# EvolEcolGroup/tidypopgen

Hardware: AMD Instinct MI355X
Metric: SNP-genotypes/s (N x M) for IBS+KING+GRM+Fst+PCA; max |delta| vs CPU ref (cpu_baseline.parity) (higher is better)
Workload: dtype fp4-e2m1 operands (exact integers, f32 accumulate) for the cross-products, the PCA Gram and the grouped counts, int8 (int32 accumulate) for the loadings, f64 for statistics

## Files before the change

### tidypopgen_amd/csrc/admix.hip

```cpp
#include "common.h"
#include "synth_common.h"

#include <math.h>

namespace {

constexpr int ADM_CHUNK = TPG_ADMIX_CHUNK_LOCI;
static_assert(ADM_CHUNK % 128 == 0, "a chunk is whole blocks of T");
constexpr uint64_t ADM_F_SALT = 0xF0F0F0F0F0F0F0F0ull;

__host__ __device__ inline double admix_u(uint64_t h) { return ((double)(h >> 11) + 0.5) * 0x1p-53; }

__device__ __forceinline__ double admix_clamp(double f) {
  return f < TPG_ADMIX_EPS ? TPG_ADMIX_EPS : f > 1.0 - TPG_ADMIX_EPS ? 1.0 - TPG_ADMIX_EPS : f;
}
__device__ __forceinline__ bool admix_finite(double x) { return fabs(x) <= 1.79769313486231570815e308; }

__device__ __forceinline__ int admix_code(uint32_t w, int e) { return (int)((w >> (8 * (e & 3) + 2 * (e >> 2))) & 3u); }

__global__ void admix_seed_q_kernel(double* __restrict__ Qd, int64_t n, int K, int KT, uint64_t seed) {
  const int64_t i = (int64_t)blockIdx.x * blockDim.x + threadIdx.x;
  if (i >= n) return;
  const uint64_t key = tpg_mix64(seed ^ tpg_mix64((uint64_t)i));
  double s = 0;
// ... 183 lines not shown
        pb = fma(qv[k], 1.0 - fs[k], pb);
      }
      cnt++;
      const double w1 = (double)g / p, w0 = (double)(2 - g) / pb;
#pragma unroll
      for (int k = 0; k < KT; k++) S[k] = fma(1.0 - fs[k], w0, fma(fs[k], w1, S[k]));
    }
  }
#pragma unroll
  for (int k = 0; k < KT; k++) S[k] += __shfl_xor(S[k], 32);
  cnt += __shfl_xor(cnt, 32);
  admix_wave_order_sum<KT>(S, cnt, stage, cnts, w, r, h);
  if (w != 0 || h != 0 || i >= n) return;
  const int64_t o = c * n + i;
#pragma unroll
  for (int k = 0; k < KT; k++) part[o * KT + k] = S[k];
  cpart[o] = cnt;
}

__global__ void admix_q_combine_kernel(const double* __restrict__ part, const int32_t* __restrict__ cpart, int64_t nchunks, int64_t n,
                                       int K, int KT, const double* __restrict__ Qd, double* __restrict__ Qn) {
  const int64_t idx = (int64_t)blockIdx.x * blockDim.x + threadIdx.x;
  if (idx >= n * KT) return;
  const int64_t i = idx / KT;
  const int k = (int)(idx % KT);
  double q = 0.0;
  if (k < K) {
    double s = 0.0;
    int64_t t = 0;
    for (int64_t c = 0; c < nchunks; c++) {
      s += part[(c * n + i) * KT + k];
      t += cpart[c * n + i];
    }
    q = Qd[idx];
    if (t > 0) q = (q / (2.0 * (double)t)) * s;
  }
  Qn[idx] = q;
}

__global__ __launch_bounds__(256) void admix_ll_sum_kernel(const double* __restrict__ ll_part, int64_t ntiles, double* __restrict__ out) {
  __shared__ double wll[4];
  double s = 0.0;
  for (int64_t t = threadIdx.x; t < ntiles; t += 256) s += ll_part[t];
  for (int o = 32; o > 0; o >>= 1) s += __shfl_xor(s, o);
  if ((threadIdx.x & 63) == 0) wll[threadIdx.x >> 6] = s;
  __syncthreads();
  if (threadIdx.x == 0) *out = ((wll[0] + wll[1]) + wll[2]) + wll[3];
}

int admix_kt(int K) { return K <= 4 ? K : K <= 8 ? 8 : K <= 16 ? 16 : 32; }

#define ADM_DISPATCH(kt, CALL) \
  switch (kt) {                \
    case 1: CALL(1); break;    \
    case 2: CALL(2); break;    \
    case 3: CALL(3); break;    \
    case 4: CALL(4); break;    \
    case 8: CALL(8); break;    \
    case 16: CALL(16); break;  \
    default: CALL(32); break;  \
  }

struct AdmixRun {
  tpg_ctx* ctx;
  const tpg_view* v;
  int K, KT;
  int64_t n, m, n_lt, n_rt, nchunks;
  DevArena sc;
  double *Q[2] = {}, *F[2] = {}, *part = nullptr, *ll_part = nullptr, *trace = nullptr;
  int32_t *cpart = nullptr, *flag = nullptr;

  int init(tpg_ctx* c, const tpg_view* view, int k, bool need_q_sweep, bool need_f_next, int64_t trace_len) {
    ctx = c; v = view; K = k; KT = admix_kt(k);
    n = v->n; m = v->m;
    n_lt = ceil_div(m, 32); n_rt = ceil_div(n, 32); nchunks = ceil_div(m, ADM_CHUNK);
    TPG_REQUIRE(n_lt <= 0x7FFFFFFF && n_rt <= 0x7FFFFFFF && nchunks <= 65535, TPG_EUNSUPPORTED, "admixture on a view of %lld x %lld",
                (long long)n, (long long)m);
    TPG_TRY(sc.get(&Q[0], (size_t)n * KT));
    TPG_TRY(sc.get(&F[0], (size_t)m * KT));
    TPG_TRY(sc.get(&ll_part, (size_t)n_lt));
    TPG_TRY(sc.get(&trace, (size_t)trace_len));
    TPG_TRY(sc.get(&flag, (size_t)1));
    if (need_f_next) TPG_TRY(sc.get(&F[1], (size_t)m * KT));
    if (need_q_sweep) {
      TPG_TRY(tpg_view_need_T(ctx, v));
      TPG_TRY(sc.get(&Q[1], (size_t)n * KT));
      TPG_TRY(sc.get(&part, (size_t)nchunks * n * KT));
      TPG_TRY(sc.get(&cpart, (size_t)nchunks * n));
    }
    return TPG_OK;
  }

  int f_sweep(int cur_q, int cur_f, bool update, int64_t slot) {
#define ADM_F(KT_)                                                                                                                  \
  do {                                                                                                                              \
    auto k_upd = admix_f_sweep_kernel<KT_, true>;                                                                                   \
    auto k_ll = admix_f_sweep_kernel<KT_, false>;                                                                                   \
    if (update)                                                                                                                     \
      TPG_LAUNCH(ctx, "admix_f_sweep", k_upd, dim3((unsigned)n_lt), dim3(256), 0, (const uint32_t*)v->L, \
                 v->Q, n, m, K, (const double*)Q[cur_q], (const double*)F[cur_f], F[1 - cur_f], ll_part);                           \
    else                                                                                                                            \
      TPG_LAUNCH(ctx, "admix_loglik", k_ll, dim3((unsigned)n_lt), dim3(256), 0, (const uint32_t*)v->L, \
                 v->Q, n, m, K, (const double*)Q[cur_q], (const double*)F[cur_f], (double*)nullptr, ll_part);                       \
  } while (0)
    ADM_DISPATCH(KT, ADM_F);
#undef ADM_F
    TPG_LAUNCH(ctx, "admix_ll_sum", admix_ll_sum_kernel, dim3(1), dim3(256), 0, (const double*)ll_part, n_lt, trace + slot);
    TPG_CHECK_LAUNCH();
    return TPG_OK;
  }

  int q_sweep(int cur_q, int cur_f) {
#define ADM_Q(KT_)                                                                                                               \
  TPG_LAUNCH(ctx, "admix_q_sweep", admix_q_sweep_kernel<KT_>, dim3((unsigned)n_rt, (unsigned)nchunks), dim3(256), 0,              \
             (const uint32_t*)v->T, v->KG, n, m, (const double*)Q[cur_q], (const double*)F[cur_f], part, cpart)
    ADM_DISPATCH(KT, ADM_Q);
#undef ADM_Q
    TPG_LAUNCH(ctx, "admix_q_combine", admix_q_combine_kernel, dim3((unsigned)ceil_div(n * KT, 256)), dim3(256), 0, (const double*)part,
               (const int32_t*)cpart, nchunks, n, K, KT, (const double*)Q[cur_q], Q[1 - cur_q]);
    TPG_CHECK_LAUNCH();
    return TPG_OK;
  }
};

int admix_check_view(const tpg_view* v, int K) {
  TPG_REQUIRE(K >= 1 && K <= TPG_ADMIX_MAX_K, TPG_EINVAL, "K = %d out of [1, %d]", K, TPG_ADMIX_MAX_K);
  TPG_REQUIRE(v->n > 0 && v->m > 0, TPG_EINVAL, "admixture needs at least one individual and one locus (view of %lld x %lld)",
              (long long)v->n, (long long)v->m);
  return TPG_OK;
}

}

extern "C" int64_t tpg_admix_chunk_loci(void) { return ADM_CHUNK; }

extern "C" int tpg_admix_params_default(tpg_admix_params* p) {
  TPG_REQUIRE(p, TPG_EINVAL, "null argument");
  p->max_iter = 1000;
  p->tol = 1e-4;
  p->update_q = 1;
  p->update_f = 1;
  p->seed = 0;
  return TPG_OK;
}

extern "C" int tpg_admix_em(tpg_ctx* ctx, const tpg_view* v, const double* ploidy, int K, const tpg_admix_params* params,
                            const double* q0, const double* f0, double* Q, double* P, double* loglik, double* loglik_trace,
                            int32_t* n_iter, int32_t* converged) {
  TpgEnter _enter(ctx);
  TPG_REQUIRE(ctx && v && Q && P, TPG_EINVAL, "null argument");
  tpg_admix_params pr;
  tpg_admix_params_default(&pr);
  if (params) pr = *params;
  TPG_TRY(admix_check_view(v, K));
  TPG_REQUIRE(pr.max_iter >= 0, TPG_EINVAL, "max_iter = %d is negative", (int)pr.max_iter);
  TPG_REQUIRE(pr.tol >= 0.0, TPG_EINVAL, "tol must be a non-negative number");
  TPG_TRY(tpg_require_diploid(v->n, ploidy, "admixture"));
  const bool upd_q = pr.update_q != 0, upd_f = pr.update_f != 0;
  const int64_t n = v->n, m = v->m;
  AdmixRun run;
  TPG_TRY(run.init(ctx, v, K, upd_q && pr.max_iter > 0, upd_f && pr.max_iter > 0, (int64_t)pr.max_iter + 1));
  const int KT = run.KT;
  const unsigned gn = (unsigned)ceil_div(n, 256), gm = (unsigned)ceil_div(m, 256);
  InBuf iq, ifr;
  TPG_HIP(hipMemsetAsync(run.flag, 0, sizeof(int32_t), ctx->stream));
  if (q0) {
// ... 72 lines not shown
```

### tidypopgen_amd/csrc/common.h

```cpp
#pragma once
#include <hip/hip_runtime.h>
#include <stdint.h>
#include <stdlib.h>

#include <map>
#include <memory>
#include <set>
#include <string>
#include <vector>

#include "../../include/tpg.h"

void tpg_set_error(const char* fmt, ...);

#define TPG_HIP(call)                                                                        \
  do {                                                                                       \
    hipError_t _e = (call);                                                                  \
    if (_e != hipSuccess) {                                                                  \
      tpg_set_error("%s:%d: %s -> %s", __FILE__, __LINE__, #call, hipGetErrorString(_e));     \
      return TPG_EHIP;                                                                       \
    }                                                                                        \
  } while (0)

#define TPG_REQUIRE(cond, code, ...)  \
// ... 47 lines not shown

struct ProfScope {
  tpg_ctx* ctx;
  ProfRec rec;
  bool on;
  ProfScope(tpg_ctx* c, const char* name);
  ~ProfScope();
};
int tpg_prof_resolve(tpg_ctx* ctx);
int tpg_gram_classes(tpg_ctx* ctx, const struct tpg_view* v, const double* d_w, double* d_what, double* d_K, bool* done,
                     bool centred_ok);
int tpg_gram_classes_exchanged(tpg_ctx* ctx, struct tpg_comm* comm, const struct tpg_view* v, const int32_t* d_counts,
                               const double* d_scale, double* d_K, bool* done);

#define TPG_LAUNCH(ctx, name, kernel, grid, block, shmem, ...)                          \
  do {                                                                                  \
    ProfScope _ps((ctx), (name));                                                       \
    hipLaunchKernelGGL(kernel, grid, block, shmem, (ctx)->stream, __VA_ARGS__);        \
  } while (0)

#define TPG_CHECK_LAUNCH() TPG_HIP(hipGetLastError())

struct tpg_fbm {
  tpg_ctx* ctx;
  uint8_t* d_bytes;
  int64_t nrow, ncol;
  int64_t bed_bpl = 0;
  bool pooled = false;
};

struct GroupedCounts {
  int32_t* cnt = nullptr;
  int64_t Mpad = 0;
  int Cpad = 0;
  int nclass = 0;
};

static inline int64_t ceil_div(int64_t a, int64_t b) { return (a + b - 1) / b; }

hipError_t tpg_pmalloc(void** p, size_t bytes);
void tpg_pfree(void* p);
void tpg_pool_trim(int pool_id);
struct TpgEnter {
  tpg_ctx* prev;
  explicit TpgEnter(tpg_ctx* ctx);
  ~TpgEnter();
};
tpg_ctx* tpg_current_ctx();

struct DevBuf {
  void* p = nullptr;
  int alloc(size_t bytes) {
    free();
    TPG_HIP(tpg_pmalloc(&p, bytes ? bytes : 16));
    return TPG_OK;
  }
  template <typename T> int alloc_n(size_t count) { return alloc(sizeof(T) * count); }
  void free() { if (p) tpg_pfree(p); p = nullptr; }
  void* release() { void* q = p; p = nullptr; return q; }
  template <typename T> T* as() const { return (T*)p; }
  DevBuf() = default;
  DevBuf(DevBuf&& o) noexcept : p(o.release()) {}
  DevBuf& operator=(DevBuf&& o) noexcept { if (this != &o) { free(); p = o.release(); } return *this; }
  DevBuf(const DevBuf&) = delete;
  DevBuf& operator=(const DevBuf&) = delete;
  ~DevBuf() { free(); }
};
struct DevArena {
  std::vector<DevBuf> blocks;
  template <typename T> int get(T** p, size_t count) {
    DevBuf b;
    TPG_TRY(b.alloc_n<T>(count));
    *p = b.as<T>();
    blocks.push_back(std::move(b));
    return TPG_OK;
  }
};

struct tpg_view {
  tpg_ctx* ctx;
  int64_t n, m;
  int64_t Q, KG;
  mutable uint4* T = nullptr;
  uint4* L;
  bool L_borrowed = false;
  size_t bytes_each;
  mutable uint4* T4 = nullptr;
  mutable DevBuf gc_buf;
  mutable GroupedCounts gc_cache;
  mutable std::vector<int32_t> gc_cls;
  uint32_t* lc_part = nullptr;
  int lc_chunks = 0;
  int64_t lc_row = 0;

  tpg_view(tpg_ctx* c, int64_t n_, int64_t m_, uint4* borrowed_L = nullptr)
      : ctx(c), n(n_), m(m_), Q(ceil_div(n_, 128)), KG(ceil_div(m_, 128)), L(borrowed_L), L_borrowed(borrowed_L != nullptr),
        bytes_each((size_t)Q * (size_t)KG * 4096) {}
  tpg_view(const tpg_view&) = delete;
  tpg_view& operator=(const tpg_view&) = delete;
  ~tpg_view();
  void drop_derived();
};
typedef std::unique_ptr<tpg_view> ViewPtr;

#define TPG_PW_PRODUCTS 5
enum { TPG_PW_SLAB_MM = 0, TPG_PW_SLAB_D = 1 , TPG_PW_SLAB_H = 2, TPG_PW_SLAB_HM = 3, TPG_PW_SLAB_MH = 4 };
#define TPG_PW_TA 3
#define TPG_PW_PLANE_INTS (TPG_PW_TA * 16 * 64)
#define TPG_PW_TILE_INTS (TPG_PW_PRODUCTS * TPG_PW_PLANE_INTS)
struct tpg_pairwise {
  tpg_ctx* ctx;
  int64_t n;
  int64_t nst;
  int64_t ntp;
  int32_t* acc;
  bool owns;
  void* order;
  int64_t nun;
  int64_t loci;
  int64_t as_pad_quirk;
  int nranks = 1, rank = 0;
  int64_t chunk_units = 0, tail_units = 0;
  std::vector<int32_t> band;
  int64_t* rowpad = nullptr;
  bool reduced = false;
  bool reducing = false;
  hipEvent_t ev_acc = nullptr, ev_red = nullptr;
  int64_t pending_loci = 0;
  int pending_lack = 0;
  int have = 31;
  std::map<int, std::pair<void*, int64_t>> orders;
};
#define TPG_PW_MAX_LOCI 2147483647ll
#define TPG_PW_HAVE_ALL (TPG_PW_ALL | TPG_PW_DH)
static inline int tpg_pw_products_for(bool ibs, bool king, bool as_or_grm) {
  if (ibs && !king && !as_or_grm) return TPG_PW_FOR_IBS_ALONE;
  return (ibs ? TPG_PW_FOR_IBS : 0) | (king ? TPG_PW_FOR_KING : 0) | (as_or_grm ? TPG_PW_FOR_AS : 0);
}

static inline bool tpg_env_set(const char* name) { return getenv(name) != nullptr; }
static inline int tpg_env_int(const char* name, int dflt) {
  const char* e = getenv(name);
  return e ? atoi(e) : dflt;
}

hipError_t tpg_h2d_async(tpg_ctx* ctx, void* dst, const void* src, size_t bytes);
hipError_t tpg_fetch_small(tpg_ctx* ctx, void* host_dst, const void* d_src, size_t bytes);
hipError_t tpg_push_small(tpg_ctx* ctx, void* d_dst, const void* host_src, size_t bytes);
hipError_t tpg_copy_dev(tpg_ctx* ctx, void* d_dst, const void* d_src, size_t bytes);
hipError_t tpg_upload(tpg_ctx* ctx, void* dst, const void* src, size_t bytes);
hipError_t tpg_download(tpg_ctx* ctx, void* dst, const void* src, size_t bytes);
int tpg_fbm_from_host_for_table(tpg_ctx* ctx, const uint8_t* bytes, int64_t nrow, int64_t ncol, const double* code256, tpg_fbm** out,
                                const double** view_table);
hipError_t tpg_upload_bedpacked(tpg_ctx* ctx, uint8_t* dst, const uint8_t* src, int64_t nrow, int64_t ncols, const uint8_t* lut16, bool* ok);
hipError_t tpg_download_rows(tpg_ctx* ctx, void* dst, size_t dpitch, const void* src, size_t width, size_t height);
void tpg_stage_keep(int buffers);

template <typename T>
static inline int tpg_dmalloc(T** p, size_t count) {
  TPG_HIP(hipMalloc((void**)p, count * sizeof(T) > 0 ? count * sizeof(T) : 16));
  return TPG_OK;
}

bool tpg_is_device_ptr(const void* p);
struct OutBuf {
  void* user = nullptr;
  void* d = nullptr;
  size_t bytes = 0;
  bool owned = false;
  int init(void* user_ptr, size_t nbytes);
  int commit(tpg_ctx* ctx);
  ~OutBuf();
  template <typename T> T* dev() { return (T*)d; }
};
struct InBuf {
  const void* d = nullptr;
  void* owned_ptr = nullptr;
  int init(tpg_ctx* ctx, const void* user_ptr, size_t nbytes);
  ~InBuf();
  template <typename T> const T* dev() { return (const T*)d; }
};
template <typename T>
struct HostIn {
  const T* p = nullptr;
  std::vector<T> keep;
  int init(tpg_ctx* ctx, const T* user, int64_t count) {
    p = user;
    if (!tpg_is_device_ptr(user)) return TPG_OK;
    keep.resize((size_t)count);
    TPG_HIP(tpg_download(ctx, keep.data(), user, sizeof(T) * (size_t)count));
    p = keep.data();
    return TPG_OK;
  }
  const T& operator[](int64_t i) const { return p[i]; }
};
int tpg_check_ranges(tpg_ctx* ctx, const int64_t* lo, const int64_t* hi, int64_t count, int64_t m, const char* what);

void tpg_resident_release(tpg_ctx* ctx);

struct tpg_comm {
  tpg_ctx* ctx = nullptr;
  int nranks = 1, rank = 0;
  void* nccl = nullptr;
  int (*host_fn)(void* user, void* buf, int64_t count, int dtype) = nullptr;
  void* host_user = nullptr;
  int32_t* d_status = nullptr;
  int a2a_state = 0;
};
#define TPG_COMM_STATUS_INTS 8
int tpg_sym_eig_topk_tol(tpg_ctx* ctx, const double* d_K, int64_t n, int k, double tol, double* lambda_host, double* d_U);
int tpg_pca_gram_allreduce(tpg_ctx* ctx, tpg_comm* comm, double* d_K, int64_t n);
int tpg_multi_stream_host(tpg_multi* mg, const uint8_t* fbm_bytes, int64_t nrow, int64_t ncol, size_t budget, const tpg_stream_job* job);
int tpg_comm_agree(tpg_comm* comm, int rc);
int tpg_comm_reduce_scatter_i32(tpg_comm* comm, int32_t* d_buf, int64_t chunk_count);
int tpg_comm_allreduce(tpg_comm* comm, void* d_buf, int64_t count, int dtype);
bool tpg_comm_alltoall_usable(tpg_comm* comm);
int tpg_comm_alltoallv64(tpg_comm* comm, const void* d_send, const size_t* scnt, const size_t* soff, void* d_recv,
                         const size_t* rcnt, const size_t* roff);

int tpg_launch_pack(tpg_ctx* ctx, const tpg_fbm* fbm, const int32_t* d_rows, const int32_t* d_cols,
                    const uint8_t* d_lut, tpg_view* v, tpg_view* v2);
int tpg_launch_unpack(tpg_ctx* ctx, const tpg_view* v, uint8_t* d_codes, int from_L);
int tpg_view_need_T(tpg_ctx* ctx, const tpg_view* v);
int tpg_view_impute_at(tpg_ctx* ctx, const tpg_view* raw, int method, uint64_t seed, int64_t col0, tpg_view** out,
                       tpg_impute_report* rep);
int tpg_launch_synth(tpg_ctx* ctx, uint8_t* d_bytes, uint64_t seed, int64_t nrow, int64_t ncol, int64_t j0,
                     int npop, uint32_t miss_thresh, int imputed_bytes);

int tpg_launch_loci_counts(tpg_ctx* ctx, const tpg_view* v, int32_t* d_counts );
int tpg_grouped_counts(tpg_ctx* ctx, const tpg_view* v, const int32_t* h_cls, int nclass, GroupedCounts* out);
struct ClassPlan {
  std::vector<int32_t> cls;
  std::vector<int32_t> group_size;
  int nclass = 0;
  int has_hap = 0;
};
int make_class_plan(int64_t n, const int32_t* groupIds0, int ngroups, const double* ploidy, ClassPlan* cp);
int tpg_check_group_ids(int64_t n, const int32_t* groupIds0, int ngroups);
int tpg_require_diploid(int64_t n, const double* ploidy, const char* what);
int tpg_launch_indiv_accumulate(tpg_ctx* ctx, const tpg_view* v, int32_t* d_acc);
int tpg_launch_indiv_finish(tpg_ctx* ctx, const int32_t* d_acc, int64_t n, int64_t m, int32_t* d_out);
```

### tidypopgen_amd/csrc/gramcls.hip

```cpp
#include <math.h>
#include <string.h>

#include <algorithm>
#include <vector>

#include <hipcub/hipcub.hpp>

#include "common.h"
#include "devfrag.h"
#include "host/host_bits2.h"

typedef int v8i __attribute__((ext_vector_type(8)));
typedef float v16f __attribute__((ext_vector_type(16)));
typedef uint32_t v4u __attribute__((ext_vector_type(4)));

constexpr int GA = 2, GB = 2, GP = GA * GB;
#define GCLS_SLAB (GP * 16 * 64)
#define GCLS_MAX_RUN 65536

__global__ void tpg_gcls_keys_kernel(const double* __restrict__ w, int64_t m, unsigned long long* __restrict__ key,
                                     uint32_t* __restrict__ idx) {
  for (int64_t j = blockIdx.x * (int64_t)blockDim.x + threadIdx.x; j < m; j += (int64_t)gridDim.x * blockDim.x) {
    const unsigned long long b = (unsigned long long)__double_as_longlong(w[j]);
    key[j] = (b + 16ull) & ~31ull;
// ... 640 lines not shown
  const double cost_dig = (double)ceil_div(nun_dig, (int64_t)(4 * ncu8)) * ((double)ceil_div(m, 128) * 0.25 * t_dig) + 65.0;
  while ((nblocks / 2 + S) / S + 2 >= (1 << 21)) S += 2;
  if (tpg_env_set("TPG_DEBUG"))
    fprintf(stderr, "[tpg] gram classes: %lld classes, %lld blocks for %lld loci, S = %d, model %.0f us (digits %.0f us)\n",
            (long long)nruns, (long long)nblocks, (long long)m, S, cost_cls, cost_dig);
  if (cost_cls > cost_dig && !force && !tpg_env_set("TPG_GRAM_CLASSES")) return TPG_OK;

  int32_t* d_src = nullptr;
  double* d_slabs = nullptr;
  unsigned long long* d_wblk = nullptr;
  ulonglong2* d_wblk2 = nullptr;
  uint4* d_T2g = nullptr;
  int2* d_order = nullptr;
  TPG_TRY(B.get(&d_src, (size_t)nblocks * 64));
  if (f64) TPG_TRY(B.get(&d_wblk, (size_t)nblocks));
  else TPG_TRY(B.get(&d_wblk2, (size_t)nblocks + 4));
  const int64_t rs2 = (nblocks + 1) / 2;
  TPG_TRY(B.get(&d_T2g, (size_t)(4 * Q) * (size_t)rs2 * 64));
  TPG_TRY(B.get(&d_order, (size_t)nun));
  TPG_TRY(B.get(&d_slabs, (size_t)S * (size_t)nun * GCLS_SLAB));
  TPG_HIP(tpg_h2d_async(ctx, d_order, order.data(), sizeof(int2) * (size_t)nun));
  TPG_HIP(hipMemsetAsync(d_src, 0xFF, sizeof(int32_t) * (size_t)nblocks * 64, ctx->stream));
  {
    ProfScope ps(ctx, "gcls_layout");
    hipLaunchKernelGGL(tpg_gcls_place_kernel, dim3(1024), dim3(256), 0, ctx->stream, (const uint32_t*)d_idx2,
                       (const unsigned long long*)d_ukeys, (const uint32_t*)d_estart, (const uint32_t*)d_bstart, (int)nruns, m,
                       d_src, d_what);
    if (f64)
      hipLaunchKernelGGL(tpg_gcls_block_table_kernel, dim3(256), dim3(256), 0, ctx->stream, (const unsigned long long*)d_ukeys,
                         (const uint32_t*)d_bstart, (const uint32_t*)d_nblk, (int)nruns, nblocks, d_wblk);
    else
      hipLaunchKernelGGL(tpg_gcls_block_table2_kernel, dim3(256), dim3(256), 0, ctx->stream, (const unsigned long long*)d_ukeys,
                         (const uint32_t*)d_bstart, (const uint32_t*)d_nblk, (int)nruns, nblocks, GCLS_GMAX, GCLS_GQ, d_wblk2);
  }
  {
    const int64_t tasks = Q * rs2;
    if (tasks >= ((int64_t)1 << 31)) return TPG_OK;
    const unsigned grid = (unsigned)std::min<int64_t>(ceil_div(tasks, 4), (int64_t)ctx->num_cu * 16);
    const int qw = tpg_env_int("TPG_GATHER_QW", Q >= 4 ? 4 : Q >= 2 ? 2 : 1);
#define GATHER_GO(C, W) TPG_LAUNCH(ctx, "gcls_gather", (tpg_gcls_gather_kernel<C, W>), dim3(grid), dim3(256), 0, src, Q, (const int32_t*)d_src, nblocks, rs2, d_T2g)
    if (cen) { if (qw == 4) GATHER_GO(true, 4); else if (qw == 2) GATHER_GO(true, 2); else GATHER_GO(true, 1); }
    else { if (qw == 4) GATHER_GO(false, 4); else if (qw == 2) GATHER_GO(false, 2); else GATHER_GO(false, 1); }
#undef GATHER_GO
  }
  if (f64)
    TPG_LAUNCH(ctx, "pca_gram_classes", tpg_gcls_gram_kernel, dim3((unsigned)nblk_grid), dim3(256), 0, (const uint4*)d_T2g, nblocks,
               rs2, nrtv, (const unsigned long long*)d_wblk, (const int2*)d_order, nun, S, d_slabs);
  else if (cen) {
    (void)hipFuncSetAttribute((const void*)tpg_gcls_gram2_kernel<true>, hipFuncAttributeMaxDynamicSharedMemorySize, GCLS2_LDS_BYTES);
    TPG_LAUNCH(ctx, "pca_gram_classes", tpg_gcls_gram2_kernel<true>, dim3((unsigned)nblk_grid), dim3(256), GCLS2_LDS_BYTES,
               (const uint4*)d_T2g, nblocks, rs2, nrtv, (const ulonglong2*)d_wblk2, (const int2*)d_order, nun, S, d_slabs);
  } else {
    (void)hipFuncSetAttribute((const void*)tpg_gcls_gram2_kernel<false>, hipFuncAttributeMaxDynamicSharedMemorySize, GCLS2_LDS_BYTES);
    TPG_LAUNCH(ctx, "pca_gram_classes", tpg_gcls_gram2_kernel<false>, dim3((unsigned)nblk_grid), dim3(256), GCLS2_LDS_BYTES,
               (const uint4*)d_T2g, nblocks, rs2, nrtv, (const ulonglong2*)d_wblk2, (const int2*)d_order, nun, S, d_slabs);
  }
  TPG_LAUNCH(ctx, "gcls_assemble", tpg_gcls_assemble_kernel, dim3((unsigned)std::min<int64_t>(nun, 4096)), dim3(256), 0,
             (const double*)d_slabs, (const int2*)d_order, nun, S, (int)n, d_K);
  TPG_CHECK_LAUNCH();
  *done = true;
  return TPG_OK;
}

__global__ __launch_bounds__(256) void tpg_gcls_l2lm_kernel(const uint4* __restrict__ L, int64_t Q, int64_t n_lt,
                                                            uint4* __restrict__ LM) {
  __shared__ uint4 sh[32][8];
  const int64_t QG = (Q + 3) / 4;
  const int lane = threadIdx.x & 63, wv = threadIdx.x >> 6;
  for (int64_t task = blockIdx.x; task < n_lt * QG; task += gridDim.x) {
    const int64_t lt = task / QG, q0 = (task % QG) * 4;
    if (q0 + wv < Q) sh[lane & 31][2 * wv + (lane >> 5)] = L[(lt * Q + q0 + wv) * 64 + lane];
    __syncthreads();
    const int r = threadIdx.x >> 3, p = threadIdx.x & 7;
    if (q0 + (p >> 1) < Q) LM[((lt * 32 + r) * Q + q0) * 2 + p] = sh[r][p];
    __syncthreads();
  }
}

int tpg_gram_classes(tpg_ctx* ctx, const tpg_view* v, const double* d_w, double* d_what, double* d_K, bool* done,
                     bool centred_ok) {
  *done = false;
  if (tpg_env_set("TPG_GRAM_DIGITS")) return TPG_OK;
  const int64_t n_lt = 4 * v->KG;
  DevBuf d_LM;
  TPG_TRY(d_LM.alloc_n<uint4>((size_t)n_lt * 32 * (size_t)v->Q * 2));
  TPG_LAUNCH(ctx, "gcls_l2lm", tpg_gcls_l2lm_kernel, dim3((unsigned)std::min<int64_t>(n_lt * ((v->Q + 3) / 4), (int64_t)ctx->num_cu * 32)),
             dim3(256), 0, (const uint4*)v->L, v->Q, n_lt, d_LM.as<uint4>());
  const GclsSrc src{d_LM.as<uint4>(), 0, 2 * v->Q, 0, 0, 2, 1};
  const int rc = gram_classes_core(ctx, v->n, v->Q, v->m, src, d_w, d_what, d_K, false, done, centred_ok);
  d_LM.free();
  return rc;
}

#define GCLX_REC_WORDS(Q) (4 * (Q) + 2)

__global__ void tpg_gclx_keys_kernel(const int32_t* __restrict__ counts, int64_t m, int n, int32_t* __restrict__ key,
                                     int32_t* __restrict__ hist) {
  for (int64_t j = blockIdx.x * (int64_t)blockDim.x + threadIdx.x; j < m; j += (int64_t)gridDim.x * blockDim.x) {
    const int c = counts[4 * j + 1] + 2 * counts[4 * j + 2];
    const int k = min(c, 2 * n - c);
    key[j] = k;
    atomicAdd(&hist[k], 1);
  }
}

__global__ void tpg_gclx_dest_kernel(const int32_t* __restrict__ key, int64_t m, const uint8_t* __restrict__ owner,
                                     uint32_t* __restrict__ dest, uint32_t* __restrict__ idx, int32_t* __restrict__ per_dest) {
  for (int64_t j = blockIdx.x * (int64_t)blockDim.x + threadIdx.x; j < m; j += (int64_t)gridDim.x * blockDim.x) {
    const uint32_t d = owner[key[j]];
    dest[j] = d;
    idx[j] = (uint32_t)j;
    atomicAdd(&per_dest[d], 1);
  }
}

__global__ __launch_bounds__(256) void tpg_gclx_pack_kernel(const uint4* __restrict__ L, int64_t Q, const uint32_t* __restrict__ order,
                                                            const double* __restrict__ scale, int64_t m,
                                                            uint4* __restrict__ rec) {
  const int lane = threadIdx.x & 63;
  const int64_t recq = 2 * Q + 1;
  for (int64_t i = (int64_t)blockIdx.x * 4 + (threadIdx.x >> 6); i < m; i += (int64_t)gridDim.x * 4) {
    const uint32_t j = order[i];
    const uint4* p = L + ((int64_t)(j >> 5) * Q) * 64 + (j & 31);
    for (int64_t t = lane; t < 2 * Q; t += 64) rec[i * recq + t] = p[(t >> 1) * 64 + (t & 1) * 32];
    if (lane == 0) {
      const double sc = scale[j], w = 1.0 / (sc * sc);
      rec[i * recq + 2 * Q] = make_uint4((uint32_t)__double_as_longlong(w), (uint32_t)(__double_as_longlong(w) >> 32), 0u, 0u);
    }
  }
}

__global__ void tpg_gclx_weights_kernel(const uint4* __restrict__ rec, int64_t Q, int64_t m, double* __restrict__ w) {
  const int64_t recq = 2 * Q + 1;
  for (int64_t i = blockIdx.x * (int64_t)blockDim.x + threadIdx.x; i < m; i += (int64_t)gridDim.x * blockDim.x) {
    const uint4 t = rec[i * recq + 2 * Q];
    w[i] = __longlong_as_double((long long)(((unsigned long long)t.y << 32) | t.x));
  }
}

int tpg_gram_classes_exchanged(tpg_ctx* ctx, tpg_comm* comm, const tpg_view* v, const int32_t* d_counts, const double* d_scale,
                               double* d_K, bool* done) {
  *done = false;
  const int R = comm->nranks, me = comm->rank;
  const int64_t n = v->n, m = v->m, Q = v->Q;
  if (R < 2 || R > 255 || n >= (1 << 30) || tpg_env_set("TPG_GRAM_NO_EXCHANGE")) return TPG_OK;
  DevArena B;
  int32_t *d_key = nullptr, *d_hist = nullptr, *d_perdest = nullptr;
  uint8_t* d_owner = nullptr;
  uint32_t *d_dest = nullptr, *d_dest2 = nullptr, *d_idx = nullptr, *d_idx2 = nullptr;
  void* d_tmp = nullptr;
  size_t t_sort = 0;
  std::vector<int32_t> hist((size_t)n + 1, 0);
  auto local = [&]() -> int {
    TPG_TRY(B.get(&d_key, (size_t)std::max<int64_t>(m, 1)));
    TPG_TRY(B.get(&d_hist, (size_t)n + 1));
    TPG_TRY(B.get(&d_perdest, (size_t)R));
    TPG_TRY(B.get(&d_owner, (size_t)n + 1));
    TPG_TRY(B.get(&d_dest, (size_t)std::max<int64_t>(m, 1)));
    TPG_TRY(B.get(&d_dest2, (size_t)std::max<int64_t>(m, 1)));
    TPG_TRY(B.get(&d_idx, (size_t)std::max<int64_t>(m, 1)));
    TPG_TRY(B.get(&d_idx2, (size_t)std::max<int64_t>(m, 1)));
    TPG_HIP(hipcub::DeviceRadixSort::SortPairs(nullptr, t_sort, d_dest, d_dest2, d_idx, d_idx2, (int)m, 0, 8, ctx->stream));
    TPG_TRY(B.get((uint8_t**)&d_tmp, t_sort));
    TPG_HIP(hipMemsetAsync(d_hist, 0, sizeof(int32_t) * ((size_t)n + 1), ctx->stream));
    TPG_HIP(hipMemsetAsync(d_perdest, 0, sizeof(int32_t) * (size_t)R, ctx->stream));
    if (m > 0)
      TPG_LAUNCH(ctx, "gclx_keys", tpg_gclx_keys_kernel, dim3(512), dim3(256), 0, d_counts, m, (int)n, d_key, d_hist);
    TPG_CHECK_LAUNCH();
    return TPG_OK;
  };
  TPG_TRY(tpg_comm_agree(comm, local()));
  if (!tpg_comm_alltoall_usable(comm)) return TPG_OK;
  {
    ProfScope ps(ctx, "gclx_histogram");
    TPG_TRY(tpg_comm_allreduce(comm, d_hist, n + 1, 0));
    TPG_HIP(hipMemcpyAsync(hist.data(), d_hist, sizeof(int32_t) * ((size_t)n + 1), hipMemcpyDeviceToHost, ctx->stream));
    TPG_HIP(hipStreamSynchronize(ctx->stream));
  }
  int64_t m_all = 0, runs_all = 0, blocks_all = 0;
  for (int64_t k = 0; k <= n; k++)
    if (hist[(size_t)k] > 0) { m_all += hist[(size_t)k]; runs_all++; blocks_all += ((int64_t)hist[(size_t)k] + 63) / 64; }
  if (m_all == 0) return TPG_OK;
  const double cost_all = (double)runs_all * 0.136 + (double)blocks_all * 0.079;
  const int nrtv = (int)ceil_div(n, 32);
  const double units = (double)nrtv * (double)nrtv / 8.0, waves = 8.0 * (double)(ctx->num_cu > 8 ? ctx->num_cu : 8);
  const double t_exch = units / waves * 4.0 * cost_all / R + 700.0 + (double)m_all / R * (double)(32 * Q + 16) / 300e3;
  const double shard_blocks = (double)blocks_all / R + (double)runs_all;
  const double t_cls_local = units / waves * 4.0 * ((double)runs_all * 0.136 + shard_blocks * 0.079) + 650.0;
  const double t_dig_local = ((double)nrtv * nrtv / 8.0 + nrtv) / (waves / 2.0) * ((double)m_all / R / 128.0) + 65.0;
  if (tpg_env_set("TPG_DEBUG") && me == 0)
    fprintf(stderr, "[tpg] gram exchange: %lld loci, %lld classes, %lld blocks over %d ranks: model %.0f us (local classes %.0f, digits %.0f)\n",
            (long long)m_all, (long long)runs_all, (long long)blocks_all, R, t_exch, t_cls_local, t_dig_local);
  if (t_exch > std::min(t_cls_local, t_dig_local) && !tpg_env_set("TPG_GRAM_EXCHANGE")) return TPG_OK;

  std::vector<uint8_t> owner((size_t)n + 1, (uint8_t)(R - 1));
  {
    double acc = 0;
    int r = 0;
    for (int64_t k = 0; k <= n; k++) {
      owner[(size_t)k] = (uint8_t)r;
      if (hist[(size_t)k] > 0) acc += 0.136 + 0.079 * (double)(((int64_t)hist[(size_t)k] + 63) / 64);
      while (r < R - 1 && acc >= cost_all * (double)(r + 1) / R) r++;
    }
  }
  std::vector<int32_t> per_dest((size_t)R, 0);
  uint4 *d_send = nullptr, *d_recv = nullptr;
  double* d_w = nullptr;
  const int64_t recq = 2 * Q + 1;
  std::vector<size_t> scnt((size_t)R), soff((size_t)R), rcnt((size_t)R), roff((size_t)R);
  std::vector<int32_t> cm((size_t)R * R, 0);
  int64_t m_in = 0;
  auto pack = [&]() -> int {
    TPG_HIP(tpg_h2d_async(ctx, d_owner, owner.data(), (size_t)n + 1));
    if (m > 0) {
      ProfScope ps(ctx, "gclx_sort");
      hipLaunchKernelGGL(tpg_gclx_dest_kernel, dim3(512), dim3(256), 0, ctx->stream, (const int32_t*)d_key, m, (const uint8_t*)d_owner,
                         d_dest, d_idx, d_perdest);
      size_t t = t_sort;
      TPG_HIP(hipcub::DeviceRadixSort::SortPairs(d_tmp, t, d_dest, d_dest2, d_idx, d_idx2, (int)m, 0, 8, ctx->stream));
    }
    TPG_HIP(hipMemcpyAsync(per_dest.data(), d_perdest, sizeof(int32_t) * (size_t)R, hipMemcpyDeviceToHost, ctx->stream));
    TPG_HIP(hipStreamSynchronize(ctx->stream));
    TPG_TRY(B.get(&d_send, (size_t)std::max<int64_t>(m, 1) * (size_t)recq));
    if (m > 0)
      TPG_LAUNCH(ctx, "gclx_pack", tpg_gclx_pack_kernel, dim3((unsigned)std::min<int64_t>(ceil_div(m, 4), (int64_t)ctx->num_cu * 16)),
                 dim3(256), 0, (const uint4*)v->L, Q, (const uint32_t*)d_idx2, d_scale, m, d_send);
    TPG_HIP(hipGetLastError());
    return TPG_OK;
  };
  TPG_TRY(tpg_comm_agree(comm, pack()));
  {
    int32_t* d_cm = nullptr;
    auto cm_up = [&]() -> int {
      TPG_TRY(B.get(&d_cm, (size_t)R * R));
      for (int d = 0; d < R; d++) cm[(size_t)me * R + d] = per_dest[(size_t)d];
      TPG_HIP(tpg_h2d_async(ctx, d_cm, cm.data(), sizeof(int32_t) * (size_t)R * R));
      return TPG_OK;
    };
    TPG_TRY(tpg_comm_agree(comm, cm_up()));
    TPG_TRY(tpg_comm_allreduce(comm, d_cm, (int64_t)R * R, 0));
    TPG_HIP(hipMemcpyAsync(cm.data(), d_cm, sizeof(int32_t) * (size_t)R * R, hipMemcpyDeviceToHost, ctx->stream));
    TPG_HIP(hipStreamSynchronize(ctx->stream));
  }
  {
    size_t so = 0, ro = 0;
    for (int r = 0; r < R; r++) {
      scnt[(size_t)r] = (size_t)cm[(size_t)me * R + r] * (size_t)recq * 2;
      soff[(size_t)r] = so;
      so += scnt[(size_t)r];
      rcnt[(size_t)r] = (size_t)cm[(size_t)r * R + me] * (size_t)recq * 2;
      roff[(size_t)r] = ro;
      ro += rcnt[(size_t)r];
      m_in += cm[(size_t)r * R + me];
    }
  }
  auto recv_alloc = [&]() -> int {
    TPG_TRY(B.get(&d_recv, (size_t)std::max<int64_t>(m_in, 1) * (size_t)recq));
    TPG_TRY(B.get(&d_w, (size_t)std::max<int64_t>(m_in, 1)));
    return TPG_OK;
  };
  TPG_TRY(tpg_comm_agree(comm, recv_alloc()));
  {
    ProfScope ps(ctx, "gclx_alltoall");
    TPG_TRY(tpg_comm_alltoallv64(comm, d_send, scnt.data(), soff.data(), d_recv, rcnt.data(), roff.data()));
  }
  if (m_in == 0) {
    TPG_HIP(hipMemsetAsync(d_K, 0, sizeof(double) * (size_t)n * (size_t)n, ctx->stream));
    *done = true;
    return TPG_OK;
  }
  TPG_LAUNCH(ctx, "gclx_weights", tpg_gclx_weights_kernel, dim3(512), dim3(256), 0, (const uint4*)d_recv, Q, m_in, d_w);
  const GclsSrc src{d_recv, 0, recq, 0, 0, 2, 1};
  bool ok = false;
  TPG_TRY(gram_classes_core(ctx, n, Q, m_in, src, d_w, nullptr, d_K, true, &ok, true));
  TPG_REQUIRE(ok, TPG_EHIP, "class Gram of the exchanged loci was not computed");
  *done = true;
  return TPG_OK;
}
```

### tidypopgen_amd/csrc/impute.hip

```cpp
#include <stdlib.h>
#include <string.h>

#include <algorithm>

#include "common.h"
#include "devfrag.h"
#include "synth_common.h"

TPG_HD int tpg_impute_fill(int method, int64_t c0, int64_t c1, int64_t c2) {
  if (method == TPG_IMPUTE_MODE) {
    int v = 0;
    int64_t best = c0;
    if (c1 > best) { v = 1; best = c1; }
    if (c2 > best) v = 2;
    return v;
  }
  const int64_t t = c0 + c1 + c2, s2 = 2 * (c1 + 2 * c2);
  if (s2 <= t) return 0;
  if (s2 < 3 * t) return 1;
  return 2;
}
TPG_HD uint64_t tpg_impute_locus_key(uint64_t seed, uint64_t j) { return tpg_mix64(seed ^ tpg_mix64(j)); }
TPG_HD int tpg_impute_draw(uint64_t locus_key, uint64_t i, uint64_t thr) {
  const uint64_t h = tpg_mix64(locus_key ^ tpg_mix64(i));
// ... 225 lines not shown
    TPG_HIP(hipStreamSynchronize(ctx->stream));
  }
  stat.free();
  TPG_REQUIRE(h[2] == 0, TPG_EUNSUPPORTED, "object x is already imputed (%llu loci hold a store byte above 3; the store is unchanged)",
              h[2]);
  if (rep) {
    rep->imputed = (int64_t)h[0];
    rep->loci_all_missing = (int64_t)h[1];
  }
  return TPG_OK;
}

__global__ __launch_bounds__(256) void tpg_impute_view_kernel(const uint4* __restrict__ L, uint4* __restrict__ out, int64_t n_lt, int64_t Q,
                                                              int64_t n, int64_t m, int method, uint64_t seed, int64_t col0,
                                                              unsigned long long* __restrict__ d_rep) {
  const int lane = threadIdx.x & 63, r = lane & 31, h = lane >> 5;
  const int64_t lt = (int64_t)blockIdx.x * 4 + (threadIdx.x >> 6);
  if (lt >= n_lt) return;
  const uint4* p = L + (lt * Q) * 64 + lane;
  uint4* o = out + (lt * Q) * 64 + lane;
  int c1 = 0, c2 = 0, c3 = 0;
  for (int64_t q = 0; q < Q; q++) {
    const uint4 a = p[q * 64];
    const uint32_t w[4] = {a.x, a.y, a.z, a.w};
#pragma unroll
    for (int d = 0; d < 4; d++) {
      const uint32_t lo = w[d] & 0x55555555u, hi = (w[d] >> 1) & 0x55555555u;
      c1 += __popc(lo & ~hi);
      c2 += __popc(hi & ~lo);
      c3 += __popc(lo & hi);
    }
  }
  c1 += __shfl_xor(c1, 32);
  c2 += __shfl_xor(c2, 32);
  c3 += __shfl_xor(c3, 32);
  const int64_t j = lt * 32 + r;
  c3 -= (int)(Q * 128 - n);
  const int64_t c0 = n - c1 - c2 - c3, t = n - c3, s = (int64_t)c1 + 2 * (int64_t)c2;
  const bool fill = j < m && t > 0 && c3 > 0;
  const int v = fill && method != TPG_IMPUTE_RANDOM ? tpg_impute_fill(method, c0, c1, c2) : 0;
  const uint64_t key = tpg_impute_locus_key(seed, (uint64_t)(col0 + j)), thr = fill ? ((uint64_t)s << 31) / (uint64_t)t : 0;
  for (int64_t q = 0; q < Q; q++) {
    const uint4 a = p[q * 64];
    uint32_t w[4] = {a.x, a.y, a.z, a.w};
    if (fill) {
#pragma unroll
      for (int d = 0; d < 4; d++) {
        const int64_t base = 128 * q + 32 * d + 16 * h;
        uint32_t miss = w[d] & (w[d] >> 1) & 0x55555555u;
        if (base + 16 > n) {
          uint32_t real = 0;
          for (int e = 0; e < 16; e++)
            if (base + e < n) real |= 1u << tpg_elem_shift(e);
          miss &= real;
        }
        if (method != TPG_IMPUTE_RANDOM) {
          w[d] = (w[d] & ~(miss * 3u)) | (miss * (uint32_t)v);
        } else {
          while (miss) {
            const int pos = __ffs(miss) - 1;
            miss &= miss - 1;
            const int e = 4 * ((pos & 7) >> 1) + (pos >> 3);
            const int vv = tpg_impute_draw(key, (uint64_t)(base + e), thr);
            w[d] = (w[d] & ~(3u << pos)) | ((uint32_t)vv << pos);
          }
        }
      }
    }
    o[q * 64] = make_uint4(w[0], w[1], w[2], w[3]);
  }
  int imp = lane < 32 && fill ? c3 : 0, allmiss = lane < 32 && j < m && t == 0 ? 1 : 0;
  imp = wave_sum(imp);
  allmiss = wave_sum(allmiss);
  if (lane == 0) {
    if (imp) atomicAdd(d_rep, (unsigned long long)imp);
    if (allmiss) atomicAdd(d_rep + 1, (unsigned long long)allmiss);
  }
}

int tpg_view_impute_at(tpg_ctx* ctx, const tpg_view* raw, int method, uint64_t seed, int64_t col0, tpg_view** out,
                       tpg_impute_report* rep) {
  TPG_REQUIRE(ctx && raw && out, TPG_EINVAL, "null argument");
  TPG_TRY(check_method(method));
  TPG_REQUIRE(raw->L, TPG_EINVAL, "the view has no locus-tiled layout");
  ViewPtr v(new tpg_view(ctx, raw->n, raw->m));
  DevBuf d_rep;
  TPG_HIP(tpg_pmalloc((void**)&v->L, v->bytes_each));
  TPG_TRY(d_rep.alloc(16));
  TPG_HIP(hipMemsetAsync(d_rep.p, 0, 16, ctx->stream));
  const int64_t n_lt = 4 * raw->KG;
  TPG_LAUNCH(ctx, "impute_view", tpg_impute_view_kernel, dim3((unsigned)ceil_div(n_lt, 4)), dim3(256), 0, (const uint4*)raw->L, v->L, n_lt,
             raw->Q, raw->n, raw->m, method, seed, col0, d_rep.as<unsigned long long>());
  TPG_CHECK_LAUNCH();
  unsigned long long h[2] = {0, 0};
  if (rep) TPG_HIP(tpg_fetch_small(ctx, h, d_rep.p, sizeof(h)));
  if (rep) {
    rep->imputed = (int64_t)h[0];
    rep->loci_all_missing = (int64_t)h[1];
  }
  *out = v.release();
  return TPG_OK;
}

extern "C" int tpg_view_impute(tpg_ctx* ctx, const tpg_view* raw, int method, uint64_t seed, tpg_view** out, tpg_impute_report* rep) {
  TpgEnter _enter(ctx);
  return tpg_view_impute_at(ctx, raw, method, seed, 0, out, rep);
}
```

### tidypopgen_amd/csrc/ld.hip

```cpp
#include "common.h"
#include "devfrag.h"
#include <hipcub/hipcub.hpp>

#include <cmath>

#define TPG_LD_MAX_N (1ll << 22)
#define TPG_LD_MAX_ROUNDS 32
#define LD_TK 4
#define LD_SC (4 * LD_TK)
#define LD_UNDECIDED 0
#define LD_KEPT 1
#define LD_FALLEN 2

typedef int ld_v8i __attribute__((ext_vector_type(8)));
typedef float ld_v16f __attribute__((ext_vector_type(16)));
#define LD_MFMA(a, b, c)                                                                                         \
  __builtin_amdgcn_mfma_scale_f32_32x32x64_f8f6f4((ld_v8i){(int)(a)[0], (int)(a)[1], (int)(a)[2], (int)(a)[3], 0, 0, 0, 0}, \
                                                  (ld_v8i){(int)(b)[0], (int)(b)[1], (int)(b)[2], (int)(b)[3], 0, 0, 0, 0}, (c), 4, 4, 0, \
                                                  (int)0x80808080, 0, (int)0x80808080)

__device__ __forceinline__ void ld_operand(const uint4& f, int S, uint32_t (&o)[4]) {
  const uint32_t p0 = S == 0 ? f.x : f.z, p1 = S == 0 ? f.y : f.w;
  o[0] = p0 & 0x33333333u;
  o[1] = (p0 >> 2) & 0x33333333u;
// ... 257 lines not shown
          base = ju + 1 + 32 * w;
        } else {
          word = back[ju * bstride + (w - stride)];
          base = ((ju >> 5) - (w - stride)) * 32;
        }
        while (word) {
          const int bb = __ffs((int)word) - 1;
          word &= word - 1;
          any |= __hip_atomic_load(&state[base + bb], __ATOMIC_RELAXED, __HIP_MEMORY_SCOPE_AGENT) == LD_KEPT;
        }
      }
      const bool falls = __ballot(any) != 0;
      if (lane == 0)
        __hip_atomic_store(&state[ju], (uint8_t)(falls ? LD_FALLEN : LD_KEPT), __ATOMIC_RELEASE, __HIP_MEMORY_SCOPE_AGENT);
      __builtin_amdgcn_fence(__ATOMIC_SEQ_CST, "agent");
    }
  }
}

__global__ __launch_bounds__(256) void tpg_ld_keep_kernel(const uint8_t* __restrict__ state, int64_t m, uint8_t* __restrict__ keep,
                                                          unsigned long long* __restrict__ kept) {
  const int64_t j = (int64_t)blockIdx.x * 256 + threadIdx.x;
  const int k = j < m && state[j] == LD_KEPT;
  if (j < m) keep[j] = (uint8_t)k;
  const unsigned long long bal = __ballot(k);
  if ((threadIdx.x & 63) == 0 && bal) atomicAdd(kept, (unsigned long long)__popcll(bal));
}

namespace {

struct LdBand {
  int64_t words = 0;
  int32_t* d_sx = nullptr;
  double* d_dd = nullptr;
  int64_t* d_hi = nullptr;
  int32_t* d_flags = nullptr;
  unsigned long long* d_counters = nullptr;
};

int ld_window(tpg_ctx* ctx, const int64_t* hi, int64_t m, HostIn<int64_t>& h, int64_t* words) {
  TPG_TRY(h.init(ctx, hi, m));
  int64_t W = 0;
  for (int64_t j = 0; j < m; j++) {
    TPG_REQUIRE(h[(size_t)j] >= j && h[(size_t)j] < m, TPG_EINVAL, "hi[%lld] = %lld outside [%lld, %lld)", (long long)j,
                (long long)h[(size_t)j], (long long)j, (long long)m);
    TPG_REQUIRE(j == 0 || h[(size_t)j] >= h[(size_t)j - 1], TPG_EINVAL, "hi decreases at locus %lld", (long long)j);
    if (h[(size_t)j] - j > W) W = h[(size_t)j] - j;
  }
  *words = ceil_div(W, 32);
  return TPG_OK;
}

int ld_check_args(tpg_ctx* ctx, const tpg_view* v, const int64_t* hi, double thr_r2) {
  TPG_REQUIRE(ctx && v && hi, TPG_EINVAL, "null argument");
  TPG_REQUIRE(thr_r2 >= 0.0 && thr_r2 <= 1.0, TPG_EINVAL, "thr_r2 must lie in [0, 1]");
  TPG_REQUIRE(v->m >= 1 && v->n >= 1, TPG_EINVAL, "empty view");
  TPG_REQUIRE(v->n < TPG_LD_MAX_N, TPG_EUNSUPPORTED, "LD of 2^22 individuals or more");
  TPG_REQUIRE(v->m < (1ll << 31) - 64, TPG_EUNSUPPORTED, "LD of 2^31 loci or more");
  return TPG_OK;
}

int ld_prepare(tpg_ctx* ctx, const tpg_view* v, const HostIn<int64_t>& h, DevArena& sc, LdBand* B) {
  const int64_t m = v->m;
  int32_t* d_counts = nullptr;
  TPG_TRY(sc.get(&d_counts, 4 * (size_t)m));
  TPG_TRY(sc.get(&B->d_sx, (size_t)m));
  TPG_TRY(sc.get(&B->d_dd, (size_t)m));
  TPG_TRY(sc.get(&B->d_hi, (size_t)m));
  TPG_TRY(sc.get(&B->d_flags, 1));
  TPG_TRY(sc.get(&B->d_counters, 2 + TPG_LD_MAX_ROUNDS));
  TPG_HIP(hipMemsetAsync(B->d_flags, 0, sizeof(int32_t), ctx->stream));
  TPG_HIP(hipMemsetAsync(B->d_counters, 0, sizeof(unsigned long long) * (2 + TPG_LD_MAX_ROUNDS), ctx->stream));
  TPG_TRY(tpg_launch_loci_counts(ctx, v, d_counts));
  TPG_LAUNCH(ctx, "ld_prep", tpg_ld_prep_kernel, dim3((unsigned)ceil_div(m, 256)), dim3(256), 0, (const int4*)d_counts, v->n, m,
             B->d_sx, B->d_dd, B->d_flags);
  TPG_CHECK_LAUNCH();
  TPG_HIP(tpg_upload(ctx, B->d_hi, h.p, sizeof(int64_t) * (size_t)m));
  return TPG_OK;
}

int ld_launch_band(tpg_ctx* ctx, const tpg_view* v, double thr_r2, const LdBand& B, uint32_t* d_bits, int64_t stride,
                   uint32_t* d_back, int64_t bstride) {
  const int64_t m = v->m;
  if (stride > 0) TPG_HIP(hipMemsetAsync(d_bits, 0, sizeof(uint32_t) * (size_t)m * (size_t)stride, ctx->stream));
  if (d_back) TPG_HIP(hipMemsetAsync(d_back, 0, sizeof(uint32_t) * (size_t)m * (size_t)bstride, ctx->stream));
  TPG_LAUNCH(ctx, "ld_band", tpg_ld_band_kernel, dim3((unsigned)ceil_div(m, 32)), dim3(256), 0, (const uint4*)v->L, v->Q, v->n,
             m, (const int64_t*)B.d_hi, (const int32_t*)B.d_sx, (const double*)B.d_dd, thr_r2, d_bits, stride, d_back,
             bstride, B.d_counters);
  TPG_CHECK_LAUNCH();
  return TPG_OK;
}

}

extern "C" int tpg_ld_band_links(tpg_ctx* ctx, const tpg_view* v, const int64_t* hi, double thr_r2, uint32_t* bits,
                                 int64_t stride_words, int64_t* n_links) {
  TpgEnter _enter(ctx);
  TPG_TRY(ld_check_args(ctx, v, hi, thr_r2));
  TPG_REQUIRE(stride_words >= 0 && (bits || stride_words == 0), TPG_EINVAL, "null argument");
  HostIn<int64_t> h;
  LdBand B;
  TPG_TRY(ld_window(ctx, hi, v->m, h, &B.words));
  TPG_REQUIRE(stride_words >= B.words, TPG_EINVAL, "stride_words = %lld, the window needs %lld", (long long)stride_words,
              (long long)B.words);
  DevArena sc;
  TPG_TRY(ld_prepare(ctx, v, h, sc, &B));
  int32_t flags = 0;
  TPG_HIP(tpg_fetch_small(ctx, &flags, B.d_flags, sizeof(flags)));
  TPG_REQUIRE(!(flags & 1), TPG_ENUMERIC, "LD of a view with missing genotypes (impute it first)");
  unsigned long long links = 0;
  if (stride_words > 0) {
    OutBuf o;
    TPG_TRY(o.init(bits, sizeof(uint32_t) * (size_t)v->m * (size_t)stride_words));
    TPG_TRY(ld_launch_band(ctx, v, thr_r2, B, o.dev<uint32_t>(), stride_words, nullptr, 0));
    TPG_HIP(tpg_fetch_small(ctx, &links, B.d_counters, sizeof(links)));
    TPG_TRY(o.commit(ctx));
  }
  if (n_links) *n_links = (int64_t)links;
  return TPG_OK;
}

extern "C" int tpg_ld_clump(tpg_ctx* ctx, const tpg_view* v, const int64_t* hi, double thr_r2, const double* S,
                            const uint8_t* exclude, uint8_t* keep, tpg_ld_report* report) {
  TpgEnter _enter(ctx);
  TPG_TRY(ld_check_args(ctx, v, hi, thr_r2));
  TPG_REQUIRE(keep, TPG_EINVAL, "null argument");
  const int64_t m = v->m;
  HostIn<int64_t> h;
  LdBand B;
  TPG_TRY(ld_window(ctx, hi, m, h, &B.words));
  const int64_t stride = B.words > 0 ? B.words : 1, bstride = B.words + 1;
  DevArena sc;
  TPG_TRY(ld_prepare(ctx, v, h, sc, &B));
  InBuf inS, inX;
  if (S) TPG_TRY(inS.init(ctx, S, sizeof(double) * (size_t)m));
  if (exclude) TPG_TRY(inX.init(ctx, exclude, (size_t)m));
  unsigned long long *d_key = nullptr, *d_key2 = nullptr;
  uint32_t *d_idx = nullptr, *d_order = nullptr, *d_rank = nullptr;
  uint8_t *d_s0 = nullptr, *d_s1 = nullptr;
  TPG_TRY(sc.get(&d_key, (size_t)m));
  TPG_TRY(sc.get(&d_key2, (size_t)m));
  TPG_TRY(sc.get(&d_idx, (size_t)m));
  TPG_TRY(sc.get(&d_order, (size_t)m));
  TPG_TRY(sc.get(&d_rank, (size_t)m));
  TPG_TRY(sc.get(&d_s0, (size_t)m));
  TPG_TRY(sc.get(&d_s1, (size_t)m));
  const unsigned g256 = (unsigned)ceil_div(m, 256);
  TPG_LAUNCH(ctx, "ld_key", tpg_ld_key_kernel, dim3(g256), dim3(256), 0, (const int32_t*)B.d_sx, S ? inS.dev<double>() : nullptr,
             v->n, m, d_key, d_idx, B.d_flags);
  TPG_CHECK_LAUNCH();
  int32_t flags = 0;
  TPG_HIP(tpg_fetch_small(ctx, &flags, B.d_flags, sizeof(flags)));
  TPG_REQUIRE(!(flags & 1), TPG_ENUMERIC, "LD clumping of a view with missing genotypes (impute it first)");
  TPG_REQUIRE(!(flags & 2), TPG_EINVAL, "NaN in S");
  {
    const int end_bit = S ? 64 : 24;
    size_t t_sort = 0;
    TPG_HIP(hipcub::DeviceRadixSort::SortPairs(nullptr, t_sort, d_key, d_key2, d_idx, d_order, (int)m, 0, end_bit, ctx->stream));
    uint8_t* d_tmp = nullptr;
    TPG_TRY(sc.get(&d_tmp, t_sort));
    ProfScope ps(ctx, "ld_sort");
    TPG_HIP(hipcub::DeviceRadixSort::SortPairs(d_tmp, t_sort, d_key, d_key2, d_idx, d_order, (int)m, 0, end_bit, ctx->stream));
  }
  TPG_LAUNCH(ctx, "ld_rank", tpg_ld_rank_kernel, dim3(g256), dim3(256), 0, (const uint32_t*)d_order, m, d_rank,
             exclude ? inX.dev<uint8_t>() : nullptr, d_s0);
  TPG_CHECK_LAUNCH();
// ... 40 lines not shown
```

### tidypopgen_amd/csrc/loci.hip

```cpp
#include <string.h>

#include "common.h"
#include <type_traits>
#include "devfrag.h"

__global__ __launch_bounds__(256) void tpg_loci_counts_kernel(const uint4* __restrict__ L, int64_t n_lt,
                                                              int64_t Q, int64_t n, int64_t m,
                                                              int4* __restrict__ out) {
  const int lane = threadIdx.x & 63;
  const int64_t lt = (int64_t)blockIdx.x * 4 + (threadIdx.x >> 6);
  if (lt >= n_lt) return;
  const uint4* p = L + (lt * Q) * 64 + lane;
  int c_lo = 0, c_hi = 0, c_both = 0;
  auto acc = [&](uint32_t w) {
    const uint32_t lo = w & 0x55555555u, hi = (w >> 1) & 0x55555555u;
    c_lo += __popc(lo);
    c_hi += __popc(hi);
    c_both += __popc(lo & hi);
  };
  int64_t q = 0;
  for (; q + 4 <= Q; q += 4) {
    uint4 a0 = p[(q + 0) * 64], a1 = p[(q + 1) * 64], a2 = p[(q + 2) * 64], a3 = p[(q + 3) * 64];
    acc(a0.x); acc(a0.y); acc(a0.z); acc(a0.w);
    acc(a1.x); acc(a1.y); acc(a1.z); acc(a1.w);
    acc(a2.x); acc(a2.y); acc(a2.z); acc(a2.w);
    acc(a3.x); acc(a3.y); acc(a3.z); acc(a3.w);
  }
  for (; q < Q; q++) {
    uint4 a0 = p[q * 64];
    acc(a0.x); acc(a0.y); acc(a0.z); acc(a0.w);
  }
  c_lo += __shfl_xor(c_lo, 32);
  c_hi += __shfl_xor(c_hi, 32);
  c_both += __shfl_xor(c_both, 32);
  const int64_t j = lt * 32 + (lane & 31);
  if (lane < 32 && j < m) {
    const int n3 = c_both, n1 = c_lo - c_both, n2 = c_hi - c_both;
    const int npad = (int)(Q * 128 - n);
    out[j] = make_int4((int)(Q * 128) - n1 - n2 - n3, n1, n2, n3 - npad);
  }
}

__global__ __launch_bounds__(256) void tpg_loci_counts_sum_kernel(const uint32_t* __restrict__ part, int chunks, int64_t row,
                                                                  int64_t n, int64_t m, int4* __restrict__ out) {
  const int64_t j = (int64_t)blockIdx.x * 256 + threadIdx.x;
  if (j >= m) return;
  int lo = 0, hi = 0, both = 0;
  for (int c = 0; c < chunks; c++) {
    const uint32_t w = part[(int64_t)c * row + j];
    lo += (int)(w & 1023u);
    hi += (int)((w >> 10) & 1023u);
    both += (int)(w >> 20);
  }
  const int n1 = lo - both, n2 = hi - both;
  out[j] = make_int4((int)n - n1 - n2 - both, n1, n2, both);
}

int tpg_launch_loci_counts(tpg_ctx* ctx, const tpg_view* v, int32_t* d_counts) {
  if (v->lc_part) {
    TPG_LAUNCH(ctx, "loci_counts", tpg_loci_counts_sum_kernel, dim3((unsigned)ceil_div(v->m, 256)), dim3(256), 0,
               (const uint32_t*)v->lc_part, v->lc_chunks, v->lc_row, v->n, v->m, (int4*)d_counts);
    TPG_CHECK_LAUNCH();
    return TPG_OK;
  }
  const int64_t n_lt = v->KG * 4;
  TPG_LAUNCH(ctx, "loci_counts", tpg_loci_counts_kernel, dim3((unsigned)ceil_div(n_lt, 4)), dim3(256), 0,
             (const uint4*)v->L, n_lt, v->Q, v->n, v->m, (int4*)d_counts);
  TPG_CHECK_LAUNCH();
  return TPG_OK;
}

extern "C" int tpg_loci_counts(tpg_ctx* ctx, const tpg_view* v, int32_t* out) {
  TpgEnter _enter(ctx);
  TPG_REQUIRE(ctx && v && out, TPG_EINVAL, "null argument");
  OutBuf o;
  TPG_TRY(o.init(out, sizeof(int32_t) * 4 * (size_t)v->m));
  TPG_TRY(tpg_launch_loci_counts(ctx, v, o.dev<int32_t>()));
  return o.commit(ctx);
}

extern "C" int tpg_indiv_counts(tpg_ctx* ctx, const tpg_view* v, int32_t* out) {
  TpgEnter _enter(ctx);
  TPG_REQUIRE(ctx && v && out, TPG_EINVAL, "null argument");
  OutBuf o;
  TPG_TRY(o.init(out, sizeof(int32_t) * 4 * (size_t)v->n));
  TPG_TRY(tpg_view_need_T(ctx, v));
  const int64_t n_rt = v->Q * 4;
  TPG_LAUNCH(ctx, "indiv_counts", tpg_loci_counts_kernel, dim3((unsigned)ceil_div(n_rt, 4)), dim3(256), 0,
             (const uint4*)v->T, n_rt, v->KG, v->m, v->n, o.dev<int4>());
  TPG_CHECK_LAUNCH();
  return o.commit(ctx);
}

#define TPG_IA_STRIDE 49
__global__ __launch_bounds__(256) void tpg_indiv_accumulate_kernel(const uint4* __restrict__ L, int64_t n_lt, int64_t Q,
                                                                   int64_t n, int64_t m, int tiles,
                                                                   int32_t* __restrict__ acc) {
  __shared__ uint32_t red[4][64 * TPG_IA_STRIDE];
  const int lane = threadIdx.x & 63, wave = threadIdx.x >> 6;
  const int64_t q = (int64_t)blockIdx.x * 4 + wave;
  const int64_t lt0 = (int64_t)blockIdx.y * tiles, lt1 = lt0 + tiles < n_lt ? lt0 + tiles : n_lt;
  uint32_t a8[4][3][4] = {};
  if (q < Q) {
    const uint4* p = L + q * 64 + lane;
    const int64_t r = lane & 31;
    for (int64_t base = lt0; base < lt1; base += 15) {
      uint32_t a4[4][3][2] = {};
#pragma unroll
      for (int g = 0; g < 5; g++) {
        uint32_t a2[4][3] = {};
#pragma unroll
        for (int u = 0; u < 3; u++) {
          const int64_t lt = base + 3 * g + u;
          uint4 w = make_uint4(0, 0, 0, 0);
          if (lt < lt1 && lt * 32 + r < m) w = p[lt * Q * 64];
          const uint32_t ws[4] = {w.x, w.y, w.z, w.w};
#pragma unroll
          for (int s = 0; s < 4; s++) {
            const uint32_t lo = ws[s] & 0x55555555u, hi = (ws[s] >> 1) & 0x55555555u;
            a2[s][0] += lo;
            a2[s][1] += hi;
            a2[s][2] += lo & hi;
          }
        }
#pragma unroll
        for (int s = 0; s < 4; s++)
#pragma unroll
          for (int pl = 0; pl < 3; pl++) {
            a4[s][pl][0] += a2[s][pl] & 0x33333333u;
            a4[s][pl][1] += (a2[s][pl] >> 2) & 0x33333333u;
          }
      }
#pragma unroll
      for (int s = 0; s < 4; s++)
#pragma unroll
        for (int pl = 0; pl < 3; pl++)
#pragma unroll
          for (int e = 0; e < 2; e++) {
            a8[s][pl][e] += a4[s][pl][e] & 0x0F0F0F0Fu;
            a8[s][pl][2 + e] += (a4[s][pl][e] >> 4) & 0x0F0F0F0Fu;
          }
    }
  }
  uint32_t* my = red[wave];
#pragma unroll
  for (int s = 0; s < 4; s++)
#pragma unroll
    for (int pl = 0; pl < 3; pl++)
#pragma unroll
      for (int k = 0; k < 4; k++) my[lane * TPG_IA_STRIDE + (s * 3 + pl) * 4 + k] = a8[s][pl][k];
  __syncthreads();
  if (q >= Q) return;
  for (int item = lane; item < 96; item += 64) {
    const int h = item / 48, j = item % 48;
    uint32_t ev = 0, od = 0;
    for (int r = 0; r < 32; r++) {
      const uint32_t x = my[(32 * h + r) * TPG_IA_STRIDE + j];
      ev += x & 0x00FF00FFu;
      od += (x >> 8) & 0x00FF00FFu;
    }
    const int k = j & 3, pl = (j >> 2) % 3, s = j / 12;
    const int64_t i0 = q * 128 + 32 * s + 16 * h + 4 * k;
    const uint32_t c[4] = {ev & 0xFFFFu, od & 0xFFFFu, ev >> 16, od >> 16};
#pragma unroll
    for (int b = 0; b < 4; b++)
      if (c[b] && i0 + b < n) atomicAdd(acc + (i0 + b) * 4 + 1 + pl, (int32_t)c[b]);
  }
}

__global__ void tpg_indiv_finish_kernel(const int4* acc, int64_t n, int32_t m, int4* out) {
  for (int64_t i = blockIdx.x * (int64_t)blockDim.x + threadIdx.x; i < n; i += (int64_t)gridDim.x * blockDim.x) {
    const int4 a = acc[i];
    const int n1 = a.y - a.w, n2 = a.z - a.w;
    out[i] = make_int4(m - n1 - n2 - a.w, n1, n2, a.w);
  }
}

int tpg_launch_indiv_accumulate(tpg_ctx* ctx, const tpg_view* v, int32_t* d_acc) {
  const int64_t n_lt = ceil_div(v->m, 32), gx = ceil_div(v->Q, 4);
  int64_t tiles = ceil_div(ceil_div(n_lt, ceil_div(4 * (int64_t)ctx->num_cu, gx)), 15) * 15;
  tiles = tiles < 30 ? 30 : tiles > 255 ? 255 : tiles;
  const int64_t gy = ceil_div(n_lt, tiles);
  TPG_REQUIRE(gy <= 65535 && gx <= 0x7FFFFFFF, TPG_EUNSUPPORTED, "per-individual counts of a view of %lld x %lld", (long long)v->n,
              (long long)v->m);
  TPG_LAUNCH(ctx, "indiv_accumulate", tpg_indiv_accumulate_kernel, dim3((unsigned)gx, (unsigned)gy), dim3(256), 0,
             (const uint4*)v->L, n_lt, v->Q, v->n, v->m, (int)tiles, d_acc);
  TPG_CHECK_LAUNCH();
  return TPG_OK;
}

int tpg_launch_indiv_finish(tpg_ctx* ctx, const int32_t* d_acc, int64_t n, int64_t m, int32_t* d_out) {
  TPG_LAUNCH(ctx, "indiv_finish", tpg_indiv_finish_kernel, dim3((unsigned)(ceil_div(n, 256) < 1024 ? ceil_div(n, 256) : 1024)),
             dim3(256), 0, (const int4*)d_acc, n, (int32_t)m, (int4*)d_out);
  TPG_CHECK_LAUNCH();
  return TPG_OK;
}

__global__ void tpg_ind_hetero_kernel(const int4* __restrict__ counts, int64_t n, int32_t* __restrict__ out) {
  for (int64_t i = blockIdx.x * (int64_t)blockDim.x + threadIdx.x; i < n; i += (int64_t)gridDim.x * blockDim.x) {
    out[2 * i] = counts[i].y;
    out[2 * i + 1] = counts[i].w;
  }
}

extern "C" int tpg_gt_ind_hetero(tpg_ctx* ctx, const tpg_view* v, int32_t* out) {
  TpgEnter _enter(ctx);
  TPG_REQUIRE(ctx && v && out, TPG_EINVAL, "null argument");
  DevBuf d_counts;
  TPG_TRY(d_counts.alloc_n<int32_t>(4 * (size_t)v->n));
  TPG_TRY(tpg_indiv_counts(ctx, v, d_counts.as<int32_t>()));
  OutBuf o;
  TPG_TRY(o.init(out, sizeof(int32_t) * 2 * (size_t)v->n));
  TPG_LAUNCH(ctx, "ind_hetero", tpg_ind_hetero_kernel, dim3(256), dim3(256), 0, (const int4*)d_counts.p, v->n, o.dev<int32_t>());
  TPG_CHECK_LAUNCH();
  TPG_HIP(hipStreamSynchronize(ctx->stream));
  return o.commit(ctx);
}

__global__ void tpg_pi_kernel(const int4* __restrict__ counts, int64_t m, double* __restrict__ pi) {
  for (int64_t j = blockIdx.x * (int64_t)blockDim.x + threadIdx.x; j < m; j += (int64_t)gridDim.x * blockDim.x) {
    const int4 c = counts[j];
    const double cnt = (double)(c.y + 2 * c.z), valid = (double)(2 * (c.x + c.y + c.z));
    pi[j] = valid > 0 ? (cnt * (valid - cnt) / (valid * (valid - 1) / 2)) : __longlong_as_double(0x7FF8000000000000ll);
  }
}

extern "C" int tpg_gt_pi_diploid(tpg_ctx* ctx, const tpg_view* v, double* pi) {
  TpgEnter _enter(ctx);
  TPG_REQUIRE(ctx && v && pi, TPG_EINVAL, "null argument");
  DevBuf d_counts;
  TPG_TRY(d_counts.alloc_n<int32_t>(4 * (size_t)v->m));
  TPG_TRY(tpg_launch_loci_counts(ctx, v, d_counts.as<int32_t>()));
  OutBuf o;
  TPG_TRY(o.init(pi, sizeof(double) * (size_t)v->m));
  TPG_LAUNCH(ctx, "pi_diploid", tpg_pi_kernel, dim3(1024), dim3(256), 0, (const int4*)d_counts.p, v->m, o.dev<double>());
  TPG_CHECK_LAUNCH();
  TPG_HIP(hipStreamSynchronize(ctx->stream));
  return o.commit(ctx);
}

__global__ void tpg_onehot_kernel(const int32_t* __restrict__ cls, int64_t n, int64_t Q, int GT,
                                  uint4* __restrict__ OH) {
  const int64_t total = Q * 2 * GT * 64;
  for (int64_t idx = blockIdx.x * (int64_t)blockDim.x + threadIdx.x; idx < total;
       idx += (int64_t)gridDim.x * blockDim.x) {
    const int lane = (int)(idx & 63);
    const int64_t t = idx >> 6;
    const int gt = (int)(t % GT);
    const int64_t qS = t / GT;
    const int S = (int)(qS & 1);
    const int64_t q = qS >> 1;
    const int c = 32 * gt + (lane & 31), h = lane >> 5;
    uint32_t w[4] = {0, 0, 0, 0};
    for (int d = 0; d < 4; d++)
      for (int j = 0; j < 8; j++) {
        const int e = (j >> 1) + 8 * (j & 1) + 4 * (d & 1);
        const int64_t i = 128 * q + 32 * (2 * S + (d >> 1)) + 16 * h + e;
        if (i < n && cls[i] == c) w[d] |= 2u << (4 * j);
      }
    OH[idx] = make_uint4(w[0], w[1], w[2], w[3]);
  }
}

#define GC_NLT 1
#define GC_D 4
template <int C, class F>
__device__ __forceinline__ void gc_static_for(F&& f) {
// ... 65 lines not shown
    constexpr int C = decltype(Cc)::value, M = decltype(Mm)::value;
    static_assert(GC_D % 2 == 0, "the slot of a group's fragments is its parity, known at compile time in the unrolled loop");
    const int qn2 = q + GC_D - 1 < Qi ? q + GC_D - 1 : Qi - 1, qo2 = q + 2 < Qi ? q + 2 : Qi - 1;
    const int cur = q & 1;
#pragma unroll
    for (int t = 0; t < GC_NLT; t++) R[M][t] = LDG(pa[t], qn2);
#pragma unroll
    for (int j = 0; j < NIT; j++) {
      const int it = wv + 4 * j;
      if (it < 2 * GT) on[C & 1][j] = frag(qo2, it);
    }
#pragma unroll
    for (int S = 0; S < 2; S++) {
      uint32_t fy[GC_NLT][4], fz[GC_NLT][4], fw[GC_NLT][4];
#pragma unroll
      for (int t = 0; t < GC_NLT; t++) {
        const uint32_t P[2] = {S == 0 ? R[C][t].x : R[C][t].z, S == 0 ? R[C][t].y : R[C][t].w};
#pragma unroll
        for (int d = 0; d < 4; d++) {
          const uint32_t X = (d & 1) ? (P[d >> 1] >> 2) & 0x33333333u : P[d >> 1] & 0x33333333u;
          fy[t][d] = X & 0x11111111u;
          fz[t][d] = X & 0x22222222u;
          fw[t][d] = fy[t][d] & (fz[t][d] >> 1);
        }
      }
#pragma unroll
      for (int g = 0; g < GT; g++) {
        const uint4 b = ohb[cur][S * GT + g][lane];
#pragma unroll
        for (int t = 0; t < GC_NLT; t++) {
          acc[0][t][g] = GC_MFMA(fy[t], b, acc[0][t][g], (int)0x80808080);
          acc[1][t][g] = GC_MFMA(fz[t], b, acc[1][t][g], 0x7F7F7F7F);
          acc[2][t][g] = GC_MFMA(fw[t], b, acc[2][t][g], (int)0x80808080);
        }
      }
    }
#pragma unroll
    for (int j = 0; j < NIT; j++) {
      const int it = wv + 4 * j;
      if (it < 2 * GT) ohb[cur ^ 1][it][lane] = on[(C & 1) ^ 1][j];
    }
    tpg_lds_barrier();
  };
  for (int q = 0; q < Qi; q += GC_D)
    gc_static_for<GC_D>([&](auto kk) {
      constexpr int k = decltype(kk)::value;
      if (q + k < Qi) group(std::integral_constant<int, k>{}, std::integral_constant<int, (k + GC_D - 1) % GC_D>{}, q + k);
    });
#pragma unroll
  for (int t = 0; t < GC_NLT; t++) {
    if (lt0 + t >= n_lt) break;
#pragma unroll
    for (int g = 0; g < GT; g++) {
      const int cs = csize[32 * (gt0 + g) + (lane & 31)];
#pragma unroll
      for (int r = 0; r < 16; r++) {
        const int64_t row = (lt0 + t) * 32 + tpg_cd_row(r, lane);
        const int64_t o = row * Cpad + 32 * (gt0 + g) + (lane & 31);
        const int nmiss = (int)acc[2][t][g][r];
        cnt[o] = (int)acc[0][t][g][r] - nmiss;
        cnt[Mpad * Cpad + o] = (int)acc[1][t][g][r] - nmiss;
        cnt[2 * Mpad * Cpad + o] = cs - nmiss;
      }
    }
  }
}

int tpg_grouped_counts(tpg_ctx* ctx, const tpg_view* v, const int32_t* h_cls, int nclass, GroupedCounts* out) {
  TPG_REQUIRE(nclass > 0, TPG_EINVAL, "no classes");
  for (int64_t i = 0; i < v->n; i++)
    TPG_REQUIRE(h_cls[i] >= 0 && h_cls[i] < nclass, TPG_EINVAL, "class id %d of individual %lld out of [0,%d)",
                h_cls[i], (long long)i, nclass);
  TPG_REQUIRE(v->n < (1 << 24), TPG_EUNSUPPORTED, "grouped counts of more than 2^24 individuals");
  GroupedCounts& gc = v->gc_cache;
  if (gc.cnt && gc.nclass == nclass && v->gc_cls.size() == (size_t)v->n &&
      memcmp(v->gc_cls.data(), h_cls, sizeof(int32_t) * (size_t)v->n) == 0) {
    *out = gc;
    return TPG_OK;
  }
  const int GT = (int)ceil_div(nclass, 32);
  const int64_t n_lt = v->KG * 4, Mpad = n_lt * 32;
  const int Cpad = GT * 32;
  gc = GroupedCounts();
  TPG_TRY(v->gc_buf.alloc_n<int32_t>(3 * (size_t)Mpad * (size_t)Cpad));
  int32_t* cnt = v->gc_buf.as<int32_t>();
  std::vector<int32_t> h_up((size_t)v->n + (size_t)GT * 32, 0);
  memcpy(h_up.data(), h_cls, sizeof(int32_t) * (size_t)v->n);
  for (int64_t i = 0; i < v->n; i++) h_up[(size_t)v->n + (size_t)h_cls[i]]++;
  DevArena sc;
  int32_t* d_cls = nullptr;
  uint4* d_oh = nullptr;
  TPG_TRY(sc.get(&d_cls, h_up.size()));
  TPG_TRY(sc.get(&d_oh, (size_t)v->Q * 2 * GT * 64));
  TPG_HIP(tpg_h2d_async(ctx, d_cls, h_up.data(), sizeof(int32_t) * h_up.size()));
  TPG_LAUNCH(ctx, "onehot", tpg_onehot_kernel, dim3(1024), dim3(256), 0, d_cls, v->n, v->Q, GT, d_oh);
  const unsigned grid = (unsigned)ceil_div(n_lt, 4 * GC_NLT);
  int g0 = 0;
  while (g0 < GT) {
    if (GT - g0 >= 2) {
      TPG_LAUNCH(ctx, "grouped_counts", tpg_grouped_counts_kernel<2>, dim3(grid), dim3(256), 0, (const uint4*)v->L,
                 (const uint4*)d_oh, n_lt, v->Q, g0, GT, (const int32_t*)(d_cls + v->n), cnt, Mpad, Cpad);
      g0 += 2;
    } else {
      TPG_LAUNCH(ctx, "grouped_counts", tpg_grouped_counts_kernel<1>, dim3(grid), dim3(256), 0, (const uint4*)v->L,
                 (const uint4*)d_oh, n_lt, v->Q, g0, GT, (const int32_t*)(d_cls + v->n), cnt, Mpad, Cpad);
      g0 += 1;
    }
  }
  TPG_CHECK_LAUNCH();
  gc.cnt = cnt;
  gc.Mpad = Mpad;
  gc.Cpad = Cpad;
  gc.nclass = nclass;
  v->gc_cls.assign(h_cls, h_cls + v->n);
  *out = gc;
  return TPG_OK;
}

int tpg_check_group_ids(int64_t n, const int32_t* groupIds0, int ngroups) {
  TPG_REQUIRE(ngroups > 0, TPG_EINVAL, "ngroups must be positive");
  if (groupIds0)
    for (int64_t i = 0; i < n; i++)
      TPG_REQUIRE(groupIds0[i] >= 0 && groupIds0[i] < ngroups, TPG_EINVAL, "groupIds[%lld] = %d out of [0,%d)", (long long)i,
                  groupIds0[i], ngroups);
  return TPG_OK;
}

int tpg_require_diploid(int64_t n, const double* ploidy, const char* what) {
  if (ploidy)
    for (int64_t i = 0; i < n; i++) TPG_REQUIRE(ploidy[i] == 2.0, TPG_EINVAL, "%s only works on diploid data", what);
  return TPG_OK;
}

int make_class_plan(int64_t n, const int32_t* groupIds0, int ngroups, const double* ploidy, ClassPlan* cp) {
  TPG_REQUIRE(ngroups > 0, TPG_EINVAL, "ngroups must be positive");
  cp->has_hap = 0;
  if (ploidy)
    for (int64_t i = 0; i < n; i++) {
      TPG_REQUIRE(ploidy[i] == 1.0 || ploidy[i] == 2.0, TPG_EUNSUPPORTED,
                  "ploidy[%lld] = %g: only diploid (2) and pseudohaploid (1) individuals are supported",
                  (long long)i, ploidy[i]);
      if (ploidy[i] == 1.0) cp->has_hap = 1;
    }
  TPG_TRY(tpg_check_group_ids(n, groupIds0, ngroups));
  cp->nclass = ngroups * (cp->has_hap ? 2 : 1);
  cp->cls.resize((size_t)n);
  cp->group_size.assign((size_t)ngroups, 0);
  for (int64_t i = 0; i < n; i++) {
    const int g = groupIds0 ? groupIds0[i] : 0;
    cp->group_size[(size_t)g]++;
    cp->cls[(size_t)i] = cp->has_hap ? 2 * g + (ploidy[i] == 1.0 ? 1 : 0) : g;
  }
  return TPG_OK;
}

struct GroupVals {
  double alt, valid, het2, nvalid_ind;
};

__device__ __forceinline__ GroupVals tpg_group_vals(const int32_t* __restrict__ cnt, int64_t Mpad, int Cpad,
                                                    int64_t j, int g, int has_hap) {
  GroupVals r;
  const int64_t plane = Mpad * Cpad;
  if (!has_hap) {
    const int64_t o = j * Cpad + g;
    const int n1 = cnt[o], n2 = cnt[plane + o], nv = cnt[2 * plane + o];
// ... 439 lines not shown
```

### tidypopgen_amd/csrc/pack.hip

```cpp
#include <type_traits>

#include "common.h"
#include "devfrag.h"
#include "synth_common.h"

#define TILE 128
#define LDS_STRIDE 132

__device__ __forceinline__ uint8_t tpg_bed_byte(uint8_t packed, int slot) {
  return (uint8_t)((0x00010302u >> (8 * ((packed >> (2 * slot)) & 3))) & 0xFF);
}

__global__ __launch_bounds__(256) void tpg_pack_kernel(const uint8_t* __restrict__ fbm, int64_t nrow, int64_t bed_bpl,
                                                       const int32_t* __restrict__ rows,
                                                       const int32_t* __restrict__ cols, uint8_t* lut_and_flag,
                                                       int64_t n, int64_t m, int64_t Q, int64_t KG,
                                                       uint32_t* __restrict__ T, uint32_t* __restrict__ L) {
  __shared__ __attribute__((aligned(16))) uint8_t smem[256 + TILE * LDS_STRIDE];
  uint8_t* lut = smem;
  uint8_t* codes = smem + 256;
  const int tid = threadIdx.x;
  const int64_t bj = blockIdx.x;
  const int64_t bi = blockIdx.y;
  lut[tid] = lut_and_flag[tid];
  __syncthreads();

  bool bad = false;
  const bool bed_fast = (bed_bpl > 0) && (rows == nullptr) && (bi * TILE + TILE <= n);
  if (bed_fast) {
    const int b = tid & 31;
#pragma unroll 4
    for (int l = tid >> 5; l < TILE; l += 8) {
      const int64_t j = bj * TILE + l;
      uint8_t pk = 0x55;
      if (j < m) {
        const int64_t src_col = cols ? (int64_t)cols[j] - 1 : j;
        pk = fbm[bi * (TILE / 4) + b + src_col * bed_bpl];
      }
#pragma unroll
      for (int q = 0; q < 4; q++) {
        uint8_t c = j < m ? lut[tpg_bed_byte(pk, q)] : (uint8_t)3;
        if (c == 0xFF) { bad = true; c = 3; }
        codes[l * LDS_STRIDE + 4 * b + q] = c;
      }
    }
  } else {
    const int ii = tid & 127;
    const int64_t i = bi * TILE + ii;
    int64_t src_row = -1;
    if (i < n) src_row = rows ? (int64_t)rows[i] - 1 : i;
    for (int l = tid >> 7; l < TILE; l += 2) {
      const int64_t j = bj * TILE + l;
      uint8_t c = 3;
      if (src_row >= 0 && j < m) {
        const int64_t src_col = cols ? (int64_t)cols[j] - 1 : j;
        const uint8_t raw = bed_bpl ? tpg_bed_byte(fbm[(src_row >> 2) + src_col * bed_bpl], (int)(src_row & 3))
                                    : fbm[src_row + src_col * nrow];
        c = lut[raw];
        if (c == 0xFF) { bad = true; c = 3; }
      }
      codes[l * LDS_STRIDE + ii] = c;
    }
  }
  if (bad) atomicOr((unsigned int*)(lut_and_flag + 256), 1u);
  __syncthreads();

#pragma unroll
  for (int it = 0; it < 4; it++) {
    const int idx = tid + 256 * it;
    const int s = idx & 3, lane = (idx >> 2) & 63, tl = idx >> 8;
    const int r = lane & 31, h = lane >> 5;
    {
      const int ind = 32 * tl + r;
      uint32_t w = 0;
#pragma unroll
      for (int e = 0; e < 16; e++) w |= (uint32_t)codes[(32 * s + 16 * h + e) * LDS_STRIDE + ind] << tpg_elem_shift(e);
      const int64_t rt = bi * 4 + tl;
      T[((rt * KG + bj) * 64 + lane) * 4 + s] = w;
    }
    {
      const int loc = 32 * tl + r;
      uint32_t w = 0;
#pragma unroll
      for (int e = 0; e < 16; e++) w |= (uint32_t)codes[loc * LDS_STRIDE + 32 * s + 16 * h + e] << tpg_elem_shift(e);
      const int64_t lt = bj * 4 + tl;
      L[((lt * Q + bi) * 64 + lane) * 4 + s] = w;
    }
  }
}

#ifndef PACK_NSUB
#define PACK_NSUB 2
#endif
__device__ __forceinline__ int64_t tpg_pack_uniform64(int64_t x) {
  const uint32_t lo = __builtin_amdgcn_readfirstlane((uint32_t)x), hi = __builtin_amdgcn_readfirstlane((uint32_t)((uint64_t)x >> 32));
  return (int64_t)(((uint64_t)hi << 32) | lo);
}
typedef uint32_t pk_u4 __attribute__((ext_vector_type(4)));
typedef pk_u4 pk_u4a8 __attribute__((aligned(8)));
template <int NV, bool BED = false>
__global__ __launch_bounds__(256) void tpg_pack_fast_kernel(const uint8_t* __restrict__ fbm, int64_t nrow,
                                                            const int32_t* __restrict__ cols, uint8_t* lut_and_flag,
                                                            int64_t n, int64_t m, int64_t Q, int64_t KG,
                                                            uint32_t* __restrict__ T0, uint32_t* __restrict__ L0,
                                                            uint32_t* __restrict__ T1, uint32_t* __restrict__ L1,
                                                            uint32_t* __restrict__ T4, int xcd_map,
                                                            uint32_t* __restrict__ P0, uint32_t* __restrict__ P1) {
  extern __shared__ __attribute__((aligned(16))) uint8_t smem[];
  bool need_[NV];
  int slot_[NV];
#pragma unroll
  for (int vw = 0; vw < NV; vw++) {
    need_[vw] = vw ? T1 != nullptr : (T0 != nullptr || T4 != nullptr);
    slot_[vw] = vw ? (need_[0] ? 1 : 0) : 0;
  }
  uint8_t* codes_all = smem + NV * (256 + 16);
  const int tid = threadIdx.x;
  constexpr int NSUB = PACK_NSUB;
  const int64_t QB = (Q + NSUB - 1) / NSUB;
  int64_t bj = blockIdx.x / QB;
  int64_t bi0 = (blockIdx.x % QB) * NSUB;
  if (xcd_map) {
    const int64_t k = blockIdx.x >> 3;
    bj = (k / QB) * 8 + (blockIdx.x & 7);
    bi0 = (k % QB) * NSUB;
    if (bj >= KG) return;
  }
#pragma unroll
  for (int vw = 0; vw < NV; vw++) smem[vw * (256 + 16) + tid] = lut_and_flag[vw * (256 + 16) + tid];
  __syncthreads();
  uint32_t lo_[NV], hi_[NV];
  bool bad_[NV];
#pragma unroll
  for (int vw = 0; vw < NV; vw++) {
    lo_[vw] = *reinterpret_cast<const uint32_t*>(smem + vw * (256 + 16));
    hi_[vw] = *reinterpret_cast<const uint32_t*>(smem + vw * (256 + 16) + 4);
    bad_[vw] = false;
  }
  if constexpr (BED) {
#pragma unroll
    for (int vw = 0; vw < NV; vw++) {
      const uint8_t* lut = smem + vw * (256 + 16);
      lo_[vw] = (uint32_t)lut[2] | ((uint32_t)lut[3] << 8) | ((uint32_t)lut[1] << 16) | ((uint32_t)lut[0] << 24);
      hi_[vw] = lo_[vw];
    }
  }
  auto conv = [&](uint32_t w, int vw) -> uint32_t {
    const uint8_t* lut = smem + vw * (256 + 16);
    const uint32_t lo = lo_[vw], hi = hi_[vw];
    bool& bad = bad_[vw];
    uint32_t c;
    if ((w & 0xF8F8F8F8u) == 0) c = __builtin_amdgcn_perm(hi, lo, w);
    else
      c = (uint32_t)lut[w & 0xFF] | ((uint32_t)lut[(w >> 8) & 0xFF] << 8) | ((uint32_t)lut[(w >> 16) & 0xFF] << 16) |
          ((uint32_t)lut[w >> 24] << 24);
    if (c & 0x80808080u) {
      bad = true;
      const uint32_t msk = ((c & 0x80808080u) >> 7) * 0xFFu;
      c = (c & ~msk) | (0x03030303u & msk);
    }
    return c;
  };
  const int c16 = tid & 7;
  uint2 va[NSUB][4], vb[NSUB][4];
#pragma unroll
  for (int sub = 0; sub < NSUB; sub++) {
    const int64_t i0 = (bi0 + sub) * TILE + 16 * c16;
#pragma unroll
    for (int it = 0; it < 4; it++) {
      const int64_t j = bj * TILE + (tid >> 3) + 32 * it;
      va[sub][it] = make_uint2(0, 0);
      vb[sub][it] = make_uint2(0, 0);
      if constexpr (BED) {
        if (j < m && bi0 + sub < Q && i0 < n) {
          const int64_t src_col = cols ? (int64_t)cols[j] - 1 : j;
          const uint8_t* p = fbm + (i0 >> 2) + src_col * nrow;
          typedef uint32_t pk_u1a1 __attribute__((aligned(1)));
          if ((i0 >> 2) + 4 <= nrow) {
            va[sub][it].x = *reinterpret_cast<const pk_u1a1*>(p);
          } else {
            uint32_t w = 0;
            for (int b = 0; (i0 >> 2) + b < nrow; b++) w |= (uint32_t)p[b] << (8 * b);
            va[sub][it].x = w;
          }
        }
      } else if (j < m && bi0 + sub < Q) {
        const int64_t src_col = cols ? (int64_t)cols[j] - 1 : j;
        const uint8_t* p = fbm + i0 + src_col * nrow;
        if (i0 + 16 <= n) {
          const pk_u4 t = *reinterpret_cast<const pk_u4a8*>(p);
          va[sub][it] = make_uint2(t[0], t[1]);
          vb[sub][it] = make_uint2(t[2], t[3]);
        } else if (i0 + 8 <= n) {
          va[sub][it] = *reinterpret_cast<const uint2*>(p);
        }
      }
    }
  }
  uint32_t anyw = 0;
#pragma unroll
  for (int sub = 0; sub < NSUB; sub++)
#pragma unroll
    for (int it = 0; it < 4; it++) anyw |= va[sub][it].x | va[sub][it].y | vb[sub][it].x | vb[sub][it].y;
  const bool fastw = BED || __builtin_amdgcn_ballot_w64((anyw & 0xF8F8F8F8u) != 0) == 0;
  uint32_t cacc[NV];
#pragma unroll
  for (int vw = 0; vw < NV; vw++) cacc[vw] = 0;
  uint32_t cnt3[NV][4];
#pragma unroll
  for (int vw = 0; vw < NV; vw++)
#pragma unroll
    for (int it = 0; it < 4; it++) cnt3[vw][it] = 0;
  const bool cnt_on = P0 != nullptr;
#pragma unroll
  for (int sub = 0; sub < NSUB; sub++) {
  const int64_t bi = bi0 + sub;
  if (bi >= Q) break;
  if (sub) __syncthreads();
  auto phase1 = [&](auto fastc, auto fullc) {
    constexpr bool FAST = decltype(fastc)::value, FULL = decltype(fullc)::value;
    const int64_t i0 = bi * TILE + 16 * c16;
    const int l0 = tid >> 3;
    const uint32_t rot0 = (uint32_t)(16 * c16 + 32 * (l0 >> 4)) & 127u;
    const uint32_t cb[2] = {(uint32_t)l0 * TILE + rot0, (uint32_t)l0 * TILE + (rot0 ^ 64u)};
    const uint32_t loff = (uint32_t)(l0 + 32 * (c16 & 1)) * 16u + (uint32_t)(c16 >> 1) * 4u;
    typedef __attribute__((address_space(1))) char gchar;
    typedef __attribute__((address_space(1))) uint32_t gu32;
#pragma unroll
    for (int it = 0; it < 4; it++) {
      const int l = l0 + 32 * it;
      const bool inside = bj * TILE + l < m;
#pragma unroll
      for (int vw = 0; vw < NV; vw++) {
        uint8_t* codes = codes_all + slot_[vw] * TILE * TILE;
        uint32_t c[4] = {0x03030303u, 0x03030303u, 0x03030303u, 0x03030303u};
        if constexpr (FAST && BED) {
          const uint32_t wb = va[sub][it].x;
#pragma unroll
          for (int q = 0; q < 4; q++) {
            const uint32_t Bq = (wb >> (8 * q)) & 0xFFu, xq = (Bq | (Bq << 12)) & 0x000F000Fu;
            const uint32_t sel = (xq | (xq << 6)) & 0x03030303u;
            uint32_t cq = __builtin_amdgcn_perm(hi_[vw], lo_[vw], sel);
            if constexpr (!FULL) {
              uint32_t keep = 0;
#pragma unroll
              for (int e = 0; e < 4; e++) keep |= (inside && i0 + 4 * q + e < n) ? (0xFFu << (8 * e)) : 0u;
              cq = (cq & keep) | (0x03030303u & ~keep);
            }
            c[q] = cq;
          }
          cacc[vw] |= (c[0] | c[1]) | (c[2] | c[3]);
        } else if constexpr (FAST) {
          const uint32_t w[4] = {va[sub][it].x, va[sub][it].y, vb[sub][it].x, vb[sub][it].y};
          const bool h0 = inside && i0 + 8 <= n, h1 = inside && i0 + 16 <= n;
#pragma unroll
          for (int q = 0; q < 4; q++) {
            const uint32_t cq = __builtin_amdgcn_perm(hi_[vw], lo_[vw], w[q]);
            c[q] = FULL || (q < 2 ? h0 : h1) ? cq : 0x03030303u;
          }
          cacc[vw] |= (c[0] | c[1]) | (c[2] | c[3]);
        } else {
          if (inside && i0 + 8 <= n) { c[0] = conv(va[sub][it].x, vw); c[1] = conv(va[sub][it].y, vw); }
          if (inside && i0 + 16 <= n) { c[2] = conv(vb[sub][it].x, vw); c[3] = conv(vb[sub][it].y, vw); }
        }
        if (need_[vw]) *reinterpret_cast<uint4*>(codes + cb[it & 1] + it * 32 * TILE) = make_uint4(c[0], c[1], c[2], c[3]);
        gchar* Lb = (gchar*)tpg_pack_uniform64((int64_t)((vw ? L1 : L0) + ((bj * 4 + it) * Q + bi) * 256));
        const uint32_t lw = c[0] | (c[1] << 2) | (c[2] << 4) | (c[3] << 6);
        *(gu32*)(Lb + loff) = lw;
        if (cnt_on) {
          uint32_t wc = lw;
          if constexpr (!FULL && BED) {
            uint32_t vm = 0;
#pragma unroll
            for (int k = 0; k < 4; k++)
#pragma unroll
              for (int b = 0; b < 4; b++) vm |= (inside && i0 + 4 * k + b < n) ? (3u << (8 * b + 2 * k)) : 0u;
            wc = lw & vm;
          } else if constexpr (!FULL) wc = (inside && i0 + 16 <= n) ? lw : (inside && i0 + 8 <= n) ? (lw & 0x0F0F0F0Fu) : 0u;
          cnt3[vw][it] += (uint32_t)__popc(wc & 0x55555555u) | ((uint32_t)__popc(wc & 0xAAAAAAAAu) << 10) |
                          ((uint32_t)__popc(wc & (wc >> 1) & 0x55555555u) << 20);
        }
      }
    }
  };
  const bool fullw = __builtin_amdgcn_ballot_w64(!(bj * TILE + (tid >> 3) + 96 < m && bi * TILE + 16 * c16 + 16 <= n)) == 0;
  if (fastw && fullw) phase1(std::true_type{}, std::true_type{});
  else if (fastw) phase1(std::true_type{}, std::false_type{});
  else phase1(std::false_type{}, std::false_type{});
  __syncthreads();
  {
    const int wv = tid >> 6, t = tid & 63;
    const int g = t >> 3, iqq = t & 7;
#pragma unroll
    for (int vw = 0; vw < NV; vw++) {
    const uint8_t* codes = codes_all + slot_[vw] * TILE * TILE;
    uint32_t* T = vw ? T1 : T0;
    uint32_t* T4v = vw ? nullptr : T4;
    if (!T && !T4v) continue;
    uint32_t d[16];
#pragma unroll
    for (int e = 0; e < 16; e++)
      d[e] = *reinterpret_cast<const uint32_t*>(codes + (16 * g + e) * TILE + ((32 * wv + 4 * iqq + 32 * g) & 127));
    const int64_t rt = bi * 4 + wv;
    typedef __attribute__((address_space(1))) char gchar2;
    if (T) {
      uint32_t W[4] = {0, 0, 0, 0};
#pragma unroll
      for (int k = 0; k < 4; k++) {
        const uint32_t x0 = d[4 * k], x1 = d[4 * k + 1], x2 = d[4 * k + 2], x3 = d[4 * k + 3];
        const uint32_t t0 = __builtin_amdgcn_perm(x1, x0, 0x05010400u), t1 = __builtin_amdgcn_perm(x1, x0, 0x07030602u);
        const uint32_t t2 = __builtin_amdgcn_perm(x3, x2, 0x05010400u), t3 = __builtin_amdgcn_perm(x3, x2, 0x07030602u);
        W[0] |= __builtin_amdgcn_perm(t2, t0, 0x05040100u) << (2 * k);
        W[1] |= __builtin_amdgcn_perm(t2, t0, 0x07060302u) << (2 * k);
        W[2] |= __builtin_amdgcn_perm(t3, t1, 0x05040100u) << (2 * k);
        W[3] |= __builtin_amdgcn_perm(t3, t1, 0x07060302u) << (2 * k);
      }
      uint32_t* dst = T + ((rt * KG + bj) * 64 + 4 * iqq + 32 * (g & 1)) * 4 + (g >> 1);
#pragma unroll
      for (int b = 0; b < 4; b++) dst[b * 4] = W[b];
      if (T4v) {
        const int sT = g >> 1;
        uint32_t* dst4 = T4v + (((rt * KG + bj) * 2 + (sT >> 1)) * 64 + 4 * iqq + 32 * (g & 1)) * 4 + 2 * (sT & 1);
#pragma unroll
        for (int b = 0; b < 4; b++) {
          uint32_t lo, hi;
          tpg_t4_words(W[b], rt * 32 + 4 * iqq + b < n ? m - (bj * TILE + 16 * g) : 0, lo, hi);
          *reinterpret_cast<uint2*>(dst4 + b * 4) = make_uint2(lo, hi);
        }
      }
    } else {
      uint32_t N[4][4];
#pragma unroll
      for (int k = 0; k < 4; k++) {
        const uint32_t x0 = d[4 * k], x1 = d[4 * k + 1], x2 = d[4 * k + 2], x3 = d[4 * k + 3];
        const uint32_t t0 = __builtin_amdgcn_perm(x1, x0, 0x05010400u), t1 = __builtin_amdgcn_perm(x1, x0, 0x07030602u);
        const uint32_t t2 = __builtin_amdgcn_perm(x3, x2, 0x05010400u), t3 = __builtin_amdgcn_perm(x3, x2, 0x07030602u);
        N[k][0] = (uint32_t)tpg_lut(TPG_NIB_LUT, __builtin_amdgcn_perm(t2, t0, 0x05040100u));
        N[k][1] = (uint32_t)tpg_lut(TPG_NIB_LUT, __builtin_amdgcn_perm(t2, t0, 0x07060302u));
        N[k][2] = (uint32_t)tpg_lut(TPG_NIB_LUT, __builtin_amdgcn_perm(t3, t1, 0x05040100u));
        N[k][3] = (uint32_t)tpg_lut(TPG_NIB_LUT, __builtin_amdgcn_perm(t3, t1, 0x07060302u));
      }
      if (!(bj * TILE + TILE <= m && bi * TILE + TILE <= n)) {
#pragma unroll
        for (int b = 0; b < 4; b++) {
          const int64_t left = rt * 32 + 4 * iqq + b < n ? m - (bj * TILE + 16 * g) : 0;
#pragma unroll
          for (int k = 0; k < 4; k++) N[k][b] &= tpg_t4_keep(left, k);
        }
      }
      const int sT = g >> 1;
      gchar2* B4 = (gchar2*)tpg_pack_uniform64((int64_t)(T4v + ((rt * KG + bj) * 2) * 256));
      const uint32_t o4 = (uint32_t)(sT >> 1) * 1024u + (uint32_t)(4 * iqq + 32 * (g & 1)) * 16u + (uint32_t)(sT & 1) * 8u;
#pragma unroll
      for (int b = 0; b < 4; b++) {
        typedef uint32_t pk_u2 __attribute__((ext_vector_type(2)));
        typedef __attribute__((address_space(1))) pk_u2 gu2;
        *(gu2*)(B4 + o4 + b * 16) = pk_u2{N[0][b] | (N[1][b] << 4), N[2][b] | (N[3][b] << 4)};
      }
    }
    }
  }
  }
#pragma unroll
  for (int vw = 0; vw < NV; vw++)
    if (bad_[vw] || (cacc[vw] & 0x80808080u)) atomicOr((unsigned int*)(lut_and_flag + vw * (256 + 16) + 256), 1u);
  if (cnt_on) {
    const int64_t Mp = KG * TILE;
#pragma unroll
    for (int vw = 0; vw < NV; vw++) {
      uint32_t* P = vw ? P1 : P0;
#pragma unroll
      for (int it = 0; it < 4; it++) {
        uint32_t pk = cnt3[vw][it];
        pk += (uint32_t)__shfl_xor((int)pk, 1);
        pk += (uint32_t)__shfl_xor((int)pk, 2);
        pk += (uint32_t)__shfl_xor((int)pk, 4);
        if (c16 == 0) P[(bi0 / NSUB) * Mp + bj * TILE + (tid >> 3) + 32 * it] = pk;
      }
    }
  }
}

int tpg_launch_pack(tpg_ctx* ctx, const tpg_fbm* fbm, const int32_t* d_rows, const int32_t* d_cols,
                    const uint8_t* d_lut, tpg_view* v, tpg_view* v2) {
  TPG_REQUIRE(v->KG < 2147483647ll && v->Q <= 65535, TPG_EINVAL, "view too large for the pack grid");
  dim3 grid((unsigned)v->KG, (unsigned)v->Q);
  const bool fast_bytes = fbm->bed_bpl == 0 && (fbm->nrow & 7) == 0 && (((uintptr_t)fbm->d_bytes) & 7) == 0;
  const bool fast_bed = fbm->bed_bpl > 0 && tpg_env_int("TPG_PACK_BED_GENERIC", 0) == 0;
  if ((fast_bytes || fast_bed) && d_rows == nullptr && !tpg_env_set("TPG_PACK_GENERIC")) {
    TPG_REQUIRE((v->KG + 8) * v->Q < 2147483647ll, TPG_EINVAL, "view too large for the pack grid");
    const int xmap = tpg_env_int("TPG_PACK_XCD", 1);
    const dim3 g1((unsigned)((xmap ? (v->KG + 7) / 8 * 8 : v->KG) * ((v->Q + PACK_NSUB - 1) / PACK_NSUB)));
    static const bool counts_on = tpg_env_int("TPG_PACK_COUNTS", 1) != 0;
    const int64_t qb = (v->Q + PACK_NSUB - 1) / PACK_NSUB;
    static_assert(PACK_NSUB * 8 * 16 < 1024, "a 10-bit field holds the counts of a chunk: NSUB x 8 threads x 16 individuals");
    if (counts_on)
      for (tpg_view* w : {v, v2}) {
        if (!w || w->lc_part) continue;
        if (tpg_pmalloc((void**)&w->lc_part, sizeof(uint32_t) * (size_t)qb * (size_t)w->KG * TILE) != hipSuccess) { w->lc_part = nullptr; continue; }
        w->lc_chunks = (int)qb;
        w->lc_row = w->KG * TILE;
      }
    uint32_t* lp0 = v->lc_part && (!v2 || v2->lc_part) ? v->lc_part : nullptr;
    uint32_t* lp1 = lp0 && v2 ? v2->lc_part : nullptr;
    if (!lp0)
      for (tpg_view* w : {v, v2})
        if (w && w->lc_part) { tpg_pfree(w->lc_part); w->lc_part = nullptr; w->lc_chunks = 0; }
    auto lds_bytes = [&](int nv, bool t_a, bool t_b) { return (size_t)nv * (256 + 16) + (size_t)((t_a ? 1 : 0) + (t_b ? 1 : 0)) * TILE * TILE; };
    if (v2 && fast_bed)
      TPG_LAUNCH(ctx, "pack2", (tpg_pack_fast_kernel<2, true>), g1, dim3(256), lds_bytes(2, v->T || v->T4, v2->T != nullptr), fbm->d_bytes, fbm->bed_bpl, d_cols, (uint8_t*)d_lut,
                 v->n, v->m, v->Q, v->KG, (uint32_t*)v->T, (uint32_t*)v->L, (uint32_t*)v2->T, (uint32_t*)v2->L,
                 (uint32_t*)v->T4, xmap, lp0, lp1);
    else if (fast_bed)
      TPG_LAUNCH(ctx, "pack", (tpg_pack_fast_kernel<1, true>), g1, dim3(256), lds_bytes(1, v->T || v->T4, false), fbm->d_bytes, fbm->bed_bpl, d_cols, (uint8_t*)d_lut,
                 v->n, v->m, v->Q, v->KG, (uint32_t*)v->T, (uint32_t*)v->L, (uint32_t*)nullptr, (uint32_t*)nullptr,
                 (uint32_t*)v->T4, xmap, lp0, lp1);
    else if (v2)
      TPG_LAUNCH(ctx, "pack2", tpg_pack_fast_kernel<2>, g1, dim3(256), lds_bytes(2, v->T || v->T4, v2->T != nullptr), fbm->d_bytes, fbm->nrow, d_cols, (uint8_t*)d_lut,
                 v->n, v->m, v->Q, v->KG, (uint32_t*)v->T, (uint32_t*)v->L, (uint32_t*)v2->T, (uint32_t*)v2->L,
                 (uint32_t*)v->T4, xmap, lp0, lp1);
    else
      TPG_LAUNCH(ctx, "pack", tpg_pack_fast_kernel<1>, g1, dim3(256), lds_bytes(1, v->T || v->T4, false), fbm->d_bytes, fbm->nrow, d_cols, (uint8_t*)d_lut,
                 v->n, v->m, v->Q, v->KG, (uint32_t*)v->T, (uint32_t*)v->L, (uint32_t*)nullptr, (uint32_t*)nullptr,
                 (uint32_t*)v->T4, xmap, lp0, lp1);
    TPG_CHECK_LAUNCH();
    return TPG_OK;
  }
  for (tpg_view* w : {v, v2}) {
    if (!w) continue;
    if (!w->T) TPG_HIP(tpg_pmalloc((void**)&w->T, w->bytes_each));
    if (w->T4) { tpg_pfree(w->T4); w->T4 = nullptr; }
  }
  TPG_LAUNCH(ctx, "pack", tpg_pack_kernel, grid, dim3(256), 0, fbm->d_bytes, fbm->nrow, fbm->bed_bpl, d_rows, d_cols,
             (uint8_t*)d_lut, v->n, v->m, v->Q, v->KG, (uint32_t*)v->T, (uint32_t*)v->L);
  if (v2)
    TPG_LAUNCH(ctx, "pack", tpg_pack_kernel, grid, dim3(256), 0, fbm->d_bytes, fbm->nrow, fbm->bed_bpl, d_rows, d_cols,
               (uint8_t*)d_lut + 256 + 16, v2->n, v2->m, v2->Q, v2->KG, (uint32_t*)v2->T, (uint32_t*)v2->L);
  TPG_CHECK_LAUNCH();
  return TPG_OK;
}

__global__ void tpg_unpack_kernel(const uint32_t* __restrict__ T, const uint32_t* __restrict__ L, int from_L,
                                  int64_t n, int64_t m, int64_t Q, int64_t KG, uint8_t* __restrict__ out) {
  const int64_t total = n * m;
  for (int64_t idx = blockIdx.x * (int64_t)blockDim.x + threadIdx.x; idx < total;
       idx += (int64_t)gridDim.x * blockDim.x) {
    const int64_t i = idx % n, j = idx / n;
    uint32_t w;
    int e;
    if (!from_L) {
      const int64_t rt = i >> 5, kg = j >> 7;
      const int r = (int)(i & 31), jj = (int)(j & 127);
      const int s = jj >> 5, h = (jj >> 4) & 1;
      e = jj & 15;
      w = T[((rt * KG + kg) * 64 + (r + 32 * h)) * 4 + s];
    } else {
      const int64_t lt = j >> 5, q = i >> 7;
      const int r = (int)(j & 31), ii = (int)(i & 127);
      const int s = ii >> 5, h = (ii >> 4) & 1;
      e = ii & 15;
      w = L[((lt * Q + q) * 64 + (r + 32 * h)) * 4 + s];
    }
    out[idx] = (uint8_t)((w >> tpg_elem_shift(e)) & 3u);
  }
}

__global__ __launch_bounds__(256) void tpg_l2t_kernel(const uint32_t* __restrict__ L, int64_t Q, int64_t KG,
                                                      uint32_t* __restrict__ T) {
  __shared__ __attribute__((aligned(16))) uint8_t codes[TILE * LDS_STRIDE];
  const int tid = threadIdx.x;
  const int64_t bj = blockIdx.x, bi = blockIdx.y;
#pragma unroll
  for (int it = 0; it < 4; it++) {
    const int idx = tid + 256 * it;
    const int s = idx & 3, lane = (idx >> 2) & 63, tl = idx >> 8;
    const int r = lane & 31, h = lane >> 5;
    const uint32_t w = L[(((bj * 4 + tl) * Q + bi) * 64 + lane) * 4 + s];
#pragma unroll
    for (int e = 0; e < 16; e++) codes[(32 * tl + r) * LDS_STRIDE + 32 * s + 16 * h + e] = (uint8_t)((w >> tpg_elem_shift(e)) & 3u);
  }
  __syncthreads();
#pragma unroll
  for (int it = 0; it < 4; it++) {
    const int idx = tid + 256 * it;
    const int s = idx & 3, lane = (idx >> 2) & 63, tl = idx >> 8;
    const int r = lane & 31, h = lane >> 5;
    const int ind = 32 * tl + r;
    uint32_t w = 0;
#pragma unroll
    for (int e = 0; e < 16; e++) w |= (uint32_t)codes[(32 * s + 16 * h + e) * LDS_STRIDE + ind] << tpg_elem_shift(e);
    T[(((bi * 4 + tl) * KG + bj) * 64 + lane) * 4 + s] = w;
  }
}

int tpg_view_need_T(tpg_ctx* ctx, const tpg_view* v) {
  if (v->T) return TPG_OK;
  TPG_REQUIRE(v->KG < 2147483647ll && v->Q <= 65535, TPG_EINVAL, "view too large for the pack grid");
  uint4* t = nullptr;
  TPG_HIP(tpg_pmalloc((void**)&t, v->bytes_each));
  TPG_LAUNCH(ctx, "l2t", tpg_l2t_kernel, dim3((unsigned)v->KG, (unsigned)v->Q), dim3(256), 0, (const uint32_t*)v->L, v->Q,
             v->KG, (uint32_t*)t);
  v->T = t;
  TPG_CHECK_LAUNCH();
  return TPG_OK;
}

int tpg_launch_unpack(tpg_ctx* ctx, const tpg_view* v, uint8_t* d_codes, int from_L) {
  if (!from_L) TPG_TRY(tpg_view_need_T(ctx, v));
  TPG_LAUNCH(ctx, "unpack", tpg_unpack_kernel, dim3(2048), dim3(256), 0, (const uint32_t*)v->T,
             (const uint32_t*)v->L, from_L, v->n, v->m, v->Q, v->KG, d_codes);
  TPG_CHECK_LAUNCH();
  return TPG_OK;
}

__global__ __launch_bounds__(256) void tpg_synth_kernel(uint8_t* __restrict__ out, uint64_t seed, int64_t nrow,
                                                        int64_t ncol, int64_t j0, int npop, uint32_t miss_thresh,
                                                        int imputed_bytes) {
  __shared__ uint32_t pjg[1024];
  for (int64_t j = blockIdx.x; j < ncol; j += gridDim.x) {
    __syncthreads();
    for (int g = threadIdx.x; g < npop; g += blockDim.x) pjg[g] = tpg_synth_pjg(seed, (uint64_t)(j0 + j), (uint32_t)g, (uint32_t)npop);
    __syncthreads();
    for (int64_t i = threadIdx.x; i < nrow; i += blockDim.x)
      out[i + j * nrow] = tpg_synth_geno(seed, (uint64_t)i, (uint64_t)(j0 + j), pjg[i % npop], miss_thresh, imputed_bytes);
  }
}

int tpg_launch_synth(tpg_ctx* ctx, uint8_t* d_bytes, uint64_t seed, int64_t nrow, int64_t ncol, int64_t j0,
                     int npop, uint32_t miss_thresh, int imputed_bytes) {
  unsigned grid = (unsigned)(ncol < 65536 ? ncol : 65536);
  TPG_LAUNCH(ctx, "synth", tpg_synth_kernel, dim3(grid), dim3(256), 0, d_bytes, seed, nrow, ncol, j0, npop,
             miss_thresh, imputed_bytes);
  TPG_CHECK_LAUNCH();
  return TPG_OK;
}
```

### tidypopgen_amd/csrc/pca.hip

```cpp
#include <math.h>
#include <stdio.h>
#include <stdlib.h>
#include <string.h>
#include <time.h>

#include <algorithm>

#include "common.h"
#include <type_traits>
#include "devfrag.h"

#define MFMA_I8(a, b, c) __builtin_amdgcn_mfma_i32_32x32x32_i8((a), (b), (c), 0, 0, 0)
#define PCA_NAN __longlong_as_double(0x7FF8000000000000ll)

__global__ void tpg_pca_center_scale_kernel(const int4* __restrict__ counts, int64_t m, int64_t n,
                                            double* __restrict__ center, double* __restrict__ scale,
                                            int* __restrict__ flags) {
  for (int64_t j = blockIdx.x * (int64_t)blockDim.x + threadIdx.x; j < m; j += (int64_t)gridDim.x * blockDim.x) {
    const int4 c = counts[j];
    if (c.w != 0) flags[0] = 1;
    const double mean = (double)(c.y + 2 * c.z) / (double)n;
    const double p = mean / 2;
    const double sd = sqrt(2 * p * (1 - p));
    if (!(sd > 0)) flags[1] = 1;
// ... 1381 lines not shown
  TPG_TRY(eig_topk_any(ctx, d_K, (int)n, k, lam.data(), ou.dev<double>(), tol));
  st.mark("eig_topk");
  std::vector<double> dh((size_t)k);
  for (int j = 0; j < k; j++) dh[(size_t)j] = sqrt(lam[(size_t)j] > 0 ? lam[(size_t)j] : 0.0);
  TPG_HIP(tpg_push_small(ctx, d_dk, dh.data(), sizeof(double) * (size_t)k));
  TPG_TRY(pca_loadings_device(ctx, v, oc.dev<double>(), os.dev<double>(), ou.dev<double>(), d_dk, k, ov.dev<double>()));
  if (tpg_is_device_ptr(d)) TPG_HIP(tpg_push_small(ctx, d, dh.data(), sizeof(double) * (size_t)k));
  else memcpy(d, dh.data(), sizeof(double) * (size_t)k);
  TPG_HIP(hipStreamSynchronize(ctx->stream));
  st.mark("loadings");
  TPG_TRY(oc.commit(ctx));
  TPG_TRY(os.commit(ctx));
  TPG_TRY(ou.commit(ctx));
  return ov.commit(ctx);
}

#define LD_TU 6

__global__ void tpg_u_digits_kernel(const double* __restrict__ U, int64_t n, int k, int FU, int64_t Q, int CT,
                                    uint4* __restrict__ UD) {
  const int64_t total = Q * 4 * CT * 64;
  for (int64_t idx = blockIdx.x * (int64_t)blockDim.x + threadIdx.x; idx < total;
       idx += (int64_t)gridDim.x * blockDim.x) {
    const int lane = (int)(idx & 63);
    const int64_t tq = idx >> 6;
    const int ct = (int)(tq % CT);
    const int64_t qs = tq / CT;
    const int s = (int)(qs & 3);
    const int64_t q = qs >> 2;
    const int col = 32 * ct + (lane & 31), h = lane >> 5;
    const int kk = col / LD_TU, t = col % LD_TU;
    uint32_t w[4] = {0, 0, 0, 0};
    if (kk < k)
      for (int e = 0; e < 16; e++) {
        const int64_t i = 128 * q + 32 * s + 16 * h + e;
        if (i >= n) continue;
        long long W = llrint(ldexp(U[i + (int64_t)kk * n], FU));
        long long dig = 0;
        for (int tt = 0; tt <= t; tt++) {
          dig = W & 127;
          if (dig >= 64) dig -= 128;
          W = (W - dig) >> 7;
        }
        w[e >> 2] |= (uint32_t)((int)dig & 0xFF) << (8 * (e & 3));
      }
    UD[idx] = make_uint4(w[0], w[1], w[2], w[3]);
  }
}

__global__ __launch_bounds__(256) void tpg_uq_colsum_kernel(const double* __restrict__ U, int64_t n, int FU,
                                                            double* __restrict__ usum) {
  __shared__ double sh[256];
  const int kk = blockIdx.x;
  double acc = 0;
  for (int64_t i = threadIdx.x; i < n; i += 256) acc += ldexp((double)llrint(ldexp(U[i + (int64_t)kk * n], FU)), -FU);
  sh[threadIdx.x] = acc;
  __syncthreads();
  for (int w = 128; w > 0; w >>= 1) {
    if ((int)threadIdx.x < w) sh[threadIdx.x] += sh[threadIdx.x + w];
    __syncthreads();
  }
  if (threadIdx.x == 0) usum[kk] = sh[0];
}

#ifndef LD_NLT
#define LD_NLT 2
#endif
#ifndef LD_WGS
#define LD_WGS 2
#endif
__device__ __forceinline__ int64_t tpg_uniform64_pca(int64_t x) {
  const uint32_t lo = __builtin_amdgcn_readfirstlane((uint32_t)x), hi = __builtin_amdgcn_readfirstlane((uint32_t)((uint64_t)x >> 32));
  return (int64_t)(((uint64_t)hi << 32) | lo);
}

template <int C, class F>
__device__ __forceinline__ void tpg_pca_static_for(F&& f) {
  if constexpr (C > 0) {
    tpg_pca_static_for<C - 1>(f);
    f(std::integral_constant<int, C - 1>{});
  }
}

template <int CTP>
__global__ __launch_bounds__(256, LD_WGS) void tpg_loadings_mfma_kernel(const uint4* __restrict__ L,
                                                                   const uint4* __restrict__ UD, int64_t n_lt,
                                                                   int64_t Q, int ct0, int CT,
                                                                   int32_t* __restrict__ out, int Cpad) {
  __shared__ __attribute__((aligned(16))) uint4 ubuf[2][4 * CTP][64];
  const int lane = threadIdx.x & 63, wv = threadIdx.x >> 6;
  const int64_t lt0 = ((int64_t)blockIdx.x * 4 + wv) * LD_NLT;
  v16i acc[LD_NLT][CTP];
#pragma unroll
  for (int t = 0; t < LD_NLT; t++)
#pragma unroll
    for (int c = 0; c < CTP; c++)
#pragma unroll
      for (int r = 0; r < 16; r++) acc[t][c][r] = 0;
  const int Qi = (int)Q;
  const int64_t lt0u = tpg_uniform64_pca(lt0);
  const char* pa[LD_NLT];
#pragma unroll
  for (int t = 0; t < LD_NLT; t++) pa[t] = (const char*)(L + ((lt0u + t < n_lt ? lt0u + t : 0) * Q) * 64);
  auto LDG = [&](const char* p, int blk) {
    uint32_t off = (uint32_t)lane * 16u + (uint32_t)blk * 1024u;
    asm("" : "+v"(off));
    return *(const uint4*)(p + off);
  };
  constexpr int LD_D = 4;
  static_assert(LD_D % 2 == 0, "the slot of a group's digit fragments is its parity");
  uint4 AR[LD_D][LD_NLT];
#pragma unroll
  for (int d = 0; d < LD_D - 1; d++)
#pragma unroll
    for (int t = 0; t < LD_NLT; t++) AR[d][t] = LDG(pa[t], d < Qi ? d : Qi - 1);
  const char* pu = (const char*)(UD + ct0 * 64);
  uint4 un[2][CTP];
  auto ufrag = [&](int q, int j) {
    const int it = wv + 4 * j;
    return LDG(pu, (q * 4 + it / CTP) * CT + it % CTP);
  };
#pragma unroll
  for (int j = 0; j < CTP; j++) {
    ubuf[0][wv + 4 * j][lane] = ufrag(0, j);
    un[1][j] = ufrag(Qi > 1 ? 1 : 0, j);
  }
  tpg_lds_barrier();
  auto group = [&](auto Cc, auto Mm, int q) {
    constexpr int C = decltype(Cc)::value, M = decltype(Mm)::value;
    const int qa = q + LD_D - 1 < Qi ? q + LD_D - 1 : Qi - 1, qu = q + 2 < Qi ? q + 2 : Qi - 1;
    const int cur = q & 1;
#pragma unroll
    for (int t = 0; t < LD_NLT; t++) AR[M][t] = LDG(pa[t], qa);
#pragma unroll
    for (int j = 0; j < CTP; j++) un[C & 1][j] = ufrag(qu, j);
#pragma unroll
    for (int s = 0; s < 4; s++) {
      v4i fg[LD_NLT];
#pragma unroll
      for (int t = 0; t < LD_NLT; t++) {
        const uint32_t w = s == 0 ? AR[C][t].x : s == 1 ? AR[C][t].y : s == 2 ? AR[C][t].z : AR[C][t].w;
#pragma unroll
        for (int k = 0; k < 4; k++) fg[t][k] = (int)tpg_codes(w, k);
      }
#pragma unroll
      for (int c = 0; c < CTP; c++) {
        const uint4 bq = ubuf[cur][s * CTP + c][lane];
        v4i fb = {(int)bq.x, (int)bq.y, (int)bq.z, (int)bq.w};
#pragma unroll
        for (int t = 0; t < LD_NLT; t++) acc[t][c] = MFMA_I8(fg[t], fb, acc[t][c]);
      }
    }
#pragma unroll
    for (int j = 0; j < CTP; j++) ubuf[cur ^ 1][wv + 4 * j][lane] = un[(C & 1) ^ 1][j];
    tpg_lds_barrier();
  };
  for (int q = 0; q < Qi; q += LD_D)
    tpg_pca_static_for<LD_D>([&](auto kk) {
      constexpr int k = decltype(kk)::value;
      if (q + k < Qi) group(std::integral_constant<int, k>{}, std::integral_constant<int, (k + LD_D - 1) % LD_D>{}, q + k);
    });
#pragma unroll
  for (int t = 0; t < LD_NLT; t++) {
    if (lt0 + t >= n_lt) break;
#pragma unroll
    for (int c = 0; c < CTP; c++)
#pragma unroll
      for (int r = 0; r < 16; r++) {
        const int64_t row = (lt0 + t) * 32 + tpg_cd_row(r, lane);
        out[row * Cpad + 32 * (ct0 + c) + (lane & 31)] = acc[t][c][r];
      }
  }
}

__global__ void tpg_loadings_finalize_kernel(const int32_t* __restrict__ acc, int Cpad, int64_t m, int k, int FU,
                                             const double* __restrict__ center, const double* __restrict__ scale,
                                             const double* __restrict__ usum, const double* __restrict__ d,
                                             double* __restrict__ vload) {
  const int64_t total = m * k;
  for (int64_t idx = blockIdx.x * (int64_t)blockDim.x + threadIdx.x; idx < total;
       idx += (int64_t)gridDim.x * blockDim.x) {
    const int kk = (int)(idx % k);
    const int64_t j = idx / k;
    long long S = 0;
#pragma unroll
    for (int t = LD_TU - 1; t >= 0; t--) S = S * 128 + (long long)acc[j * Cpad + kk * LD_TU + t];
    const double gu = ldexp((double)S, -FU);
    vload[j + (int64_t)kk * m] = (gu - center[j] * usum[kk]) / (scale[j] * d[kk]);
  }
}

__global__ __launch_bounds__(1024) void tpg_absmax_kernel(const double* __restrict__ x, int64_t total, double* __restrict__ out) {
  __shared__ double sh[1024];
  double mx = 0;
  bool bad = false;
  for (int64_t i = threadIdx.x; i < total; i += 1024) {
    const double a = fabs(x[i]);
    if (a != a) bad = true;
    mx = a > mx ? a : mx;
  }
  sh[threadIdx.x] = bad ? __longlong_as_double(0x7FF8000000000000ll) : mx;
  __syncthreads();
  for (int w = 512; w > 0; w >>= 1) {
    if ((int)threadIdx.x < w) {
      const double a = sh[threadIdx.x], b = sh[threadIdx.x + w];
      sh[threadIdx.x] = (a != a || b != b) ? __longlong_as_double(0x7FF8000000000000ll) : (a > b ? a : b);
    }
    __syncthreads();
  }
  if (threadIdx.x == 0) out[0] = sh[0];
}

static int pca_loadings_device(tpg_ctx* ctx, const tpg_view* v, const double* d_center, const double* d_scale,
                               const double* d_U, const double* d_dk, int k, double* d_V) {
  const int64_t n = v->n, m = v->m;
  double amax = 0;
  {
    DevBuf d_amax;
    TPG_TRY(d_amax.alloc_n<double>(1));
    TPG_LAUNCH(ctx, "loadings_u_digits", tpg_absmax_kernel, dim3(1), dim3(1024), 0, d_U, n * (int64_t)k, d_amax.as<double>());
    TPG_HIP(tpg_fetch_small(ctx, &amax, d_amax.p, sizeof(double)));
  }
  TPG_REQUIRE(amax > 0 && amax == amax && amax < 1e300, TPG_ENUMERIC, "degenerate eigenvectors");
  int ex = 0;
  frexp(amax, &ex);
  const int FU = 7 * LD_TU - 2 - ex;
  const int CT = (int)ceil_div((int64_t)k * LD_TU, 32);
  const int Cpad = CT * 32;
  const int64_t n_lt = v->KG * 4;
  DevBuf b_UD, b_acc, b_usum;
  TPG_TRY(b_UD.alloc((size_t)v->Q * 4 * CT * 1024));
  TPG_TRY(b_acc.alloc_n<int32_t>((size_t)n_lt * 32 * (size_t)Cpad));
  TPG_TRY(b_usum.alloc_n<double>((size_t)k));
  uint4* const d_UD = b_UD.as<uint4>();
  int32_t* const d_acc = b_acc.as<int32_t>();
  double* const d_usum = b_usum.as<double>();
  TPG_LAUNCH(ctx, "loadings_u_digits", tpg_u_digits_kernel, dim3(1024), dim3(256), 0, d_U, n, k, FU, v->Q, CT, d_UD);
  TPG_LAUNCH(ctx, "loadings_u_digits", tpg_uq_colsum_kernel, dim3((unsigned)k), dim3(256), 0, d_U, n, FU, d_usum);
  const unsigned grid = (unsigned)ceil_div(n_lt, 4 * LD_NLT);
  for (int ct0 = 0; ct0 < CT;) {
    const int left = CT - ct0;
#define LD_LAUNCH(C)                                                                                             \
  TPG_LAUNCH(ctx, "loadings_mfma", tpg_loadings_mfma_kernel<C>, dim3(grid), dim3(256), 0, (const uint4*)v->L,     \
             (const uint4*)d_UD, n_lt, v->Q, ct0, CT, d_acc, Cpad)
    if (left >= 4) { LD_LAUNCH(4); ct0 += 4; }
    else if (left == 3) { LD_LAUNCH(3); ct0 += 3; }
    else if (left == 2) { LD_LAUNCH(2); ct0 += 2; }
    else { LD_LAUNCH(1); ct0 += 1; }
#undef LD_LAUNCH
  }
  TPG_LAUNCH(ctx, "loadings_finalize", tpg_loadings_finalize_kernel, dim3(2048), dim3(256), 0, (const int32_t*)d_acc,
             Cpad, m, k, FU, d_center, d_scale, (const double*)d_usum, d_dk, d_V);
  TPG_CHECK_LAUNCH();
  TPG_HIP(hipStreamSynchronize(ctx->stream));
  return TPG_OK;
}

int tpg_sym_eig_topk_tol(tpg_ctx* ctx, const double* d_K, int64_t n, int k, double tol, double* lambda_host, double* d_U) {
  TPG_REQUIRE(ctx && d_K && lambda_host && d_U, TPG_EINVAL, "null argument");
  TPG_REQUIRE(n > 0 && k >= 1 && k <= n, TPG_EINVAL, "bad n = %lld / k = %d", (long long)n, k);
  return eig_topk_any(ctx, d_K, (int)n, k, lambda_host, d_U, tol);
}

extern "C" int tpg_sym_eig_topk(tpg_ctx* ctx, const double* K, int64_t n, int k, double* lambda, double* U) {
  TpgEnter _enter(ctx);
  TPG_REQUIRE(ctx && K && lambda && U, TPG_EINVAL, "null argument");
  TPG_REQUIRE(n > 0 && k >= 1 && k <= n, TPG_EINVAL, "bad n = %lld / k = %d", (long long)n, k);
  InBuf ik;
  TPG_TRY(ik.init(ctx, K, sizeof(double) * (size_t)n * (size_t)n));
  OutBuf ou;
  TPG_TRY(ou.init(U, sizeof(double) * (size_t)n * (size_t)k));
  std::vector<double> lam((size_t)k);
  TPG_TRY(eig_topk_any(ctx, ik.dev<double>(), (int)n, k, lam.data(), ou.dev<double>(), 1e-12));
  if (tpg_is_device_ptr(lambda)) TPG_HIP(hipMemcpyAsync(lambda, lam.data(), sizeof(double) * (size_t)k, hipMemcpyHostToDevice, ctx->stream));
  else memcpy(lambda, lam.data(), sizeof(double) * (size_t)k);
  TPG_HIP(hipStreamSynchronize(ctx->stream));
  return ou.commit(ctx);
}

extern "C" int tpg_pca_loadings(tpg_ctx* ctx, const tpg_view* v, const double* center, const double* scale,
                                const double* U, const double* d, int k, double* vload) {
  TpgEnter _enter(ctx);
  TPG_REQUIRE(ctx && v && center && scale && U && d && vload, TPG_EINVAL, "null argument");
  TPG_REQUIRE(k >= 1, TPG_EINVAL, "k must be positive");
  const int64_t n = v->n, m = v->m;
  InBuf ic, is, iu, id;
  TPG_TRY(ic.init(ctx, center, sizeof(double) * (size_t)m));
  TPG_TRY(is.init(ctx, scale, sizeof(double) * (size_t)m));
  TPG_TRY(iu.init(ctx, U, sizeof(double) * (size_t)n * (size_t)k));
  TPG_TRY(id.init(ctx, d, sizeof(double) * (size_t)k));
  OutBuf ov;
  TPG_TRY(ov.init(vload, sizeof(double) * (size_t)m * (size_t)k));
  DevBuf d_counts, d_flag;
  TPG_TRY(d_counts.alloc_n<int32_t>(4 * (size_t)m));
  TPG_TRY(d_flag.alloc_n<int>(2));
  int flag[2] = {0, 1};
  TPG_TRY(tpg_launch_loci_counts(ctx, v, d_counts.as<int32_t>()));
  TPG_HIP(hipMemsetAsync(d_flag.p, 0, 2 * sizeof(int), ctx->stream));
  TPG_LAUNCH(ctx, "pca_center_check", tpg_center_is_mean_kernel, dim3(1024), dim3(256), 0, (const int4*)d_counts.p,
             ic.dev<double>(), m, n, d_flag.as<int>());
  TPG_HIP(tpg_fetch_small(ctx, flag, d_flag.p, 2 * sizeof(int)));
  d_counts.free();
  d_flag.free();
  if (!flag[1]) {
    TPG_TRY(pca_loadings_device(ctx, v, ic.dev<double>(), is.dev<double>(), iu.dev<double>(), id.dev<double>(), k,
                                ov.dev<double>()));
  } else {
    DevBuf d_inv;
    TPG_TRY(d_inv.alloc_n<double>((size_t)m));
    TPG_LAUNCH(ctx, "inv_scale", tpg_inv_kernel, dim3(1024), dim3(256), 0, is.dev<double>(), m, d_inv.as<double>());
    TPG_TRY(run_sweep(ctx, SW_ROWSCALE, v->L, v->KG * 4, v->Q, m, n, ic.dev<double>(), d_inv.as<double>(), iu.dev<double>(), n, k,
                      ov.dev<double>(), id.dev<double>(), nullptr));
  }
  return ov.commit(ctx);
}
```

### tidypopgen_amd/csrc/runtime.hip

```cpp
#include <ctype.h>
#include <fcntl.h>
#include <math.h>
#include <sched.h>
#include <stdarg.h>
#include <stdio.h>
#include <string.h>
#include <sys/mman.h>
#include <sys/stat.h>
#include <unistd.h>

#include "common.h"
#include "host/host_bedpack.h"
#include "host/host_nibpack.h"

#include <mutex>
#include <thread>
#include <unordered_map>

static thread_local char g_err[1024] = "";

struct Pool {
  std::multimap<size_t, void*> free_blocks;
  size_t cached_bytes = 0;
  int device = 0;
// ... 1023 lines not shown
extern "C" int tpg_fbm_alloc_bed(tpg_ctx* ctx, int64_t n, int64_t m, tpg_fbm** out) {
  TpgEnter _enter(ctx);
  TPG_REQUIRE(ctx && out, TPG_EINVAL, "null argument");
  TPG_REQUIRE(n > 0 && m > 0, TPG_EINVAL, "empty .bed (%lld x %lld)", (long long)n, (long long)m);
  tpg_fbm* f = new tpg_fbm{ctx, nullptr, n, m};
  f->bed_bpl = (n + 3) / 4;
  hipError_t e = hipMalloc((void**)&f->d_bytes, (size_t)f->bed_bpl * (size_t)m);
  if (e != hipSuccess) { delete f; tpg_set_error("hipMalloc failed: %s", hipGetErrorString(e)); return TPG_EHIP; }
  *out = f;
  return TPG_OK;
}

extern "C" int tpg_fbm_upload_bed_snps(tpg_ctx* ctx, tpg_fbm* fbm, const uint8_t* host_snps, int64_t snp0, int64_t nsnps) {
  TpgEnter _enter(ctx);
  TPG_REQUIRE(ctx && fbm && host_snps, TPG_EINVAL, "null argument");
  TPG_REQUIRE(fbm->bed_bpl > 0, TPG_EUNSUPPORTED, "not a .bed store (tpg_fbm_upload_cols fills a byte FBM)");
  TPG_REQUIRE(snp0 >= 0 && nsnps >= 0 && snp0 + nsnps <= fbm->ncol, TPG_EINVAL, "SNPs [%lld, %lld) outside the store",
              (long long)snp0, (long long)(snp0 + nsnps));
  const size_t sz = (size_t)nsnps * (size_t)fbm->bed_bpl;
  uint8_t* dst = fbm->d_bytes + (size_t)snp0 * (size_t)fbm->bed_bpl;
  TPG_HIP(sz >= XFER_BIG ? tpg_upload_pinned(ctx, dst, host_snps, sz) : tpg_upload(ctx, dst, host_snps, sz));
  return TPG_OK;
}

extern "C" int tpg_fbm_open_bed(tpg_ctx* ctx, const char* path, int64_t n, int64_t m, tpg_fbm** out) {
  TpgEnter _enter(ctx);
  TPG_REQUIRE(ctx && path && out, TPG_EINVAL, "null argument");
  TPG_REQUIRE(n > 0 && m > 0, TPG_EINVAL, "empty .bed (%lld x %lld)", (long long)n, (long long)m);
  int fd = open(path, O_RDONLY);
  TPG_REQUIRE(fd >= 0, TPG_EINVAL, "cannot open %s", path);
  const size_t sz = 3 + (size_t)((n + 3) / 4) * (size_t)m;
  struct stat st;
  if (fstat(fd, &st) != 0 || (size_t)st.st_size < sz) {
    close(fd);
    tpg_set_error("%s is smaller than a %lld x %lld .bed", path, (long long)n, (long long)m);
    return TPG_EINVAL;
  }
  void* p = mmap(nullptr, sz, PROT_READ, MAP_PRIVATE, fd, 0);
  close(fd);
  TPG_REQUIRE(p != MAP_FAILED, TPG_EINVAL, "mmap of %s failed", path);
  const uint8_t* b = (const uint8_t*)p;
  int rc;
  if (b[0] != 0x6C || b[1] != 0x1B || b[2] != 0x01) {
    tpg_set_error("%s is not a SNP-major PLINK .bed (magic %02x %02x %02x)", path, b[0], b[1], b[2]);
    rc = TPG_EINVAL;
  } else {
    rc = tpg_fbm_from_bed_host(ctx, b + 3, n, m, out);
  }
  munmap(p, sz);
  return rc;
}

extern "C" int tpg_fbm_to_host(tpg_ctx* ctx, const tpg_fbm* fbm, uint8_t* bytes) {
  TpgEnter _enter(ctx);
  TPG_REQUIRE(ctx && fbm && bytes, TPG_EINVAL, "null argument");
  TPG_REQUIRE(fbm->bed_bpl == 0, TPG_EUNSUPPORTED, "a .bed store has no FBM bytes; unpack a view instead");
  TPG_HIP(hipMemcpyAsync(bytes, fbm->d_bytes, (size_t)fbm->nrow * (size_t)fbm->ncol, hipMemcpyDeviceToHost, ctx->stream));
  TPG_HIP(hipStreamSynchronize(ctx->stream));
  return TPG_OK;
}

extern "C" void tpg_fbm_free(tpg_fbm* fbm) {
  if (!fbm) return;
  if (fbm->d_bytes) {
    if (fbm->pooled) tpg_pfree(fbm->d_bytes);
    else (void)hipFree(fbm->d_bytes);
  }
  delete fbm;
}

static void make_lut(const double* code256, uint8_t* lut) {
  for (int b = 0; b < 256; b++) {
    if (!code256) { lut[b] = b < 3 ? (uint8_t)b : 3; continue; }
    double x = code256[b];
    if (!(x > -1)) lut[b] = 3;
    else if (x == 0.0) lut[b] = 0;
    else if (x == 1.0) lut[b] = 1;
    else if (x == 2.0) lut[b] = 2;
    else lut[b] = 0xFF;
  }
}

static int view_create_impl(tpg_ctx* ctx, const tpg_fbm* fbm, const int32_t* rowInd1, int64_t n, const int32_t* colInd1,
                            int64_t m, const double* code256_a, const double* code256_b, bool two, tpg_view** out_a,
                            tpg_view** out_b) {
  TPG_REQUIRE(ctx && fbm && out_a && (!two || out_b), TPG_EINVAL, "null argument");
  if (!rowInd1) n = fbm->nrow;
  if (!colInd1) m = fbm->ncol;
  TPG_REQUIRE(n > 0 && m > 0, TPG_EINVAL, "empty view (%lld x %lld)", (long long)n, (long long)m);
  TPG_REQUIRE(n < (1ll << 24), TPG_EINVAL, "n = %lld too large", (long long)n);
  if (rowInd1)
    for (int64_t i = 0; i < n; i++)
      TPG_REQUIRE(rowInd1[i] >= 1 && rowInd1[i] <= fbm->nrow, TPG_EINVAL, "rowInd[%lld] = %d out of [1,%lld]",
                  (long long)i, rowInd1[i], (long long)fbm->nrow);
  if (colInd1)
    for (int64_t j = 0; j < m; j++)
      TPG_REQUIRE(colInd1[j] >= 1 && colInd1[j] <= fbm->ncol, TPG_EINVAL, "colInd[%lld] = %d out of [1,%lld]",
                  (long long)j, colInd1[j], (long long)fbm->ncol);
  const int nv = two ? 2 : 1;
  uint8_t lut[2 * (256 + 16)];
  memset(lut, 0, sizeof(lut));
  make_lut(code256_a, lut);
  if (two) make_lut(code256_b, lut + 256 + 16);
  ViewPtr v[2];
  DevBuf d_rows, d_cols, d_lut;
  for (int k = 0; k < nv; k++) {
    v[k].reset(new tpg_view(ctx, n, m));
    if (!two && code256_a) TPG_HIP(tpg_pmalloc((void**)&v[k]->T, v[k]->bytes_each));
    else if (k == 0) TPG_HIP(tpg_pmalloc((void**)&v[k]->T4, 2 * v[k]->bytes_each));
    TPG_HIP(tpg_pmalloc((void**)&v[k]->L, v[k]->bytes_each));
  }
  TPG_TRY(d_lut.alloc(sizeof(lut)));
  TPG_HIP(tpg_h2d_async(ctx, d_lut.p, lut, (size_t)nv * (256 + 16)));
  if (rowInd1) {
    TPG_TRY(d_rows.alloc_n<int32_t>((size_t)n));
    TPG_HIP(tpg_h2d_async(ctx, d_rows.p, rowInd1, sizeof(int32_t) * (size_t)n));
  }
  if (colInd1) {
    TPG_TRY(d_cols.alloc_n<int32_t>((size_t)m));
    TPG_HIP(tpg_h2d_async(ctx, d_cols.p, colInd1, sizeof(int32_t) * (size_t)m));
  }
  TPG_TRY(tpg_launch_pack(ctx, fbm, d_rows.as<int32_t>(), d_cols.as<int32_t>(), d_lut.as<uint8_t>(), v[0].get(), v[1].get()));
  uint8_t back[2 * (256 + 16)];
  TPG_HIP(tpg_fetch_small(ctx, back, d_lut.p, (size_t)nv * (256 + 16)));
  for (int k = 0; k < nv; k++) {
    int32_t bad;
    memcpy(&bad, back + k * (256 + 16) + 256, sizeof(bad));
    TPG_REQUIRE(!bad, TPG_EUNSUPPORTED,
                "code256 maps an occurring FBM byte to a value outside {0,1,2,NA}; the 2-bit device path cannot represent it");
  }
  *out_a = v[0].release();
  if (two) *out_b = v[1].release();
  return TPG_OK;
}

extern "C" int tpg_view_create(tpg_ctx* ctx, const tpg_fbm* fbm, const int32_t* rowInd1, int64_t n,
                               const int32_t* colInd1, int64_t m, const double* code256, tpg_view** out) {
  TpgEnter _enter(ctx);
  return view_create_impl(ctx, fbm, rowInd1, n, colInd1, m, code256, nullptr, false, out, nullptr);
}

extern "C" int tpg_view_create_pair(tpg_ctx* ctx, const tpg_fbm* fbm, const int32_t* rowInd1, int64_t n,
                                    const int32_t* colInd1, int64_t m, const double* code256_a, const double* code256_b,
                                    tpg_view** out_a, tpg_view** out_b) {
  TpgEnter _enter(ctx);
  return view_create_impl(ctx, fbm, rowInd1, n, colInd1, m, code256_a, code256_b, true, out_a, out_b);
}

tpg_view::~tpg_view() {
  drop_derived();
  if (L && !L_borrowed) tpg_pfree(L);
}
void tpg_view::drop_derived() {
  if (T) tpg_pfree(T);
  if (T4) tpg_pfree(T4);
  if (lc_part) tpg_pfree(lc_part);
  T = T4 = nullptr;
  lc_part = nullptr;
  lc_chunks = 0;
  gc_buf.free();
  gc_cache = GroupedCounts();
  gc_cls.clear();
}
extern "C" void tpg_view_free(tpg_view* v) { delete v; }
extern "C" int64_t tpg_view_n(const tpg_view* v) { return v ? v->n : 0; }
extern "C" int64_t tpg_view_m(const tpg_view* v) { return v ? v->m : 0; }

extern "C" int tpg_view_unpack(tpg_ctx* ctx, const tpg_view* v, uint8_t* codes) {
  TpgEnter _enter(ctx);
  TPG_REQUIRE(ctx && v && codes, TPG_EINVAL, "null argument");
  OutBuf o;
  TPG_TRY(o.init(codes, (size_t)v->n * (size_t)v->m));
  TPG_TRY(tpg_launch_unpack(ctx, v, o.dev<uint8_t>(), 0));
  DevBuf d2;
  TPG_TRY(d2.alloc((size_t)v->n * (size_t)v->m));
  TPG_TRY(tpg_launch_unpack(ctx, v, d2.as<uint8_t>(), 1));
  std::vector<uint8_t> a((size_t)v->n * (size_t)v->m), b((size_t)v->n * (size_t)v->m);
  TPG_HIP(hipMemcpyAsync(a.data(), o.dev<uint8_t>(), a.size(), hipMemcpyDeviceToHost, ctx->stream));
  TPG_HIP(hipMemcpyAsync(b.data(), d2.p, b.size(), hipMemcpyDeviceToHost, ctx->stream));
  TPG_HIP(hipStreamSynchronize(ctx->stream));
  TPG_REQUIRE(a == b, TPG_EHIP, "internal error: T and L layouts of the view disagree");
  return o.commit(ctx);
}
```

### tidypopgen_amd/csrc/stream.hip

```cpp
#include <fcntl.h>
#include <math.h>
#include <stdio.h>
#include <string.h>
#include <sys/mman.h>
#include <sys/stat.h>
#include <unistd.h>

#include <atomic>
#include <chrono>
#include <condition_variable>
#include <deque>
#include <memory>
#include <mutex>
#include <thread>

#include "common.h"

namespace {

enum SrcKind { SRC_BYTES = 0, SRC_BED = 1, SRC_SYNTH = 2 };

struct StreamSource {
  SrcKind kind = SRC_BYTES;
  const uint8_t* bytes = nullptr;
// ... 377 lines not shown
      }
      hipError_t e = hipSuccess;
      if (t.ready) e = hipStreamWaitEvent(down_ctx->stream, t.ready, 0);
      stamp("    download starts, MB:", (long long)(t.width * t.height >> 20));
      if (e == hipSuccess) e = tpg_download_rows(down_ctx, t.dst, t.dpitch, t.src, t.width, t.height);
      stamp("    download done");
      if (e != hipSuccess) {
        char buf[160];
        snprintf(buf, sizeof(buf), "download of a block's results failed: %s", hipGetErrorString(e));
        sh.fail(TPG_EHIP, buf);
        return;
      }
      {
        std::lock_guard<std::mutex> lk(sh.mu);
        bytes_down += t.width * t.height;
        if (t.slot >= 0) out[t.slot].pending--;
      }
      sh.cv.notify_all();
    }
  }
  void start_downloader() {
    if (down_running) return;
    down_stop = false;
    down_th = std::thread([this] { downloader(); });
    down_running = true;
  }
  int join_downloader() {
    if (!down_running) return TPG_OK;
    {
      std::lock_guard<std::mutex> lk(sh.mu);
      down_stop = true;
    }
    sh.cv.notify_all();
    down_th.join();
    down_running = false;
    if (sh.failed) { tpg_set_error("%s", sh.msg.c_str()); return sh.code; }
    return TPG_OK;
  }
  int wait_slot(int slot) {
    std::unique_lock<std::mutex> lk(sh.mu);
    sh.cv.wait(lk, [&] { return sh.failed || out[slot].pending == 0; });
    if (sh.failed) { tpg_set_error("%s", sh.msg.c_str()); return sh.code; }
    return TPG_OK;
  }

  int rows_out(void* dst, size_t elem, int64_t rows_total, int64_t q, const void* d_src, int64_t mb, int64_t ncols, hipEvent_t ev,
               int slot) {
    if (!dst || mb <= 0 || ncols <= 0) return TPG_OK;
    uint8_t* to = (uint8_t*)dst + elem * (size_t)q;
    if (tpg_is_device_ptr(dst)) {
      TPG_HIP(hipMemcpy2DAsync(to, elem * (size_t)rows_total, d_src, elem * (size_t)mb, elem * (size_t)mb, (size_t)ncols,
                               hipMemcpyDeviceToDevice, ctx->stream));
      return TPG_OK;
    }
    start_downloader();
    DownTask t;
    t.ready = ev;
    t.src = d_src;
    t.dst = to;
    t.width = elem * (size_t)mb;
    t.height = (size_t)ncols;
    t.dpitch = elem * (size_t)rows_total;
    t.slot = slot;
    {
      std::lock_guard<std::mutex> lk(sh.mu);
      if (slot >= 0) out[slot].pending++;
      down_q.push_back(t);
    }
    sh.cv.notify_all();
    return TPG_OK;
  }

  void sample() {
    const size_t u = device_used();
    if (u > peak_used) peak_used = u;
  }

  int make_views(const tpg_fbm* f, int slot, ViewPtr* v ) {
    const tpg_stream_job* j = job;
    tpg_view* p[3] = {nullptr, nullptr, nullptr};
    int rc;
    const int a = 0, b = ntab == 2 ? 1 : (view_of_pca >= 0 ? view_of_pca : 2);
    if (ntab == 1) rc = tpg_view_create(ctx, f, j->rowInd1, n, nullptr, 0, block_table(slot, tab[0]), &p[0]);
    else rc = tpg_view_create_pair(ctx, f, j->rowInd1, n, nullptr, 0, tab[a], tab[b], &p[a], &p[b]);
    if (rc == TPG_OK && ntab == 3) rc = tpg_view_create(ctx, f, j->rowInd1, n, nullptr, 0, tab[3 - a - b], &p[3 - a - b]);
    for (int t = 0; t < 3; t++) v[t].reset(p[t]);
    return rc;
  }

  int alloc_common() {
    const size_t unit = src->unit();
    const int64_t bmax = std::min<int64_t>(B, P1 - P0);
    for (int k = 0; k < 2 && k < nblocks; k++) TPG_TRY(d_blk[k].alloc((size_t)bmax * unit));
    for (int k = 0; k < 2; k++) {
      if (!out[k].ev) TPG_HIP(hipEventCreateWithFlags(&out[k].ev, hipEventDisableTiming));
      if (!out[k].ev2) TPG_HIP(hipEventCreateWithFlags(&out[k].ev2, hipEventDisableTiming));
    }
    for (int k = 0; k < 4; k++)
      if (!ev_fin[k]) TPG_HIP(hipEventCreateWithFlags(&ev_fin[k], hipEventDisableTiming));
    return TPG_OK;
  }

  int sweep1() {
    const tpg_stream_job* j = job;
    TpgEnter _enter(ctx);
    t_start = now();
    base_used = device_used();
    peak_used = base_used;
    TPG_TRY(alloc_common());
    const int G = j->ngroups, P = j->P;
    const int64_t bmax = std::min<int64_t>(B, P1 - P0);
    if (want_pw) {
      if (comm) TPG_TRY(tpg_pairwise_create_sharded(ctx, comm, n, &pw));
      else TPG_TRY(tpg_pairwise_create(ctx, n, nullptr, &pw));
    }
    if (want_fst) {
      TPG_TRY(d_fsum.alloc(sizeof(double) * 2 * (size_t)P * (size_t)j->nfst));
      TPG_TRY(d_fpart.alloc(sizeof(double) * 2 * (size_t)P));
      TPG_HIP(hipMemsetAsync(d_fsum.p, 0, sizeof(double) * 2 * (size_t)P * (size_t)j->nfst, ctx->stream));
    }
    if (want_pca) {
      TPG_TRY(d_K.alloc(sizeof(double) * (size_t)n * (size_t)n));
      have_K = false;
      fro = 0.0;
      saved_fbits = ctx->pca_digit_fbits;
      if (budget) ctx->pca_digit_fbits = 30;
      big_views = budget == 0 && keep_views && nblocks > 1;
      batch_gram = big_views && nblocks > 2 && src->kind != SRC_BYTES && tpg_env_int("TPG_STREAM_GRAM_BATCH", 1) != 0;
      gram_from = 0;
      if (big_views) {
        const size_t per128 = (size_t)ceil_div(n, 128) * 4096;
        TPG_TRY(bigL.alloc((size_t)ceil_div(P1 - P0, 128) * per128));
        TPG_TRY(big_c.alloc(8 * (size_t)(P1 - P0)));
        TPG_TRY(big_s.alloc(8 * (size_t)(P1 - P0)));
      }
    }
    for (int s = 0; s < 2 && s < nblocks; s++) {
      OutSlot& o = out[s];
      if (j->alt_freq) TPG_TRY(o.af.alloc(16 * (size_t)bmax));
      if (j->grouped_alt_freq) TPG_TRY(o.gaf.alloc(16 * (size_t)G * (size_t)bmax));
      if (j->grouped_missingness) TPG_TRY(o.gm.alloc(8 * (size_t)G * (size_t)bmax));
      if (j->loci_counts) TPG_TRY(o.lc.alloc(16 * (size_t)bmax));
      for (int i = 0; i < j->nfst; i++)
        if (j->fst_by_locus[i]) {
          TPG_TRY(o.fl[i].alloc(8 * (size_t)P * (size_t)bmax));
          if (j->fst_return_num_dem) TPG_TRY(o.fd[i].alloc(8 * (size_t)P * (size_t)bmax));
        }
      if (want_pca) {
        TPG_TRY(o.dc.alloc(8 * (size_t)bmax));
        TPG_TRY(o.ds.alloc(8 * (size_t)bmax));
      }
    }
    if (nblocks == 0) return TPG_OK;
    if (ntab == 1) set_bedpack(tab[0]);
    TPG_TRY(start_uploader());
    std::vector<double> tot_scratch((size_t)(P > 0 ? P : 1));
    for (int64_t b = 0; b < nblocks; b++) {
      int64_t q0, q1;
      block_range(b, &q0, &q1);
      const int64_t mb = q1 - q0;
      const int slot = (int)(b & 1);
      stamp("wait for block", b);
      TPG_TRY(wait_block(b));
      stamp("got block", b);
      const tpg_fbm f = block_fbm(slot, mb);
      ViewPtr v[3];
      TPG_TRY(make_views(&f, slot, v));
      release_block(b);
      stamp("packed", b);
      OutSlot& o = out[slot];
      TPG_TRY(wait_slot(slot));
      stamp("output slot free", b);
      if (want_loc || want_fst) {
        const tpg_view* vl = v[view_of_loc].get();
        if (j->alt_freq) TPG_TRY(tpg_alt_freq_dip_pseudo(ctx, vl, j->ploidy, j->as_counts, o.af.as<double>()));
        if (j->grouped_alt_freq)
          TPG_TRY(tpg_grouped_alt_freq_dip_pseudo(ctx, vl, j->groupIds0, G, j->ploidy, j->as_counts, o.gaf.as<double>()));
        if (j->grouped_missingness) TPG_TRY(tpg_grouped_missingness(ctx, vl, j->groupIds0, G, o.gm.as<double>()));
        if (j->loci_counts) TPG_TRY(tpg_loci_counts(ctx, vl, o.lc.as<int32_t>()));
        for (int i = 0; i < j->nfst; i++) {
          if (j->fst_tot[i]) {
            TPG_TRY(tpg_pairwise_pop_fst_sums(ctx, vl, j->groupIds0, G, j->ploidy, j->fst_method[i], j->pairs1, P, d_fpart.as<double>(),
                                              d_fpart.as<double>() + P));
            hipLaunchKernelGGL(tpg_stream_add_kernel, dim3(8), dim3(256), 0, ctx->stream, d_fsum.as<double>() + 2 * (size_t)P * (size_t)i,
                               (const double*)d_fpart.as<double>(), (int64_t)2 * P);
            TPG_CHECK_LAUNCH();
          }
          if (j->fst_by_locus[i])
            TPG_TRY(tpg_pairwise_pop_fst(ctx, vl, j->groupIds0, G, j->ploidy, j->fst_method[i], j->pairs1, P, 1, j->fst_return_num_dem ? 1 : 0,
                                         tot_scratch.data(), o.fl[i].as<double>(), j->fst_return_num_dem ? o.fd[i].as<double>() : nullptr));
        }
        TPG_HIP(hipEventRecord(o.ev, ctx->stream));
        TPG_TRY(rows_out(j->alt_freq, 8, m, q0, o.af.p, mb, 2, o.ev, slot));
        TPG_TRY(rows_out(j->grouped_alt_freq, 8, m, q0, o.gaf.p, mb, 2 * (int64_t)G, o.ev, slot));
        TPG_TRY(rows_out(j->grouped_missingness, 8, m, q0, o.gm.p, mb, G, o.ev, slot));
        if (j->loci_counts) TPG_TRY(rows_out(j->loci_counts, 16, 1, q0, o.lc.p, mb, 1, o.ev, slot));
        for (int i = 0; i < j->nfst; i++) {
          TPG_TRY(rows_out(j->fst_by_locus[i], 8, m, q0, o.fl[i].p, mb, P, o.ev, slot));
          if (j->fst_return_num_dem && j->fst_by_locus[i]) TPG_TRY(rows_out(j->fst_by_locus_den[i], 8, m, q0, o.fd[i].p, mb, P, o.ev, slot));
        }
      }
      stamp("per-locus enqueued", b);
      if (want_pw) TPG_TRY(tpg_pairwise_accumulate_products(ctx, pw, v[view_of_pw].get(), 0, -1, products));
      if (want_pca) {
        tpg_view* vp = v[view_of_pca].get();
        ViewPtr imp;
        if (impute) {
          TPG_TRY(tpg_view_impute_at(ctx, vp, impute, j->impute_seed, q0, &vp, nullptr));
          imp.reset(vp);
        }
        double *dc = o.dc.as<double>(), *ds = o.ds.as<double>();
        Kept* kp = nullptr;
        if (keep_views) {
          kept.emplace_back();
          kp = &kept.back();
          kp->q0 = q0;
          kp->mb = mb;
          TPG_TRY(kp->dc.alloc(8 * (size_t)mb));
          TPG_TRY(kp->ds.alloc(8 * (size_t)mb));
          dc = kp->dc.as<double>();
          ds = kp->ds.as<double>();
        }
        TPG_TRY(tpg_pca_center_scale(ctx, vp, dc, ds));
        if (!batch_gram) {
          if (!have_K) TPG_TRY(tpg_pca_gram(ctx, vp, dc, ds, d_K.as<double>()));
          else TPG_TRY(tpg_pca_gram_add(ctx, vp, dc, ds, d_K.as<double>()));
          have_K = true;
        }
        if (j->square_frobenius) {
          double fb = 0;
          TPG_TRY(tpg_square_frobenius(ctx, vp, dc, ds, &fb));
          fro += fb;
        }
        hipEvent_t ev = o.ev2;
        TPG_HIP(hipEventRecord(ev, ctx->stream));
        TPG_TRY(rows_out(j->center, 8, m, q0, dc, mb, 1, ev, keep_views ? -1 : slot));
        TPG_TRY(rows_out(j->scale, 8, m, q0, ds, mb, 1, ev, keep_views ? -1 : slot));
        if (kp) {
          kp->v = std::move(imp ? imp : v[view_of_pca]);
          kp->v->drop_derived();
        }
        if (big_views) {
          const size_t per128 = (size_t)ceil_div(n, 128) * 4096;
          uint8_t* at = bigL.as<uint8_t>() + (size_t)((q0 - P0) / 128) * per128;
          TPG_HIP(tpg_copy_dev(ctx, at, kp->v->L, (size_t)kp->v->KG * per128));
          TPG_HIP(tpg_copy_dev(ctx, big_c.as<double>() + (q0 - P0), dc, 8 * (size_t)mb));
          TPG_HIP(tpg_copy_dev(ctx, big_s.as<double>() + (q0 - P0), ds, 8 * (size_t)mb));
          tpg_pfree(kp->v->L);
          kp->v->L = (uint4*)at;
          kp->v->L_borrowed = true;
          if (batch_gram && b == nblocks - 1) {
            const tpg_view bv(ctx, n, (q1 - P0) - gram_from, (uint4*)(bigL.as<uint8_t>() + (size_t)(gram_from / 128) * per128));
            const double *bc = big_c.as<double>() + gram_from, *bs = big_s.as<double>() + gram_from;
            if (!have_K) TPG_TRY(tpg_pca_gram(ctx, &bv, bc, bs, d_K.as<double>()));
            else TPG_TRY(tpg_pca_gram_add(ctx, &bv, bc, bs, d_K.as<double>()));
            have_K = true;
            gram_from = q1 - P0;
            stamp("gram batch enqueued", b);
          }
        }
      }
      sample();
    }
    up_th.join();
    if (sh.failed) { tpg_set_error("%s", sh.msg.c_str()); return sh.code; }
    t_sweep1 = now() - t_start;
    stamp("first sweep enqueued");
    return TPG_OK;
  }

  int setup_qc() {
    const tpg_stream_qc_job* c = qc;
    TPG_REQUIRE(c->loci_counts || c->hwe_p || c->grouped_counts || c->grouped_hwe_p || c->indiv_counts, TPG_EINVAL,
                "the job asks for nothing");
    TPG_REQUIRE(c->midp == 0 || c->midp == 1, TPG_EINVAL, "midp must be 0 or 1");
    if (c->grouped_counts || c->grouped_hwe_p) {
      TPG_REQUIRE(c->groupIds0 && c->ngroups >= 1, TPG_EINVAL, "grouped outputs need groupIds and ngroups");
      TPG_TRY(tpg_check_group_ids(n, c->groupIds0, c->ngroups));
    }
    TPG_REQUIRE(!c->indiv_counts || m < (1ll << 31), TPG_EUNSUPPORTED, "per-individual counts of 2^31 loci or more do not fit int32");
    want_loc = true;
    code_loc = c->code256;
    tab[0] = c->code256;
    ntab = 1;
    view_of_loc = 0;
    return TPG_OK;
  }

  int sweep_qc() {
    const tpg_stream_qc_job* c = qc;
    TpgEnter _enter(ctx);
    t_start = now();
    base_used = device_used();
    peak_used = base_used;
    TPG_TRY(alloc_common());
    const int G = c->ngroups;
    const int64_t bmax = std::min<int64_t>(B, P1 - P0);
    if (c->indiv_counts) {
      TPG_TRY(d_icnt.alloc(16 * (size_t)n));
      TPG_HIP(hipMemsetAsync(d_icnt.p, 0, 16 * (size_t)n, ctx->stream));
    }
    for (int s = 0; s < 2 && s < nblocks; s++) {
      OutSlot& o = out[s];
      if (c->loci_counts) TPG_TRY(o.lc.alloc(16 * (size_t)bmax));
      if (c->hwe_p) TPG_TRY(o.hw.alloc(8 * (size_t)bmax));
      if (c->grouped_counts) TPG_TRY(o.gcn.alloc(12 * (size_t)G * (size_t)bmax));
      if (c->grouped_hwe_p) TPG_TRY(o.ghw.alloc(8 * (size_t)G * (size_t)bmax));
    }
    set_bedpack(tab[0]);
    TPG_TRY(start_uploader());
    for (int64_t b = 0; b < nblocks; b++) {
      int64_t q0, q1;
      block_range(b, &q0, &q1);
      const int64_t mb = q1 - q0;
      const int slot = (int)(b & 1);
      stamp("wait for block", b);
      TPG_TRY(wait_block(b));
      const tpg_fbm f = block_fbm(slot, mb);
      ViewPtr v[3];
      TPG_TRY(make_views(&f, slot, v));
      release_block(b);
      stamp("packed", b);
      OutSlot& o = out[slot];
      TPG_TRY(wait_slot(slot));
      const tpg_view* vl = v[0].get();
      if (c->loci_counts) TPG_TRY(tpg_loci_counts(ctx, vl, o.lc.as<int32_t>()));
      if (c->hwe_p) TPG_TRY(tpg_loci_hwe(ctx, vl, c->midp, o.hw.as<double>()));
// ... 532 lines not shown
```

Baseline: 135.6 billion.

## Pack the second view directly in locus-major layout and convert lazily

The pack kernel gains a mode that writes the second view straight into a locus-major (LM) layout, using shuffles to transpose within registers. The Gram-by-classes path and the loadings MFMA kernel read LM directly, which removes the separate l2lm conversion kernel and its scratch buffer. Consumers that need the tiled L layout call a new lazy lm2l conversion. The streaming path keeps the old layout. This adds kernel complexity and may cost extra conversions when L-dependent stages run on an LM-only view.

Measured after the change: 136.7 billion, median of 6. About the same (+0.8%).

```diff
diff --git a/tidypopgen_amd/csrc/admix.hip b/tidypopgen_amd/csrc/admix.hip
--- a/tidypopgen_amd/csrc/admix.hip
+++ b/tidypopgen_amd/csrc/admix.hip
@@ -289,6 +289,7 @@
     TPG_TRY(sc.get(&trace, (size_t)trace_len));
     TPG_TRY(sc.get(&flag, (size_t)1));
     if (need_f_next) TPG_TRY(sc.get(&F[1], (size_t)m * KT));
+    TPG_TRY(tpg_view_need_L(ctx, v));
     if (need_q_sweep) {
       TPG_TRY(tpg_view_need_T(ctx, v));
       TPG_TRY(sc.get(&Q[1], (size_t)n * KT));
diff --git a/tidypopgen_amd/csrc/common.h b/tidypopgen_amd/csrc/common.h
--- a/tidypopgen_amd/csrc/common.h
+++ b/tidypopgen_amd/csrc/common.h
@@ -153,7 +153,8 @@
   int64_t n, m;
   int64_t Q, KG;
   mutable uint4* T = nullptr;
-  uint4* L;
+  mutable uint4* L;
+  uint4* LM = nullptr;
   bool L_borrowed = false;
   size_t bytes_each;
   mutable uint4* T4 = nullptr;
@@ -290,9 +291,13 @@
                          const size_t* rcnt, const size_t* roff);
 
 int tpg_launch_pack(tpg_ctx* ctx, const tpg_fbm* fbm, const int32_t* d_rows, const int32_t* d_cols,
-                    const uint8_t* d_lut, tpg_view* v, tpg_view* v2);
+                    const uint8_t* d_lut, tpg_view* v, tpg_view* v2, bool v2_locus_major);
+int tpg_view_create_pair_as(tpg_ctx* ctx, const tpg_fbm* fbm, const int32_t* rowInd1, int64_t n, const int32_t* colInd1, int64_t m,
+                            const double* code256_a, const double* code256_b, bool second_locus_major, tpg_view** out_a,
+                            tpg_view** out_b);
 int tpg_launch_unpack(tpg_ctx* ctx, const tpg_view* v, uint8_t* d_codes, int from_L);
 int tpg_view_need_T(tpg_ctx* ctx, const tpg_view* v);
+int tpg_view_need_L(tpg_ctx* ctx, const tpg_view* v);
 int tpg_view_impute_at(tpg_ctx* ctx, const tpg_view* raw, int method, uint64_t seed, int64_t col0, tpg_view** out,
                        tpg_impute_report* rep);
 int tpg_launch_synth(tpg_ctx* ctx, uint8_t* d_bytes, uint64_t seed, int64_t nrow, int64_t ncol, int64_t j0,
diff --git a/tidypopgen_amd/csrc/gramcls.hip b/tidypopgen_amd/csrc/gramcls.hip
--- a/tidypopgen_amd/csrc/gramcls.hip
+++ b/tidypopgen_amd/csrc/gramcls.hip
@@ -746,6 +746,10 @@
   *done = false;
   if (tpg_env_set("TPG_GRAM_DIGITS")) return TPG_OK;
   const int64_t n_lt = 4 * v->KG;
+  if (v->LM) {
+    const GclsSrc src{(const uint4*)v->LM, 0, 2 * v->Q, 0, 0, 2, 1};
+    return gram_classes_core(ctx, v->n, v->Q, v->m, src, d_w, d_what, d_K, false, done, centred_ok);
+  }
   DevBuf d_LM;
   TPG_TRY(d_LM.alloc_n<uint4>((size_t)n_lt * 32 * (size_t)v->Q * 2));
   TPG_LAUNCH(ctx, "gcls_l2lm", tpg_gcls_l2lm_kernel, dim3((unsigned)std::min<int64_t>(n_lt * ((v->Q + 3) / 4), (int64_t)ctx->num_cu * 32)),
@@ -886,6 +890,7 @@
     TPG_HIP(hipMemcpyAsync(per_dest.data(), d_perdest, sizeof(int32_t) * (size_t)R, hipMemcpyDeviceToHost, ctx->stream));
     TPG_HIP(hipStreamSynchronize(ctx->stream));
     TPG_TRY(B.get(&d_send, (size_t)std::max<int64_t>(m, 1) * (size_t)recq));
+    TPG_TRY(tpg_view_need_L(ctx, v));
     if (m > 0)
       TPG_LAUNCH(ctx, "gclx_pack", tpg_gclx_pack_kernel, dim3((unsigned)std::min<int64_t>(ceil_div(m, 4), (int64_t)ctx->num_cu * 16)),
                  dim3(256), 0, (const uint4*)v->L, Q, (const uint32_t*)d_idx2, d_scale, m, d_send);
diff --git a/tidypopgen_amd/csrc/impute.hip b/tidypopgen_amd/csrc/impute.hip
--- a/tidypopgen_amd/csrc/impute.hip
+++ b/tidypopgen_amd/csrc/impute.hip
@@ -331,7 +331,7 @@
                        tpg_impute_report* rep) {
   TPG_REQUIRE(ctx && raw && out, TPG_EINVAL, "null argument");
   TPG_TRY(check_method(method));
-  TPG_REQUIRE(raw->L, TPG_EINVAL, "the view has no locus-tiled layout");
+  TPG_TRY(tpg_view_need_L(ctx, raw));
   ViewPtr v(new tpg_view(ctx, raw->n, raw->m));
   DevBuf d_rep;
   TPG_HIP(tpg_pmalloc((void**)&v->L, v->bytes_each));
diff --git a/tidypopgen_amd/csrc/ld.hip b/tidypopgen_amd/csrc/ld.hip
--- a/tidypopgen_amd/csrc/ld.hip
+++ b/tidypopgen_amd/csrc/ld.hip
@@ -363,6 +363,7 @@
 int ld_launch_band(tpg_ctx* ctx, const tpg_view* v, double thr_r2, const LdBand& B, uint32_t* d_bits, int64_t stride,
                    uint32_t* d_back, int64_t bstride) {
   const int64_t m = v->m;
+  TPG_TRY(tpg_view_need_L(ctx, v));
   if (stride > 0) TPG_HIP(hipMemsetAsync(d_bits, 0, sizeof(uint32_t) * (size_t)m * (size_t)stride, ctx->stream));
   if (d_back) TPG_HIP(hipMemsetAsync(d_back, 0, sizeof(uint32_t) * (size_t)m * (size_t)bstride, ctx->stream));
   TPG_LAUNCH(ctx, "ld_band", tpg_ld_band_kernel, dim3((unsigned)ceil_div(m, 32)), dim3(256), 0, (const uint4*)v->L, v->Q, v->n,
diff --git a/tidypopgen_amd/csrc/loci.hip b/tidypopgen_amd/csrc/loci.hip
--- a/tidypopgen_amd/csrc/loci.hip
+++ b/tidypopgen_amd/csrc/loci.hip
@@ -63,6 +63,7 @@
     TPG_CHECK_LAUNCH();
     return TPG_OK;
   }
+  TPG_TRY(tpg_view_need_L(ctx, v));
   const int64_t n_lt = v->KG * 4;
   TPG_LAUNCH(ctx, "loci_counts", tpg_loci_counts_kernel, dim3((unsigned)ceil_div(n_lt, 4)), dim3(256), 0,
              (const uint4*)v->L, n_lt, v->Q, v->n, v->m, (int4*)d_counts);
@@ -183,6 +184,7 @@
   const int64_t gy = ceil_div(n_lt, tiles);
   TPG_REQUIRE(gy <= 65535 && gx <= 0x7FFFFFFF, TPG_EUNSUPPORTED, "per-individual counts of a view of %lld x %lld", (long long)v->n,
               (long long)v->m);
+  TPG_TRY(tpg_view_need_L(ctx, v));
   TPG_LAUNCH(ctx, "indiv_accumulate", tpg_indiv_accumulate_kernel, dim3((unsigned)gx, (unsigned)gy), dim3(256), 0,
              (const uint4*)v->L, n_lt, v->Q, v->n, v->m, (int)tiles, d_acc);
   TPG_CHECK_LAUNCH();
@@ -414,6 +416,7 @@
   const int64_t n_lt = v->KG * 4, Mpad = n_lt * 32;
   const int Cpad = GT * 32;
   gc = GroupedCounts();
+  TPG_TRY(tpg_view_need_L(ctx, v));
   TPG_TRY(v->gc_buf.alloc_n<int32_t>(3 * (size_t)Mpad * (size_t)Cpad));
   int32_t* cnt = v->gc_buf.as<int32_t>();
   std::vector<int32_t> h_up((size_t)v->n + (size_t)GT * 32, 0);
diff --git a/tidypopgen_amd/csrc/pack.hip b/tidypopgen_amd/csrc/pack.hip
--- a/tidypopgen_amd/csrc/pack.hip
+++ b/tidypopgen_amd/csrc/pack.hip
@@ -1,3 +1,4 @@
+#include <algorithm>
 #include <type_traits>
 
 #include "common.h"
@@ -98,14 +99,15 @@
 }
 typedef uint32_t pk_u4 __attribute__((ext_vector_type(4)));
 typedef pk_u4 pk_u4a8 __attribute__((aligned(8)));
-template <int NV, bool BED = false>
+template <int NV, bool BED = false, bool LMV = false>
 __global__ __launch_bounds__(256) void tpg_pack_fast_kernel(const uint8_t* __restrict__ fbm, int64_t nrow,
                                                             const int32_t* __restrict__ cols, uint8_t* lut_and_flag,
                                                             int64_t n, int64_t m, int64_t Q, int64_t KG,
                                                             uint32_t* __restrict__ T0, uint32_t* __restrict__ L0,
                                                             uint32_t* __restrict__ T1, uint32_t* __restrict__ L1,
                                                             uint32_t* __restrict__ T4, int xcd_map,
-                                                            uint32_t* __restrict__ P0, uint32_t* __restrict__ P1) {
+                                                            uint32_t* __restrict__ P0, uint32_t* __restrict__ P1,
+                                                            uint32_t* __restrict__ LM1) {
   extern __shared__ __attribute__((aligned(16))) uint8_t smem[];
   bool need_[NV];
   int slot_[NV];
@@ -212,6 +214,9 @@
 #pragma unroll
     for (int it = 0; it < 4; it++) cnt3[vw][it] = 0;
   const bool cnt_on = P0 != nullptr;
+  uint32_t lmw[4 * NSUB];
+#pragma unroll
+  for (int k = 0; k < 4 * NSUB; k++) lmw[k] = 0;
 #pragma unroll
   for (int sub = 0; sub < NSUB; sub++) {
   const int64_t bi = bi0 + sub;
@@ -264,9 +269,13 @@
           if (inside && i0 + 16 <= n) { c[2] = conv(vb[sub][it].x, vw); c[3] = conv(vb[sub][it].y, vw); }
         }
         if (need_[vw]) *reinterpret_cast<uint4*>(codes + cb[it & 1] + it * 32 * TILE) = make_uint4(c[0], c[1], c[2], c[3]);
-        gchar* Lb = (gchar*)tpg_pack_uniform64((int64_t)((vw ? L1 : L0) + ((bj * 4 + it) * Q + bi) * 256));
         const uint32_t lw = c[0] | (c[1] << 2) | (c[2] << 4) | (c[3] << 6);
-        *(gu32*)(Lb + loff) = lw;
+        if (LMV && vw == 1) {
+          lmw[it * NSUB + sub] = lw;
+        } else {
+          gchar* Lb = (gchar*)tpg_pack_uniform64((int64_t)((vw ? L1 : L0) + ((bj * 4 + it) * Q + bi) * 256));
+          *(gu32*)(Lb + loff) = lw;
+        }
         if (cnt_on) {
           uint32_t wc = lw;
           if constexpr (!FULL && BED) {
@@ -361,6 +370,45 @@
     }
   }
   }
+  if constexpr (LMV) {
+    static_assert(NV == 2, "the locus-major layout is the second view's");
+    typedef __attribute__((address_space(1))) char gchar;
+    const int l0 = tid >> 3, h = c16 & 1, s = c16 >> 1;
+    const uint32_t row = (uint32_t)l0 * (uint32_t)Q * 32u + (uint32_t)h * 16u;
+    if constexpr (NSUB == 2) {
+      typedef __attribute__((address_space(1))) pk_u4 gu4;
+      const bool has1 = bi0 + 1 < Q;
+#pragma unroll
+      for (int half = 0; half < 2; half++) {
+        uint32_t x[4] = {lmw[4 * half], lmw[4 * half + 1], lmw[4 * half + 2], lmw[4 * half + 3]};
+#pragma unroll
+        for (int b = 0; b < 2; b++) {
+          const bool up = (s >> b) & 1;
+#pragma unroll
+          for (int k = 0; k < 4; k++) {
+            if ((k >> b) & 1) continue;
+            const int k2 = k | (1 << b);
+            const uint32_t got = (uint32_t)__shfl_xor((int)(up ? x[k] : x[k2]), 2 << b);
+            if (up) x[k] = got;
+            else x[k2] = got;
+          }
+        }
+        gchar* Mb = (gchar*)tpg_pack_uniform64((int64_t)(LM1 + (bj * 4 + 2 * half) * Q * 256 + bi0 * 8));
+        const uint32_t off = (uint32_t)(s >> 1) * (uint32_t)Q * 1024u + row + (uint32_t)(s & 1) * 32u;
+        if (has1 || !(s & 1)) *(gu4*)(Mb + off) = pk_u4{x[0], x[1], x[2], x[3]};
+      }
+    } else {
+      typedef __attribute__((address_space(1))) uint32_t gu32;
+#pragma unroll
+      for (int it = 0; it < 4; it++)
+#pragma unroll
+        for (int sub = 0; sub < NSUB; sub++) {
+          if (bi0 + sub >= Q) break;
+          gchar* Mb = (gchar*)tpg_pack_uniform64((int64_t)(LM1 + (bj * 4 + it) * Q * 256 + (bi0 + sub) * 8));
+          *(gu32*)(Mb + row + (uint32_t)s * 4u) = lmw[it * NSUB + sub];
+        }
+    }
+  }
 #pragma unroll
   for (int vw = 0; vw < NV; vw++)
     if (bad_[vw] || (cacc[vw] & 0x80808080u)) atomicOr((unsigned int*)(lut_and_flag + vw * (256 + 16) + 256), 1u);
@@ -381,13 +429,24 @@
   }
 }
 
+static bool tpg_pack_fast_bed(const tpg_fbm* fbm) { return fbm->bed_bpl > 0 && tpg_env_int("TPG_PACK_BED_GENERIC", 0) == 0; }
+static bool tpg_pack_takes_fast_route(const tpg_fbm* fbm, const int32_t* d_rows) {
+  const bool fast_bytes = fbm->bed_bpl == 0 && (fbm->nrow & 7) == 0 && (((uintptr_t)fbm->d_bytes) & 7) == 0;
+  return (fast_bytes || tpg_pack_fast_bed(fbm)) && d_rows == nullptr && !tpg_env_set("TPG_PACK_GENERIC");
+}
+
 int tpg_launch_pack(tpg_ctx* ctx, const tpg_fbm* fbm, const int32_t* d_rows, const int32_t* d_cols,
-                    const uint8_t* d_lut, tpg_view* v, tpg_view* v2) {
+                    const uint8_t* d_lut, tpg_view* v, tpg_view* v2, bool v2_locus_major) {
   TPG_REQUIRE(v->KG < 2147483647ll && v->Q <= 65535, TPG_EINVAL, "view too large for the pack grid");
   dim3 grid((unsigned)v->KG, (unsigned)v->Q);
-  const bool fast_bytes = fbm->bed_bpl == 0 && (fbm->nrow & 7) == 0 && (((uintptr_t)fbm->d_bytes) & 7) == 0;
-  const bool fast_bed = fbm->bed_bpl > 0 && tpg_env_int("TPG_PACK_BED_GENERIC", 0) == 0;
-  if ((fast_bytes || fast_bed) && d_rows == nullptr && !tpg_env_set("TPG_PACK_GENERIC")) {
+  const bool fast_route = tpg_pack_takes_fast_route(fbm, d_rows);
+  if (v2 && !v2->L && !v2->LM) {
+    if (v2_locus_major && fast_route) TPG_HIP(tpg_pmalloc((void**)&v2->LM, v2->bytes_each));
+    else TPG_HIP(tpg_pmalloc((void**)&v2->L, v2->bytes_each));
+  }
+  TPG_REQUIRE(v->L, TPG_EINVAL, "the view has no locus-tiled layout");
+  const bool fast_bed = tpg_pack_fast_bed(fbm);
+  if (fast_route) {
     TPG_REQUIRE((v->KG + 8) * v->Q < 2147483647ll, TPG_EINVAL, "view too large for the pack grid");
     const int xmap = tpg_env_int("TPG_PACK_XCD", 1);
     const dim3 g1((unsigned)((xmap ? (v->KG + 7) / 8 * 8 : v->KG) * ((v->Q + PACK_NSUB - 1) / PACK_NSUB)));
@@ -407,22 +466,29 @@
       for (tpg_view* w : {v, v2})
         if (w && w->lc_part) { tpg_pfree(w->lc_part); w->lc_part = nullptr; w->lc_chunks = 0; }
     auto lds_bytes = [&](int nv, bool t_a, bool t_b) { return (size_t)nv * (256 + 16) + (size_t)((t_a ? 1 : 0) + (t_b ? 1 : 0)) * TILE * TILE; };
-    if (v2 && fast_bed)
+#define PACK2_LM(BED_)                                                     \
+  TPG_LAUNCH(ctx, "pack2", (tpg_pack_fast_kernel<2, BED_, true>), g1, dim3(256), lds_bytes(2, v->T || v->T4, v2->T != nullptr), fbm->d_bytes, \
+             BED_ ? fbm->bed_bpl : fbm->nrow, d_cols, (uint8_t*)d_lut, v->n, v->m, v->Q, v->KG, (uint32_t*)v->T, (uint32_t*)v->L,        \
+             (uint32_t*)v2->T, (uint32_t*)nullptr, (uint32_t*)v->T4, xmap, lp0, lp1, (uint32_t*)v2->LM)
+    if (v2 && v2->LM && fast_bed) PACK2_LM(true);
+    else if (v2 && v2->LM) PACK2_LM(false);
+#undef PACK2_LM
+    else if (v2 && fast_bed)
       TPG_LAUNCH(ctx, "pack2", (tpg_pack_fast_kernel<2, true>), g1, dim3(256), lds_bytes(2, v->T || v->T4, v2->T != nullptr), fbm->d_bytes, fbm->bed_bpl, d_cols, (uint8_t*)d_lut,
                  v->n, v->m, v->Q, v->KG, (uint32_t*)v->T, (uint32_t*)v->L, (uint32_t*)v2->T, (uint32_t*)v2->L,
-                 (uint32_t*)v->T4, xmap, lp0, lp1);
+                 (uint32_t*)v->T4, xmap, lp0, lp1, (uint32_t*)nullptr);
     else if (fast_bed)
       TPG_LAUNCH(ctx, "pack", (tpg_pack_fast_kernel<1, true>), g1, dim3(256), lds_bytes(1, v->T || v->T4, false), fbm->d_bytes, fbm->bed_bpl, d_cols, (uint8_t*)d_lut,
                  v->n, v->m, v->Q, v->KG, (uint32_t*)v->T, (uint32_t*)v->L, (uint32_t*)nullptr, (uint32_t*)nullptr,
-                 (uint32_t*)v->T4, xmap, lp0, lp1);
+                 (uint32_t*)v->T4, xmap, lp0, lp1, (uint32_t*)nullptr);
     else if (v2)
       TPG_LAUNCH(ctx, "pack2", tpg_pack_fast_kernel<2>, g1, dim3(256), lds_bytes(2, v->T || v->T4, v2->T != nullptr), fbm->d_bytes, fbm->nrow, d_cols, (uint8_t*)d_lut,
                  v->n, v->m, v->Q, v->KG, (uint32_t*)v->T, (uint32_t*)v->L, (uint32_t*)v2->T, (uint32_t*)v2->L,
-                 (uint32_t*)v->T4, xmap, lp0, lp1);
+                 (uint32_t*)v->T4, xmap, lp0, lp1, (uint32_t*)nullptr);
     else
       TPG_LAUNCH(ctx, "pack", tpg_pack_fast_kernel<1>, g1, dim3(256), lds_bytes(1, v->T || v->T4, false), fbm->d_bytes, fbm->nrow, d_cols, (uint8_t*)d_lut,
                  v->n, v->m, v->Q, v->KG, (uint32_t*)v->T, (uint32_t*)v->L, (uint32_t*)nullptr, (uint32_t*)nullptr,
-                 (uint32_t*)v->T4, xmap, lp0, lp1);
+                 (uint32_t*)v->T4, xmap, lp0, lp1, (uint32_t*)nullptr);
     TPG_CHECK_LAUNCH();
     return TPG_OK;
   }
@@ -493,8 +559,36 @@
   }
 }
 
+__global__ __launch_bounds__(256) void tpg_lm2l_kernel(const uint4* __restrict__ LM, int64_t Q, int64_t n_lt, uint4* __restrict__ L) {
+  __shared__ uint4 sh[32][8];
+  const int64_t QG = (Q + 3) / 4;
+  const int lane = threadIdx.x & 63, wv = threadIdx.x >> 6;
+  for (int64_t task = blockIdx.x; task < n_lt * QG; task += gridDim.x) {
+    const int64_t lt = task / QG, q0 = (task % QG) * 4;
+    const int r = threadIdx.x >> 3, p = threadIdx.x & 7;
+    if (q0 + (p >> 1) < Q) sh[r][p] = LM[((lt * 32 + r) * Q + q0) * 2 + p];
+    __syncthreads();
+    if (q0 + wv < Q) L[(lt * Q + q0 + wv) * 64 + lane] = sh[lane & 31][2 * wv + (lane >> 5)];
+    __syncthreads();
+  }
+}
+
+int tpg_view_need_L(tpg_ctx* ctx, const tpg_view* v) {
+  if (v->L) return TPG_OK;
+  TPG_REQUIRE(v->LM, TPG_EINVAL, "the view has no locus-tiled layout");
+  const int64_t n_lt = 4 * v->KG;
+  uint4* l = nullptr;
+  TPG_HIP(tpg_pmalloc((void**)&l, v->bytes_each));
+  TPG_LAUNCH(ctx, "lm2l", tpg_lm2l_kernel, dim3((unsigned)std::min<int64_t>(n_lt * ((v->Q + 3) / 4), (int64_t)ctx->num_cu * 32)), dim3(256),
+             0, (const uint4*)v->LM, v->Q, n_lt, l);
+  v->L = l;
+  TPG_CHECK_LAUNCH();
+  return TPG_OK;
+}
+
 int tpg_view_need_T(tpg_ctx* ctx, const tpg_view* v) {
   if (v->T) return TPG_OK;
+  TPG_TRY(tpg_view_need_L(ctx, v));
   TPG_REQUIRE(v->KG < 2147483647ll && v->Q <= 65535, TPG_EINVAL, "view too large for the pack grid");
   uint4* t = nullptr;
   TPG_HIP(tpg_pmalloc((void**)&t, v->bytes_each));
@@ -507,6 +601,7 @@
 
 int tpg_launch_unpack(tpg_ctx* ctx, const tpg_view* v, uint8_t* d_codes, int from_L) {
   if (!from_L) TPG_TRY(tpg_view_need_T(ctx, v));
+  else TPG_TRY(tpg_view_need_L(ctx, v));
   TPG_LAUNCH(ctx, "unpack", tpg_unpack_kernel, dim3(2048), dim3(256), 0, (const uint32_t*)v->T,
              (const uint32_t*)v->L, from_L, v->n, v->m, v->Q, v->KG, d_codes);
   TPG_CHECK_LAUNCH();
diff --git a/tidypopgen_amd/csrc/pca.hip b/tidypopgen_amd/csrc/pca.hip
--- a/tidypopgen_amd/csrc/pca.hip
+++ b/tidypopgen_amd/csrc/pca.hip
@@ -1487,7 +1487,7 @@
   }
 }
 
-template <int CTP>
+template <int CTP, bool LM>
 __global__ __launch_bounds__(256, LD_WGS) void tpg_loadings_mfma_kernel(const uint4* __restrict__ L,
                                                                    const uint4* __restrict__ UD, int64_t n_lt,
                                                                    int64_t Q, int ct0, int CT,
@@ -1512,13 +1512,23 @@
     asm("" : "+v"(off));
     return *(const uint4*)(p + off);
   };
+  const uint32_t lm_lane = ((uint32_t)(lane & 31) * 2u * (uint32_t)Qi + (uint32_t)(lane >> 5)) * 16u;
+  auto LDA = [&](const char* p, int blk) {
+    if constexpr (!LM) {
+      return LDG(p, blk);
+    } else {
+      uint32_t off = lm_lane + (uint32_t)blk * 32u;
+      asm("" : "+v"(off));
+      return *(const uint4*)(p + off);
+    }
+  };
   constexpr int LD_D = 4;
   static_assert(LD_D % 2 == 0, "the slot of a group's digit fragments is its parity");
   uint4 AR[LD_D][LD_NLT];
 #pragma unroll
   for (int d = 0; d < LD_D - 1; d++)
 #pragma unroll
-    for (int t = 0; t < LD_NLT; t++) AR[d][t] = LDG(pa[t], d < Qi ? d : Qi - 1);
+    for (int t = 0; t < LD_NLT; t++) AR[d][t] = LDA(pa[t], d < Qi ? d : Qi - 1);
   const char* pu = (const char*)(UD + ct0 * 64);
   uint4 un[2][CTP];
   auto ufrag = [&](int q, int j) {
@@ -1536,7 +1546,7 @@
     const int qa = q + LD_D - 1 < Qi ? q + LD_D - 1 : Qi - 1, qu = q + 2 < Qi ? q + 2 : Qi - 1;
     const int cur = q & 1;
 #pragma unroll
-    for (int t = 0; t < LD_NLT; t++) AR[M][t] = LDG(pa[t], qa);
+    for (int t = 0; t < LD_NLT; t++) AR[M][t] = LDA(pa[t], qa);
 #pragma unroll
     for (int j = 0; j < CTP; j++) un[C & 1][j] = ufrag(qu, j);
 #pragma unroll
@@ -1645,9 +1655,15 @@
   const unsigned grid = (unsigned)ceil_div(n_lt, 4 * LD_NLT);
   for (int ct0 = 0; ct0 < CT;) {
     const int left = CT - ct0;
-#define LD_LAUNCH(C)                                                                                             \
-  TPG_LAUNCH(ctx, "loadings_mfma", tpg_loadings_mfma_kernel<C>, dim3(grid), dim3(256), 0, (const uint4*)v->L,     \
-             (const uint4*)d_UD, n_lt, v->Q, ct0, CT, d_acc, Cpad)
+#define LD_LAUNCH(C)                                                                                                     \
+  do {                                                                                                                   \
+    if (v->LM)                                                                                                           \
+      TPG_LAUNCH(ctx, "loadings_mfma", (tpg_loadings_mfma_kernel<C, true>), dim3(grid), dim3(256), 0, (const uint4*)v->LM, \
+                 (const uint4*)d_UD, n_lt, v->Q, ct0, CT, d_acc, Cpad);                                                  \
+    else                                                                                                                 \
+      TPG_LAUNCH(ctx, "loadings_mfma", (tpg_loadings_mfma_kernel<C, false>), dim3(grid), dim3(256), 0, (const uint4*)v->L, \
+                 (const uint4*)d_UD, n_lt, v->Q, ct0, CT, d_acc, Cpad);                                                  \
+  } while (0)
     if (left >= 4) { LD_LAUNCH(4); ct0 += 4; }
     else if (left == 3) { LD_LAUNCH(3); ct0 += 3; }
     else if (left == 2) { LD_LAUNCH(2); ct0 += 2; }
@@ -1714,6 +1730,7 @@
     DevBuf d_inv;
     TPG_TRY(d_inv.alloc_n<double>((size_t)m));
     TPG_LAUNCH(ctx, "inv_scale", tpg_inv_kernel, dim3(1024), dim3(256), 0, is.dev<double>(), m, d_inv.as<double>());
+    TPG_TRY(tpg_view_need_L(ctx, v));
     TPG_TRY(run_sweep(ctx, SW_ROWSCALE, v->L, v->KG * 4, v->Q, m, n, ic.dev<double>(), d_inv.as<double>(), iu.dev<double>(), n, k,
                       ov.dev<double>(), id.dev<double>(), nullptr));
   }
diff --git a/tidypopgen_amd/csrc/runtime.hip b/tidypopgen_amd/csrc/runtime.hip
--- a/tidypopgen_amd/csrc/runtime.hip
+++ b/tidypopgen_amd/csrc/runtime.hip
@@ -1129,8 +1129,8 @@
 }
 
 static int view_create_impl(tpg_ctx* ctx, const tpg_fbm* fbm, const int32_t* rowInd1, int64_t n, const int32_t* colInd1,
-                            int64_t m, const double* code256_a, const double* code256_b, bool two, tpg_view** out_a,
-                            tpg_view** out_b) {
+                            int64_t m, const double* code256_a, const double* code256_b, bool two, bool second_locus_major,
+                            tpg_view** out_a, tpg_view** out_b) {
   TPG_REQUIRE(ctx && fbm && out_a && (!two || out_b), TPG_EINVAL, "null argument");
   if (!rowInd1) n = fbm->nrow;
   if (!colInd1) m = fbm->ncol;
@@ -1155,7 +1155,7 @@
     v[k].reset(new tpg_view(ctx, n, m));
     if (!two && code256_a) TPG_HIP(tpg_pmalloc((void**)&v[k]->T, v[k]->bytes_each));
     else if (k == 0) TPG_HIP(tpg_pmalloc((void**)&v[k]->T4, 2 * v[k]->bytes_each));
-    TPG_HIP(tpg_pmalloc((void**)&v[k]->L, v[k]->bytes_each));
+    if (!(k == 1 && second_locus_major)) TPG_HIP(tpg_pmalloc((void**)&v[k]->L, v[k]->bytes_each));
   }
   TPG_TRY(d_lut.alloc(sizeof(lut)));
   TPG_HIP(tpg_h2d_async(ctx, d_lut.p, lut, (size_t)nv * (256 + 16)));
@@ -1167,7 +1167,8 @@
     TPG_TRY(d_cols.alloc_n<int32_t>((size_t)m));
     TPG_HIP(tpg_h2d_async(ctx, d_cols.p, colInd1, sizeof(int32_t) * (size_t)m));
   }
-  TPG_TRY(tpg_launch_pack(ctx, fbm, d_rows.as<int32_t>(), d_cols.as<int32_t>(), d_lut.as<uint8_t>(), v[0].get(), v[1].get()));
+  TPG_TRY(tpg_launch_pack(ctx, fbm, d_rows.as<int32_t>(), d_cols.as<int32_t>(), d_lut.as<uint8_t>(), v[0].get(), v[1].get(),
+                          two && second_locus_major));
   uint8_t back[2 * (256 + 16)];
   TPG_HIP(tpg_fetch_small(ctx, back, d_lut.p, (size_t)nv * (256 + 16)));
   for (int k = 0; k < nv; k++) {
@@ -1184,24 +1185,34 @@
 extern "C" int tpg_view_create(tpg_ctx* ctx, const tpg_fbm* fbm, const int32_t* rowInd1, int64_t n,
                                const int32_t* colInd1, int64_t m, const double* code256, tpg_view** out) {
   TpgEnter _enter(ctx);
-  return view_create_impl(ctx, fbm, rowInd1, n, colInd1, m, code256, nullptr, false, out, nullptr);
+  return view_create_impl(ctx, fbm, rowInd1, n, colInd1, m, code256, nullptr, false, false, out, nullptr);
 }
 
 extern "C" int tpg_view_create_pair(tpg_ctx* ctx, const tpg_fbm* fbm, const int32_t* rowInd1, int64_t n,
                                     const int32_t* colInd1, int64_t m, const double* code256_a, const double* code256_b,
                                     tpg_view** out_a, tpg_view** out_b) {
-  TpgEnter _enter(ctx);
-  return view_create_impl(ctx, fbm, rowInd1, n, colInd1, m, code256_a, code256_b, true, out_a, out_b);
+  return tpg_view_create_pair_as(ctx, fbm, rowInd1, n, colInd1, m, code256_a, code256_b, true, out_a, out_b);
+}
+int tpg_view_create_pair_as(tpg_ctx* ctx, const tpg_fbm* fbm, const int32_t* rowInd1, int64_t n, const int32_t* colInd1, int64_t m,
+                            const double* code256_a, const double* code256_b, bool second_locus_major, tpg_view** out_a,
+                            tpg_view** out_b) {
+  TpgEnter _enter(ctx);
+  return view_create_impl(ctx, fbm, rowInd1, n, colInd1, m, code256_a, code256_b, true, second_locus_major, out_a, out_b);
 }
 
 tpg_view::~tpg_view() {
   drop_derived();
   if (L && !L_borrowed) tpg_pfree(L);
+  if (LM) tpg_pfree(LM);
 }
 void tpg_view::drop_derived() {
   if (T) tpg_pfree(T);
   if (T4) tpg_pfree(T4);
   if (lc_part) tpg_pfree(lc_part);
+  if (LM && L && !L_borrowed) {
+    tpg_pfree(L);
+    L = nullptr;
+  }
   T = T4 = nullptr;
   lc_part = nullptr;
   lc_chunks = 0;
diff --git a/tidypopgen_amd/csrc/stream.hip b/tidypopgen_amd/csrc/stream.hip
--- a/tidypopgen_amd/csrc/stream.hip
+++ b/tidypopgen_amd/csrc/stream.hip
@@ -483,7 +483,7 @@
     int rc;
     const int a = 0, b = ntab == 2 ? 1 : (view_of_pca >= 0 ? view_of_pca : 2);
     if (ntab == 1) rc = tpg_view_create(ctx, f, j->rowInd1, n, nullptr, 0, block_table(slot, tab[0]), &p[0]);
-    else rc = tpg_view_create_pair(ctx, f, j->rowInd1, n, nullptr, 0, tab[a], tab[b], &p[a], &p[b]);
+    else rc = tpg_view_create_pair_as(ctx, f, j->rowInd1, n, nullptr, 0, tab[a], tab[b], false, &p[a], &p[b]);
     if (rc == TPG_OK && ntab == 3) rc = tpg_view_create(ctx, f, j->rowInd1, n, nullptr, 0, tab[3 - a - b], &p[3 - a - b]);
     for (int t = 0; t < 3; t++) v[t].reset(p[t]);
     return rc;
@@ -644,6 +644,7 @@
         if (big_views) {
           const size_t per128 = (size_t)ceil_div(n, 128) * 4096;
           uint8_t* at = bigL.as<uint8_t>() + (size_t)((q0 - P0) / 128) * per128;
+          TPG_TRY(tpg_view_need_L(ctx, kp->v.get()));
           TPG_HIP(tpg_copy_dev(ctx, at, kp->v->L, (size_t)kp->v->KG * per128));
           TPG_HIP(tpg_copy_dev(ctx, big_c.as<double>() + (q0 - P0), dc, 8 * (size_t)mb));
           TPG_HIP(tpg_copy_dev(ctx, big_s.as<double>() + (q0 - P0), ds, 8 * (size_t)mb));
```
